# kepengxu/PGTFormer

Measured on NVIDIA B200. Metric: clips_per_s, higher is better.
Workload: dtype bf16

## Files before the change

pgtformer_b200/csrc/attention.cu:

```cuda
#include <cstdlib>

#include "common.cuh"

namespace pgt {

__device__ __forceinline__ void mma_bf16_16816(float (&c)[4], const uint32_t (&a)[4], uint32_t b0, uint32_t b1) {
  asm volatile(
      "mma.sync.aligned.m16n8k16.row.col.f32.bf16.bf16.f32 {%0,%1,%2,%3}, {%4,%5,%6,%7}, {%8,%9}, {%0,%1,%2,%3};"
      : "+f"(c[0]), "+f"(c[1]), "+f"(c[2]), "+f"(c[3])
      : "r"(a[0]), "r"(a[1]), "r"(a[2]), "r"(a[3]), "r"(b0), "r"(b1));
}
__device__ __forceinline__ void ldmatrix_x2_trans(uint32_t& r0, uint32_t& r1, const void* smem_row_ptr) {
  const uint32_t a = static_cast<uint32_t>(__cvta_generic_to_shared(smem_row_ptr));
  asm volatile("ldmatrix.sync.aligned.m8n8.x2.trans.shared.b16 {%0,%1}, [%2];" : "=r"(r0), "=r"(r1) : "r"(a));
}
__device__ __forceinline__ void cp_async16(void* smem_dst, const void* gsrc, bool pred) {
  const uint32_t d = static_cast<uint32_t>(__cvta_generic_to_shared(smem_dst));
  const int sz = pred ? 16 : 0;
  asm volatile("cp.async.cg.shared.global [%0], [%1], 16, %2;" ::"r"(d), "l"(gsrc), "r"(sz) : "memory");
}
__device__ __forceinline__ void cp_async_commit() { asm volatile("cp.async.commit_group;" ::: "memory"); }
template <int N>
__device__ __forceinline__ void cp_async_wait() { asm volatile("cp.async.wait_group %0;" ::"n"(N) : "memory"); }

constexpr int WIN_N = 48;

template <int D>
__global__ void __launch_bounds__(256)
window_attn_kernel(const __nv_bfloat16* __restrict__ qkv, int ldqkv, int H, int W, int C, int heads, int shift,
                   const float* __restrict__ bias_tab, __nv_bfloat16* __restrict__ out, int ldo) {
  extern __shared__ __align__(16) unsigned char smem_raw[];
  __shared__ int tok[WIN_N];
  __shared__ int lab[WIN_N];
  const int LDR = 3 * C + 8;
  __nv_bfloat16* rows = reinterpret_cast<__nv_bfloat16*>(smem_raw);
  const int nwx = W >> 2;
  const int wx = blockIdx.x % nwx, wy = blockIdx.x / nwx, clip = blockIdx.y;
  if (threadIdx.x < WIN_N) {
    const int i = threadIdx.x;
    const int fr = i >> 4, iy = (i >> 2) & 3, ix = i & 3;
    const int ys = wy * 4 + iy, xs = wx * 4 + ix;
    const int y = (ys + shift) % H, x = (xs + shift) % W;
    tok[i] = ((clip * 3 + fr) * H + y) * W + x;
    const int hr = ys < H - 4 ? 0 : (ys < H - shift ? 1 : 2);
    const int wr = xs < W - 4 ? 0 : (xs < W - shift ? 1 : 2);
    lab[i] = hr * 3 + wr;
  }
  __syncthreads();
  {
    const int chunks = (3 * C) >> 3;
    for (int i = threadIdx.x; i < WIN_N * chunks; i += 256) {
      const int r = i / chunks, c = i - r * chunks;
      cp_async16(rows + (size_t)r * LDR + c * 8, qkv + (size_t)tok[r] * ldqkv + c * 8, true);
    }
    cp_async_commit();
    cp_async_wait<0>();
  }
  __syncthreads();
  const int warp = threadIdx.x >> 5, lane = threadIdx.x & 31;
  const int g = lane >> 2, t = lane & 3;
  const float scale = rsqrtf((float)D);
  constexpr float LOG2E = 1.4426950408889634f;

// ... 69 lines not shown
        for (int nt = 0; nt < D / 8; ++nt) {
          uint32_t b0, b1;
          ldmatrix_x2_trans(b0, b1, vs + (size_t)(kk * 16 + (lane & 15)) * LDR + nt * 8);
          mma_bf16_16816(o[nt], a, b0, b1);
        }
      }
      __syncwarp();
      __nv_bfloat16* o0 = rows + (size_t)r0 * LDR + h * D;
      __nv_bfloat16* o1 = rows + (size_t)r1 * LDR + h * D;
#pragma unroll
      for (int nt = 0; nt < D / 8; ++nt) {
        *reinterpret_cast<uint32_t*>(o0 + nt * 8 + 2 * t) = pack_bf16x2(o[nt][0], o[nt][1]);
        *reinterpret_cast<uint32_t*>(o1 + nt * 8 + 2 * t) = pack_bf16x2(o[nt][2], o[nt][3]);
      }
    }
  }
  __syncthreads();
  {
    const int chunks = C >> 3;
    for (int i = threadIdx.x; i < WIN_N * chunks; i += 256) {
      const int r = i / chunks, c = i - r * chunks;
      *reinterpret_cast<uint4*>(out + (size_t)tok[r] * ldo + c * 8) = *reinterpret_cast<const uint4*>(rows + (size_t)r * LDR + c * 8);
    }
  }
}

constexpr int FA_BM = 64;
constexpr int FA_BN = 64;

template <int D>
__global__ void __launch_bounds__(128)
mha_fwd_kernel(const __nv_bfloat16* __restrict__ q, int ldq, const __nv_bfloat16* __restrict__ k, int ldk,
               const __nv_bfloat16* __restrict__ v, int ldv, int L, int heads, __nv_bfloat16* __restrict__ out, int ldo) {
  constexpr int LDS = D + 8;
  extern __shared__ __align__(16) unsigned char smem_raw[];
  __nv_bfloat16* ks = reinterpret_cast<__nv_bfloat16*>(smem_raw);
  __nv_bfloat16* vs = ks + 2 * FA_BN * LDS;
  const int qt = blockIdx.x, h = blockIdx.y, clip = blockIdx.z;
  const int warp = threadIdx.x >> 5, lane = threadIdx.x & 31, g = lane >> 2, t = lane & 3;
  const size_t row_base = (size_t)clip * L;
  const __nv_bfloat16* kbase = k + row_base * ldk + h * D;
  const __nv_bfloat16* vbase = v + row_base * ldv + h * D;
  const int ntiles = (L + FA_BN - 1) / FA_BN;
  constexpr int CH = D / 8;

  auto load_tile = [&](int tile, int buf) {
    for (int i = threadIdx.x; i < FA_BN * CH; i += 128) {
      const int r = i / CH, c = i % CH;
      const int key = tile * FA_BN + r;
      const bool ok = key < L;
      const size_t kr = ok ? key : 0;
      cp_async16(ks + ((size_t)buf * FA_BN + r) * LDS + c * 8, kbase + kr * ldk + c * 8, ok);
      cp_async16(vs + ((size_t)buf * FA_BN + r) * LDS + c * 8, vbase + kr * ldv + c * 8, ok);
    }
  };
  load_tile(0, 0);
  cp_async_commit();

  const int qr0 = qt * FA_BM + warp * 16 + g, qr1 = qr0 + 8;
  const bool v0 = qr0 < L, v1 = qr1 < L;
  const __nv_bfloat16* q0 = q + (row_base + (v0 ? qr0 : 0)) * ldq + h * D;
  const __nv_bfloat16* q1 = q + (row_base + (v1 ? qr1 : 0)) * ldq + h * D;
  uint32_t qa[D / 16][4];
#pragma unroll
  for (int kk = 0; kk < D / 16; ++kk) {
    qa[kk][0] = v0 ? __ldg(reinterpret_cast<const uint32_t*>(q0 + kk * 16 + 2 * t)) : 0u;
// ... 76 lines not shown
  __nv_bfloat16* o0 = out + (row_base + qr0) * ldo + h * D;
  __nv_bfloat16* o1 = out + (row_base + qr1) * ldo + h * D;
#pragma unroll
  for (int nt = 0; nt < D / 8; ++nt) {
    if (v0) *reinterpret_cast<uint32_t*>(o0 + nt * 8 + 2 * t) = pack_bf16x2(o[nt][0] * i0, o[nt][1] * i0);
    if (v1) *reinterpret_cast<uint32_t*>(o1 + nt * 8 + 2 * t) = pack_bf16x2(o[nt][2] * i1, o[nt][3] * i1);
  }
}

int mha_tc_launch(const void* q, int ldq, const void* k, int ldk, const void* v, int ldv, int clips, int L, int heads,
                  int d, void* out, int ldo, cudaStream_t stream);

}

using namespace pgt;

extern "C" int pgt_window_attention(const void* qkv, int ldqkv, int clips, int H, int W, int C, int heads, int shift,
                                    const float* bias_tab, void* out, int ldo, void* stream) {
  PGT_CHECK_ARG(qkv && bias_tab && out && clips > 0 && H > 0 && W > 0 && heads > 0);
  PGT_CHECK_ARG(H % 4 == 0 && W % 4 == 0 && C % heads == 0 && ldqkv % 8 == 0 && ldo % 8 == 0 && ldqkv >= 3 * C);
  PGT_CHECK_ARG(shift >= 0 && shift < 4);
  if (H <= 4 || W <= 4) shift = 0;
  const int d = C / heads;
  cudaStream_t st = static_cast<cudaStream_t>(stream);
  dim3 grid((H / 4) * (W / 4), clips);
  const size_t smem = (size_t)WIN_N * (3 * C + 8) * 2;
  ProfScope ps(PGT_PROF_WINDOW_ATTN, 4.0 * WIN_N * WIN_N * C * (double)grid.x * grid.y, st);
  if (d == 32) {
    static bool attr32 = false;
    if (!attr32) {
      PGT_CUDA_OK(cudaFuncSetAttribute(window_attn_kernel<32>, cudaFuncAttributeMaxDynamicSharedMemorySize, (int)smem));
      attr32 = true;
    }
    window_attn_kernel<32><<<grid, 256, smem, st>>>(reinterpret_cast<const __nv_bfloat16*>(qkv), ldqkv, H, W, C, heads,
                                                    shift, bias_tab, reinterpret_cast<__nv_bfloat16*>(out), ldo);
  } else if (d == 64) {
    static bool attr = false;
    if (!attr) {
      PGT_CUDA_OK(cudaFuncSetAttribute(window_attn_kernel<64>, cudaFuncAttributeMaxDynamicSharedMemorySize, (int)smem));
      attr = true;
    }
    window_attn_kernel<64><<<grid, 256, smem, st>>>(reinterpret_cast<const __nv_bfloat16*>(qkv), ldqkv, H, W, C, heads,
                                                    shift, bias_tab, reinterpret_cast<__nv_bfloat16*>(out), ldo);
  } else {
    return PGT_ERR_UNSUPPORTED;
  }
  PGT_LAUNCH_OK();
  return PGT_OK;
}

extern "C" int pgt_mha_fwd(const void* q, int ldq, const void* k, int ldk, const void* v, int ldv, int clips, int L,
                           int heads, int d, void* out, int ldo, void* stream) {
  PGT_CHECK_ARG(q && k && v && out && clips > 0 && L > 0 && heads > 0);
  PGT_CHECK_ARG(ldq % 8 == 0 && ldk % 8 == 0 && ldv % 8 == 0 && ldo % 8 == 0);
  if (d != 64) return PGT_ERR_UNSUPPORTED;
  static const bool no_tc = getenv("PGT_MHA_NO_TC") != nullptr;
  if (!no_tc) {
    ProfScope pst(PGT_PROF_MHA, 4.0 * (double)L * L * d * heads * clips, static_cast<cudaStream_t>(stream), "mha_tc");
    const int rc = mha_tc_launch(q, ldq, k, ldk, v, ldv, clips, L, heads, d, out, ldo, static_cast<cudaStream_t>(stream));
    if (rc != PGT_ERR_UNSUPPORTED) return rc;
  }
  dim3 grid(ceil_div(L, FA_BM), heads, clips);
  const size_t smem = (size_t)4 * FA_BN * (64 + 8) * 2;
  ProfScope ps(PGT_PROF_MHA, 4.0 * (double)L * L * d * heads * clips, static_cast<cudaStream_t>(stream));
  mha_fwd_kernel<64><<<grid, 128, smem, static_cast<cudaStream_t>(stream)>>>(
      reinterpret_cast<const __nv_bfloat16*>(q), ldq, reinterpret_cast<const __nv_bfloat16*>(k), ldk,
      reinterpret_cast<const __nv_bfloat16*>(v), ldv, L, heads, reinterpret_cast<__nv_bfloat16*>(out), ldo);
  PGT_LAUNCH_OK();
  return PGT_OK;
}
```

pgtformer_b200/csrc/codebook.cu:

```cuda
#include <float.h>

#include "common.cuh"

namespace pgt {

__global__ void __launch_bounds__(256)
argmax_gather_kernel(const float* __restrict__ logits, int T, int K, const float* __restrict__ codebook, int E,
                     const int64_t* __restrict__ idx_in, int64_t* __restrict__ idx_out, void* __restrict__ quant,
                     int ldq, int quant_dtype) {
  const int row = (blockIdx.x * blockDim.x + threadIdx.x) >> 5;
  const int lane = threadIdx.x & 31;
  if (row >= T) return;
  int best_i;
  if (idx_in != nullptr) {
    best_i = (int)idx_in[row];
  } else {
    const float4* p = reinterpret_cast<const float4*>(logits + (size_t)row * K);
    float best = -FLT_MAX;
    best_i = 0x7fffffff;
    const int nvec = K >> 2;
    for (int i = lane; i < nvec; i += 32) {
      float4 v;
      asm volatile("ld.global.nc.L1::no_allocate.v4.f32 {%0,%1,%2,%3}, [%4];"
                   : "=f"(v.x), "=f"(v.y), "=f"(v.z), "=f"(v.w) : "l"(p + i));
      const int b = i * 4;
      if (v.x > best) { best = v.x; best_i = b; }
      if (v.y > best) { best = v.y; best_i = b + 1; }
      if (v.z > best) { best = v.z; best_i = b + 2; }
      if (v.w > best) { best = v.w; best_i = b + 3; }
    }
#pragma unroll
    for (int o = 16; o > 0; o >>= 1) {
      const float ov = __shfl_xor_sync(0xffffffffu, best, o);
      const int oi = __shfl_xor_sync(0xffffffffu, best_i, o);
      if (ov > best || (ov == best && oi < best_i)) { best = ov; best_i = oi; }
    }
  }
  if (lane == 0 && idx_out != nullptr) idx_out[row] = best_i;
  if (quant != nullptr) {
    const float4* src = reinterpret_cast<const float4*>(codebook + (size_t)best_i * E);
    if (quant_dtype == PGT_BF16) {
      __nv_bfloat16* dst = reinterpret_cast<__nv_bfloat16*>(quant) + (size_t)row * ldq;
      for (int i = lane; i < (E >> 2); i += 32) {
        const float4 v = __ldg(src + i);
        uint2 u;
        u.x = pack_bf16x2(v.x, v.y);
        u.y = pack_bf16x2(v.z, v.w);
        *reinterpret_cast<uint2*>(dst + i * 4) = u;
      }
    } else {
      float4* dst = reinterpret_cast<float4*>(reinterpret_cast<float*>(quant) + (size_t)row * ldq);
      for (int i = lane; i < (E >> 2); i += 32) dst[i] = __ldg(src + i);
    }
  }
}

constexpr int AM_TT = 64;
constexpr int AM_TC = 64;
constexpr int AM_KC = 32;
constexpr int AM_LD = AM_TT + 4;

struct CandD {
  double v;
  int i;
};

__global__ void __launch_bounds__(256)
l2_argmin_kernel(const float* __restrict__ z, int T, int E, const float* __restrict__ cb, int K,
                 int64_t* __restrict__ idx, float* __restrict__ quant, const int* __restrict__ list,
                 const int* __restrict__ count, int min_count) {
  __shared__ __align__(16) float xs[AM_KC][AM_LD];
  __shared__ __align__(16) float es[AM_KC][AM_LD];
  __shared__ CandD merge[AM_TT][16];
  __shared__ int winner[AM_TT];
  const int tx = threadIdx.x & 15;
  const int ty = threadIdx.x >> 4;
  const int n_tok = list != nullptr ? *count : T;
  if (list != nullptr && n_tok <= min_count) return;
  auto token = [&](int i) { return list != nullptr ? list[i] : i; };
  const int lrow = threadIdx.x >> 2;
  const int lcol = (threadIdx.x & 3) * 8;
  for (int t0 = blockIdx.x * AM_TT; t0 < n_tok; t0 += gridDim.x * AM_TT) {
    CandD best[4];
#pragma unroll
    for (int a = 0; a < 4; ++a) { best[a].v = DBL_MAX; best[a].i = 0x7fffffff; }
    for (int c0 = 0; c0 < K; c0 += AM_TC) {
      double acc[4][4];
#pragma unroll
      for (int a = 0; a < 4; ++a)
#pragma unroll
        for (int b = 0; b < 4; ++b) acc[a][b] = 0.0;
      for (int k0 = 0; k0 < E; k0 += AM_KC) {
        {
          const int ti = t0 + lrow;
          float4 a = make_float4(0, 0, 0, 0), b = a;
          if (ti < n_tok) {
            const float4* p = reinterpret_cast<const float4*>(z + (size_t)token(ti) * E + k0 + lcol);
            a = __ldg(p); b = __ldg(p + 1);
          }
          xs[lcol + 0][lrow] = a.x; xs[lcol + 1][lrow] = a.y; xs[lcol + 2][lrow] = a.z; xs[lcol + 3][lrow] = a.w;
          xs[lcol + 4][lrow] = b.x; xs[lcol + 5][lrow] = b.y; xs[lcol + 6][lrow] = b.z; xs[lcol + 7][lrow] = b.w;
          const int c = c0 + lrow;
          a = make_float4(0, 0, 0, 0); b = a;
// ... 28 lines not shown
          const int c = c0 + tx * 4 + b;
          if (c < K && acc[a][b] < best[a].v) { best[a].v = acc[a][b]; best[a].i = c; }
        }
    }
#pragma unroll
    for (int a = 0; a < 4; ++a) merge[ty * 4 + a][tx] = best[a];
    __syncthreads();
    if (threadIdx.x < AM_TT) {
      CandD w = merge[threadIdx.x][0];
      for (int j = 1; j < 16; ++j) {
        const CandD c = merge[threadIdx.x][j];
        if (c.v < w.v || (c.v == w.v && c.i < w.i)) w = c;
      }
      winner[threadIdx.x] = w.i;
      if (t0 + threadIdx.x < n_tok) idx[token(t0 + threadIdx.x)] = w.i;
    }
    __syncthreads();
    if (quant != nullptr) {
      const int warp = threadIdx.x >> 5, lane = threadIdx.x & 31;
      for (int tt = warp; tt < AM_TT; tt += 8) {
        if (t0 + tt >= n_tok) continue;
        const int t = token(t0 + tt), bi = winner[tt];
        for (int e = lane; e < E; e += 32) quant[(size_t)t * E + e] = cb[(size_t)bi * E + e];
      }
    }
    __syncthreads();
  }
}

__global__ void __launch_bounds__(256)
l2_argmin_short_list_kernel(const float* __restrict__ z, int E, const float* __restrict__ cb, int K,
                            int64_t* __restrict__ idx, float* __restrict__ quant, const int* __restrict__ list,
                            const int* __restrict__ count, int max_count) {
  const int n_tok = *count;
  if (n_tok > max_count) return;
  const int lane = threadIdx.x & 31;
  const int gw = (blockIdx.x * blockDim.x + threadIdx.x) >> 5, nw = (gridDim.x * blockDim.x) >> 5;
  for (int i = gw; i < n_tok; i += nw) {
    const int t = list[i];
    double bd = DBL_MAX;
    int bi = 0x7fffffff;
    for (int k = 0; k < K; ++k) {
      double s = 0.0;
      for (int e = lane * 4; e < E; e += 128) {
        const float4 a = __ldg(reinterpret_cast<const float4*>(z + (size_t)t * E + e));
        const float4 b = __ldg(reinterpret_cast<const float4*>(cb + (size_t)k * E + e));
        double d;
        d = (double)a.x - (double)b.x; s = fma(d, d, s);
        d = (double)a.y - (double)b.y; s = fma(d, d, s);
        d = (double)a.z - (double)b.z; s = fma(d, d, s);
        d = (double)a.w - (double)b.w; s = fma(d, d, s);
      }
#pragma unroll
      for (int o = 16; o > 0; o >>= 1) s += __shfl_xor_sync(0xffffffffu, s, o);
      if (s < bd) { bd = s; bi = k; }
    }
    if (lane == 0) idx[t] = bi;
    if (quant != nullptr)
      for (int e = lane; e < E; e += 32) quant[(size_t)t * E + e] = cb[(size_t)bi * E + e];
  }
}

constexpr int AM_SHORT_LIST = 2048;

int l2_argmin_list_launch(const float* z, int T, int E, const float* codebook, int K, int64_t* idx, float* quant,
                          const int* list, const int* count, int grid, cudaStream_t st) {
  if (E % AM_KC != 0 || E % 4 != 0) return PGT_ERR_UNSUPPORTED;
  l2_argmin_short_list_kernel<<<num_sms(), 256, 0, st>>>(z, E, codebook, K, idx, quant, list, count, AM_SHORT_LIST);
  PGT_LAUNCH_OK();
  l2_argmin_kernel<<<grid, 256, 0, st>>>(z, T, E, codebook, K, idx, quant, list, count, AM_SHORT_LIST);
  PGT_LAUNCH_OK();
  return PGT_OK;
}

}

using namespace pgt;

extern "C" int pgt_argmax_gather(const float* logits, int T, int K, const float* codebook, int E,
                                 const int64_t* idx_in, int64_t* idx, void* quant, int ldq, int quant_dtype,
                                 void* stream) {
  PGT_CHECK_ARG((logits || idx_in) && T > 0 && K > 0 && K % 4 == 0);
  PGT_CHECK_ARG(quant == nullptr || (codebook != nullptr && E % 4 == 0 && ldq % 4 == 0));
  PGT_CHECK_ARG((reinterpret_cast<uintptr_t>(logits) & 15) == 0);
  const int warps = 8;
  ProfScope ps(PGT_PROF_ARGMAX, (double)T * K * 4 + (double)T * 8 + (quant ? (double)T * E * (quant_dtype == PGT_BF16 ? 2 : 4) : 0.0),
               static_cast<cudaStream_t>(stream));
  argmax_gather_kernel<<<ceil_div(T, warps), warps * 32, 0, static_cast<cudaStream_t>(stream)>>>(
      logits, T, K, codebook, E, idx_in, idx, quant, ldq, quant_dtype);
  PGT_LAUNCH_OK();
  return PGT_OK;
}

extern "C" int pgt_l2_argmin(const float* z, int T, int E, const float* codebook, int K, int64_t* idx, float* quant,
                             void* stream) {
  PGT_CHECK_ARG(z && codebook && idx && T > 0 && K > 0 && E > 0 && E % AM_KC == 0);
  PGT_CHECK_ARG((reinterpret_cast<uintptr_t>(z) & 15) == 0 && (reinterpret_cast<uintptr_t>(codebook) & 15) == 0);
  ProfScope ps(PGT_PROF_ARGMIN, 2.0 * T * (double)K * E, static_cast<cudaStream_t>(stream));
  l2_argmin_kernel<<<ceil_div(T, AM_TT), 256, 0, static_cast<cudaStream_t>(stream)>>>(z, T, E, codebook, K, idx, quant, nullptr, nullptr, 0);
  PGT_LAUNCH_OK();
  return PGT_OK;
}
```

pgtformer_b200/csrc/common.cuh:

```cuda
#pragma once
#include <cuda_bf16.h>
#include <cuda_runtime.h>
#include <stdint.h>

#include "../../include/pgt_b200.h"

namespace pgt {

void set_cuda_error(cudaError_t e, const char* where);
void count_launch(int n = 1);
int num_sms();
bool prof_enabled();
void prof_before(int cls, double work, cudaStream_t st, const char* desc);
void prof_after(cudaStream_t st);
struct ProfScope {
  cudaStream_t st; bool on;
  ProfScope(int cls, double work, cudaStream_t s, const char* desc = nullptr) : st(s), on(prof_enabled()) { if (on) prof_before(cls, work, s, desc); }
  ~ProfScope() { if (on) prof_after(st); }
};

#define PGT_CHECK_ARG(cond) \
  do {                      \
    if (!(cond)) return PGT_ERR_INVALID; \
  } while (0)

#define PGT_CUDA_OK(expr)                         \
  do {                                            \
    cudaError_t _e = (expr);                      \
    if (_e != cudaSuccess) {                      \
      ::pgt::set_cuda_error(_e, #expr);           \
      return PGT_ERR_CUDA;                        \
    }                                             \
  } while (0)

#define PGT_LAUNCH_OK()                           \
  do {                                            \
    cudaError_t _e = cudaGetLastError();          \
    if (_e != cudaSuccess) {                      \
      ::pgt::set_cuda_error(_e, "kernel launch"); \
      return PGT_ERR_CUDA;                        \
    }                                             \
    ::pgt::count_launch();                        \
  } while (0)

static inline int ceil_div(int a, int b) { return (a + b - 1) / b; }

__device__ __forceinline__ float rcp_approx(float x) {
  float r;
  asm("rcp.approx.ftz.f32 %0, %1;" : "=f"(r) : "f"(x));
  return r;
}
__device__ __forceinline__ float ex2_approx(float x) {
  float r;
  asm("ex2.approx.ftz.f32 %0, %1;" : "=f"(r) : "f"(x));
  return r;
}

__device__ __forceinline__ float gelu_erf(float v) {
  const float az = fabsf(v);
  const float t = rcp_approx(fmaf(0.3275911f * 0.70710678118654752440f, az, 1.0f));
  float poly = fmaf(1.061405429f, t, -1.453152027f);
  poly = fmaf(poly, t, 1.421413741f);
  poly = fmaf(poly, t, -0.284496736f);
  poly = fmaf(poly, t, 0.254829592f);
  const float e = ex2_approx(v * v * (-0.5f * 1.4426950408889634f));
  const float w = poly * t * e;
  return fmaf(az * -0.5f, w, fmaxf(v, 0.f));
}

__device__ __forceinline__ float apply_act(float v, int act) {
  switch (act) {
    case PGT_ACT_GELU: return gelu_erf(v);
    case PGT_ACT_SILU: return v * rcp_approx(1.0f + ex2_approx(v * -1.4426950408889634f));
    case PGT_ACT_LRELU02: return v > 0.f ? v : 0.2f * v;
    case PGT_ACT_RELU: return fmaxf(v, 0.f);
    case PGT_ACT_SIGMOID: return rcp_approx(1.0f + ex2_approx(v * -1.4426950408889634f));
    default: return v;
  }
// ... 25 lines not shown
```

pgtformer_b200/csrc/conv_out.cu:

```cuda
#include <cstdio>

#include "common.cuh"
#include "ptx.cuh"
#include "tmap.cuh"

namespace pgt {

constexpr int CO_TW = 8, CO_TH = 16;
constexpr int CO_SW = CO_TW + 2, CO_SH = CO_TH + 2;
constexpr int CO_PITCH = CO_SW * 128;
constexpr int CO_SLAB = ((CO_SH * CO_PITCH + 1023) / 1024) * 1024;
constexpr int CO_NB = 16;
constexpr int CO_WBYTES = 9 * CO_NB * 128;
constexpr int CO_BUILDERS = 256;
constexpr int CO_THREADS = 32 + CO_BUILDERS + 128;
constexpr int CO_SMEM = 2 * CO_SLAB + CO_WBYTES + 2 * 128 * 4  + 256 + 1024;

__device__ __forceinline__ uint64_t co_desc_sbo(uint32_t saddr, uint32_t sbo_bytes) {
  uint64_t d = 0;
  d |= static_cast<uint64_t>((saddr >> 4) & 0x3FFF);
  d |= static_cast<uint64_t>((sbo_bytes >> 4) & 0x3FFF) << 32;
  d |= static_cast<uint64_t>(1) << 46;
  d |= static_cast<uint64_t>(2) << 61;
  return d;
// ... 35 lines not shown
  uint8_t* sW = smem + 2 * CO_SLAB;
  float* sAB = reinterpret_cast<float*>(sW + CO_WBYTES);
  uint64_t* bars = reinterpret_cast<uint64_t*>(sAB + 2 * 128);
  uint64_t* slab_full = bars;
  uint64_t* slab_empty = bars + 2;
  uint64_t* acc_full = bars + 4;
  uint64_t* acc_empty = bars + 6;
  uint32_t* tmem_ptr = reinterpret_cast<uint32_t*>(bars + 8);

  const int warp = threadIdx.x >> 5, lane = threadIdx.x & 31;
  if (warp == 0) {
    if (lane == 0) {
      for (int i = 0; i < 2; ++i) {
        mbar_init(&slab_full[i], CO_BUILDERS);
        mbar_init(&slab_empty[i], 1);
        mbar_init(&acc_full[i], 1);
        mbar_init(&acc_empty[i], 128);
      }
      fence_barrier_init();
    }
    tmem_alloc<32>(tmem_ptr);
    tc_fence_before();
  }
  for (int i = threadIdx.x; i < 9 * CO_NB * 8; i += CO_THREADS) {
    const int tap = i / (CO_NB * 8), r = (i / 8) % CO_NB, ch = i % 8;
    uint4 v = make_uint4(0, 0, 0, 0);
    if (r < p.cout) v = __ldg(reinterpret_cast<const uint4*>(p.w + (size_t)r * p.ldw + tap * 64 + ch * 8));
    *reinterpret_cast<uint4*>(sW + tap * (CO_NB * 128) + r * 128 + ((ch ^ (r & 7)) << 4)) = v;
  }
  fence_proxy_async();
  __syncthreads();
  tc_fence_after();
  const uint32_t tmem_base = *tmem_ptr;
  const int per_frame = p.tiles_x * p.tiles_y;

  if (warp == 0) {
    constexpr uint32_t idesc = umma_idesc_bf16(128, CO_NB);
    int it = 0;
    for (int tile = blockIdx.x; tile < p.num_tiles; tile += gridDim.x, ++it) {
      const int buf = it & 1;
      const uint32_t ph = (it >> 1) & 1;
      mbar_wait(&slab_full[buf], ph);
      mbar_wait(&acc_empty[buf], ph ^ 1);
      tc_fence_after();
      if (elect_one()) {
        const uint32_t sa = smem_u32(slab + buf * CO_SLAB);
#pragma unroll
        for (int tap = 0; tap < 9; ++tap) {
          const uint64_t da = co_desc_sbo(sa + ((tap / 3) * CO_SW + (tap % 3)) * 128, CO_PITCH);
          const uint64_t db = umma_desc_k_sw128(smem_u32(sW + tap * (CO_NB * 128)));
#pragma unroll
          for (int k = 0; k < 4; ++k) umma_bf16_ss(tmem_base + buf * CO_NB, da + 2 * k, db + 2 * k, idesc, (tap | k) != 0 ? 1u : 0u);
        }
        umma_commit(&slab_empty[buf]);
        umma_commit(&acc_full[buf]);
      }
      __syncwarp();
    }
  } else if (warp <= 8) {
    const int bt = threadIdx.x - 32;
    const int chunk = bt & 7;
    int it = 0;
    for (int tile = blockIdx.x; tile < p.num_tiles; tile += gridDim.x, ++it) {
      const int buf = it & 1;
      const uint32_t ph = (it >> 1) & 1;
      const int f = tile / per_frame, r = tile - f * per_frame;
// ... 69 lines not shown
    }
  }

  tc_fence_before();
  __syncthreads();
  if (warp == 0) {
    tc_fence_after();
    tmem_dealloc<32>(tmem_base);
  }
}

}

using namespace pgt;

extern "C" int pgt_conv_out_gn(const void* x, int F, int H, int W, int Cin, int ldx, const float* gn_ab, const void* Wp,
                               int ldw, int Cout, const float* bias, float* out, void* stream) {
  PGT_CHECK_ARG(x && gn_ab && Wp && out && F > 0);
  if (Cin != 64 || Cout < 1 || Cout > 3 || H % CO_TH != 0 || W % CO_TW != 0 || ldx % 8 != 0 || ldw % 8 != 0)
    return PGT_ERR_UNSUPPORTED;
  PGT_CHECK_ARG((reinterpret_cast<uintptr_t>(x) & 15) == 0 && (reinterpret_cast<uintptr_t>(Wp) & 15) == 0 &&
                (reinterpret_cast<uintptr_t>(gn_ab) & 15) == 0);
  cudaStream_t st = static_cast<cudaStream_t>(stream);
  ConvOutParams p{};
  p.x = reinterpret_cast<const __nv_bfloat16*>(x); p.ldx = ldx; p.F = F; p.H = H; p.W = W; p.cout = Cout;
  p.ab = gn_ab; p.w = reinterpret_cast<const __nv_bfloat16*>(Wp); p.ldw = ldw; p.bias = bias; p.out = out;
  p.tiles_x = W / CO_TW; p.tiles_y = H / CO_TH; p.num_tiles = F * p.tiles_x * p.tiles_y;
  static PerDeviceOnce once;
  PGT_CUDA_OK(once.run([] { return cudaFuncSetAttribute(conv_out_gn_kernel, cudaFuncAttributeMaxDynamicSharedMemorySize, CO_SMEM); }));
  const int grid = p.num_tiles < 2 * num_sms() ? p.num_tiles : 2 * num_sms();
  char desc[64];
  snprintf(desc, sizeof(desc), "conv_out_gn F%d H%d W%d N%d", F, H, W, Cout);
  ProfScope ps(PGT_PROF_GEMM, 2.0 * F * (double)H * W * Cout * 9 * Cin, st, desc);
  conv_out_gn_kernel<<<grid, CO_THREADS, CO_SMEM, st>>>(p);
  PGT_LAUNCH_OK();
  return PGT_OK;
}
```

pgtformer_b200/csrc/elementwise.cu:

```cuda
#include <algorithm>

#include "common.cuh"
#include "tmap.cuh"

namespace pgt {

__global__ void copy2d_kernel(const __nv_bfloat16* __restrict__ x, int ldx, size_t T, int C,
                              __nv_bfloat16* __restrict__ y, int ldy) {
  const int vc = C >> 3;
  const size_t total = T * vc;
  const size_t stride = (size_t)gridDim.x * blockDim.x;
  size_t i = (size_t)blockIdx.x * blockDim.x + threadIdx.x;
  for (; i + 3 * stride < total; i += 4 * stride) {
    uint4 u[4];
#pragma unroll
    for (int k = 0; k < 4; ++k) {
      const size_t j = i + k * stride;
      u[k] = __ldg(reinterpret_cast<const uint4*>(x + (j / vc) * ldx) + (j % vc));
    }
#pragma unroll
    for (int k = 0; k < 4; ++k) {
      const size_t j = i + k * stride;
      reinterpret_cast<uint4*>(y + (j / vc) * ldy)[j % vc] = u[k];
    }
  }
  for (; i < total; i += stride)
    reinterpret_cast<uint4*>(y + (i / vc) * ldy)[i % vc] = __ldg(reinterpret_cast<const uint4*>(x + (i / vc) * ldx) + (i % vc));
}

__global__ void nchw_to_nhwc_kernel(const float* __restrict__ x, int C, int HW, const float* __restrict__ mean,
                                    const float* __restrict__ stdv, __nv_bfloat16* __restrict__ y, int ldy) {
  __shared__ float tile[32][33];
  const int f = blockIdx.z;
  const int p0 = blockIdx.x * 32, c0 = blockIdx.y * 32;
  for (int j = threadIdx.y; j < 32; j += blockDim.y) {
    const int c = c0 + j, p = p0 + threadIdx.x;
    float v = 0.f;
    if (c < C && p < HW) {
      v = x[((size_t)f * C + c) * HW + p];
      if (mean != nullptr) v = (v - mean[c]) / stdv[c];
    }
    tile[j][threadIdx.x] = v;
  }
  __syncthreads();
  for (int j = threadIdx.y; j < 32; j += blockDim.y) {
    const int p = p0 + j, c = c0 + threadIdx.x;
    if (p < HW && c < ldy && c0 + 32 <= ((C + 31) / 32) * 32) {
      if (c < C) y[((size_t)f * HW + p) * ldy + c] = __float2bfloat16_rn(tile[threadIdx.x][j]);
    }
  }
}

__global__ void nhwc_to_f32_kernel(const __nv_bfloat16* __restrict__ x, int ldx, int HW, int C, float* __restrict__ y,
                                   int to_nchw) {
  __shared__ float tile[32][33];
  const int f = blockIdx.z;
  const int p0 = blockIdx.x * 32, c0 = blockIdx.y * 32;
  for (int j = threadIdx.y; j < 32; j += blockDim.y) {
    const int p = p0 + j, c = c0 + threadIdx.x;
    tile[j][threadIdx.x] = (p < HW && c < C) ? __bfloat162float(x[((size_t)f * HW + p) * ldx + c]) : 0.f;
  }
  __syncthreads();
  if (to_nchw) {
    for (int j = threadIdx.y; j < 32; j += blockDim.y) {
      const int c = c0 + j, p = p0 + threadIdx.x;
      if (c < C && p < HW) y[((size_t)f * C + c) * HW + p] = tile[threadIdx.x][j];
    }
  } else {
    for (int j = threadIdx.y; j < 32; j += blockDim.y) {
      const int p = p0 + j, c = c0 + threadIdx.x;
      if (c < C && p < HW) y[((size_t)f * HW + p) * C + c] = tile[j][threadIdx.x];
    }
  }
}

}

using namespace pgt;

static int ew_grid(size_t total, int threads) {
  size_t b = (total + threads - 1) / threads;
  const size_t cap = (size_t)num_sms() * 32;
  return (int)(b < cap ? (b ? b : 1) : cap);
}

extern "C" int pgt_copy2d(const void* x, int ldx, int T, int C, void* y, int ldy, void* stream) {
  PGT_CHECK_ARG(x && y && T > 0 && C % 8 == 0 && ldx % 8 == 0 && ldy % 8 == 0);
  ProfScope ps(PGT_PROF_MOVE, 2.0 * (double)T * C * 2, static_cast<cudaStream_t>(stream), "pgt_copy2d");
  const size_t total = (size_t)T * (C / 8);
  copy2d_kernel<<<ew_grid(total, 256), 256, 0, static_cast<cudaStream_t>(stream)>>>(
      reinterpret_cast<const __nv_bfloat16*>(x), ldx, (size_t)T, C, reinterpret_cast<__nv_bfloat16*>(y), ldy);
  PGT_LAUNCH_OK();
  return PGT_OK;
}

extern "C" int pgt_nchw_f32_to_nhwc_bf16(const float* x, int F, int C, int HW, const float* mean, const float* stdv,
                                         void* y, int ldy, void* stream) {
  PGT_CHECK_ARG(x && y && F > 0 && C > 0 && HW > 0 && ldy >= C && (mean == nullptr) == (stdv == nullptr));
  ProfScope ps(PGT_PROF_MOVE, 6.0 * F * (double)C * HW, static_cast<cudaStream_t>(stream), "pgt_nchw_f32_to_nhwc_bf16");
  dim3 grid(ceil_div(HW, 32), ceil_div(C, 32), F);
  nchw_to_nhwc_kernel<<<grid, dim3(32, 8), 0, static_cast<cudaStream_t>(stream)>>>(
      x, C, HW, mean, stdv, reinterpret_cast<__nv_bfloat16*>(y), ldy);
  PGT_LAUNCH_OK();
  return PGT_OK;
}

extern "C" int pgt_nhwc_bf16_to_f32(const void* x, int ldx, int F, int HW, int C, float* y, int to_nchw, void* stream) {
  PGT_CHECK_ARG(x && y && F > 0 && C > 0 && HW > 0 && ldx >= C);
  ProfScope ps(PGT_PROF_MOVE, 6.0 * F * (double)C * HW, static_cast<cudaStream_t>(stream), "pgt_nhwc_bf16_to_f32");
  dim3 grid(ceil_div(HW, 32), ceil_div(C, 32), F);
  nhwc_to_f32_kernel<<<grid, dim3(32, 8), 0, static_cast<cudaStream_t>(stream)>>>(
      reinterpret_cast<const __nv_bfloat16*>(x), ldx, HW, C, y, to_nchw);
  PGT_LAUNCH_OK();
  return PGT_OK;
}

namespace pgt {
__global__ void regroup_frames_kernel(const __nv_bfloat16* __restrict__ x, int ldx, int b, int P, int C,
                                      __nv_bfloat16* __restrict__ y, int ldy, int dir) {
  const int vc = C >> 3;
  const size_t total = (size_t)b * 3 * P * vc;
  for (size_t i = (size_t)blockIdx.x * blockDim.x + threadIdx.x; i < total; i += (size_t)gridDim.x * blockDim.x) {
    const int v = (int)(i % vc);
    size_t r = i / vc;
    const int p = (int)(r % P); r /= P;
    const int fr = (int)(r % 3);
    const int clip = (int)(r / 3);
    const size_t frame_row = ((size_t)clip * 3 + fr) * P + p;
    const size_t clip_row = (size_t)clip * P + p;
    if (dir == 0)
      reinterpret_cast<uint4*>(y + clip_row * ldy + fr * C)[v] = __ldg(reinterpret_cast<const uint4*>(x + frame_row * ldx) + v);
    else
      reinterpret_cast<uint4*>(y + frame_row * ldy)[v] = __ldg(reinterpret_cast<const uint4*>(x + clip_row * ldx + fr * C) + v);
  }
}
}

extern "C" int pgt_regroup_frames(const void* x, int ldx, int clips, int P, int C, void* y, int ldy, int dir,
                                  void* stream) {
  PGT_CHECK_ARG(x && y && clips > 0 && P > 0 && C % 8 == 0 && ldx % 8 == 0 && ldy % 8 == 0 && (dir == 0 || dir == 1));
  ProfScope ps(PGT_PROF_MOVE, 4.0 * clips * 3.0 * P * C, static_cast<cudaStream_t>(stream), "pgt_regroup_frames");
  const size_t total = (size_t)clips * 3 * P * (C / 8);
  regroup_frames_kernel<<<ew_grid(total, 256), 256, 0, static_cast<cudaStream_t>(stream)>>>(
      reinterpret_cast<const __nv_bfloat16*>(x), ldx, clips, P, C, reinterpret_cast<__nv_bfloat16*>(y), ldy, dir);
  PGT_LAUNCH_OK();
  return PGT_OK;
}


namespace pgt {
__constant__ float c_u8_to_unit[256];

__global__ void u8hwc_to_f32nchw_kernel(const uint8_t* __restrict__ x, size_t HW, size_t total, float* __restrict__ y) {
  for (size_t i = (size_t)blockIdx.x * blockDim.x + threadIdx.x; i < total; i += (size_t)gridDim.x * blockDim.x) {
    const size_t f = i / HW, p = i - f * HW;
    const uint8_t* s = x + (f * HW + p) * 3;
    float* d = y + f * 3 * HW + p;
    d[0] = c_u8_to_unit[s[0]];
    d[HW] = c_u8_to_unit[s[1]];
    d[2 * HW] = c_u8_to_unit[s[2]];
  }
}

__global__ void f32nchw_to_u8hwc_kernel(const float* __restrict__ x, size_t HW, int first, int step, size_t total,
                                        uint8_t* __restrict__ y) {
  for (size_t i = (size_t)blockIdx.x * blockDim.x + threadIdx.x; i < total; i += (size_t)gridDim.x * blockDim.x) {
    const size_t j = i / HW, p = i - j * HW;
    const float* s = x + ((size_t)first + j * step) * 3 * HW + p;
    uint8_t* d = y + (j * HW + p) * 3;
#pragma unroll
    for (int c = 0; c < 3; ++c) {
      const float v = fminf(fmaxf(s[c * HW], 0.f), 1.f) * 255.0f;
      d[c] = (uint8_t)v;
    }
  }
}

__global__ void gather_frames_kernel(const uint4* __restrict__ x, size_t vec_per_frame, const int* __restrict__ idx,
                                     uint4* __restrict__ y) {
  const uint4* s = x + (size_t)idx[blockIdx.y] * vec_per_frame;
  uint4* d = y + (size_t)blockIdx.y * vec_per_frame;
  for (size_t i = (size_t)blockIdx.x * blockDim.x + threadIdx.x; i < vec_per_frame; i += (size_t)gridDim.x * blockDim.x)
    d[i] = __ldg(s + i);
}
}

extern "C" int pgt_u8hwc_to_f32nchw(const void* x_u8, int F, int H, int W, float* y, void* stream) {
  PGT_CHECK_ARG(x_u8 && y && F > 0 && H > 0 && W > 0);
  static pgt::PerDeviceOnce once;
  PGT_CUDA_OK(once.run([] {
    float t[256];
    for (int v = 0; v < 256; ++v) t[v] = (float)((double)v / 255.0);
    return cudaMemcpyToSymbol(pgt::c_u8_to_unit, t, sizeof(t));
  }));
  const size_t HW = (size_t)H * W, total = (size_t)F * HW;
  ProfScope ps(PGT_PROF_MOVE, 15.0 * (double)total, static_cast<cudaStream_t>(stream), "pgt_u8hwc_to_f32nchw");
  pgt::u8hwc_to_f32nchw_kernel<<<ew_grid(total, 256), 256, 0, static_cast<cudaStream_t>(stream)>>>(
      static_cast<const uint8_t*>(x_u8), HW, total, y);
  PGT_LAUNCH_OK();
  return PGT_OK;
}

extern "C" int pgt_f32nchw_to_u8hwc(const float* x, int first, int step, int n, int H, int W, void* y_u8, void* stream) {
  PGT_CHECK_ARG(x && y_u8 && n > 0 && H > 0 && W > 0 && first >= 0 && step >= 1);
  const size_t HW = (size_t)H * W, total = (size_t)n * HW;
  ProfScope ps(PGT_PROF_MOVE, 15.0 * (double)total, static_cast<cudaStream_t>(stream), "pgt_f32nchw_to_u8hwc");
  pgt::f32nchw_to_u8hwc_kernel<<<ew_grid(total, 256), 256, 0, static_cast<cudaStream_t>(stream)>>>(
      x, HW, first, step, total, static_cast<uint8_t*>(y_u8));
  PGT_LAUNCH_OK();
  return PGT_OK;
}

extern "C" int pgt_gather_frames(const void* x, long long frame_bytes, const int* idx_dev, int n, void* y, void* stream) {
  PGT_CHECK_ARG(x && y && idx_dev && n > 0 && frame_bytes > 0 && frame_bytes % 16 == 0);
  PGT_CHECK_ARG((reinterpret_cast<uintptr_t>(x) & 15) == 0 && (reinterpret_cast<uintptr_t>(y) & 15) == 0);
  const size_t vec = (size_t)frame_bytes / 16;
  ProfScope ps(PGT_PROF_MOVE, 2.0 * (double)n * frame_bytes, static_cast<cudaStream_t>(stream), "pgt_gather_frames");
  unsigned bx = (unsigned)std::min<size_t>((vec + 255) / 256, 1024);
  pgt::gather_frames_kernel<<<dim3(bx, n), 256, 0, static_cast<cudaStream_t>(stream)>>>(
      static_cast<const uint4*>(x), vec, idx_dev, static_cast<uint4*>(y));
  PGT_LAUNCH_OK();
  return PGT_OK;
}
```

pgtformer_b200/csrc/gemm_tc.cu:

```cuda
#include <cudaTypedefs.h>
#include <cstdio>
#include <cstdlib>

#include "common.cuh"
#include "tmap.cuh"
#include "ptx.cuh"
#include "epi_common.cuh"

namespace pgt {

constexpr int BM = 128;
constexpr int BK = 64;
constexpr int EPI_WARPS = 8;
constexpr int GEMM_THREADS = 64 + EPI_WARPS * 32 + 32;
constexpr int A_STAGE_BYTES = BM * BK * 2;
constexpr int PANEL_BYTES = BM * 128;
constexpr int NUM_SLOTS = 4;
constexpr int PREFETCH_TILES = 2;

enum { MODE_LINEAR = 0, MODE_CONV_S1 = 1, MODE_CONV_S2 = 2 };

struct GemmParams {
  int mode;
  int M, N, K;
// ... 497 lines not shown
  const int num_tiles = p.m_tiles * p.n_tiles;

  if (warp == 0 && lane == 0) {
    tma_prefetch_desc(&tmA);
    tma_prefetch_desc(&tmB);
    if (p.fast_epi) tma_prefetch_desc(&tmO);
    if (p.has_res_map) tma_prefetch_desc(&tmR);
    if (p.fast_epi && p.epi_mode == PGT_EPI_SFT) tma_prefetch_desc(&tmX);
    for (int i = 0; i < STAGES; ++i) {
      mbar_init(&full_bar[i], 1);
      mbar_init(&empty_bar[i], 1);
    }
    for (int i = 0; i < 2; ++i) {
      mbar_init(&tmem_full[i], 1);
      mbar_init(&tmem_empty[i], PAIR ? 2 * EPI_WARPS : EPI_WARPS * 32);
      mbar_init(&res_bar[2 * i], 1);
      mbar_init(&res_bar[2 * i + 1], 1);
      mbar_init(&slot_ready[2 * i], EPI_WARPS * 32);
      mbar_init(&slot_ready[2 * i + 1], EPI_WARPS * 32);
    }
    fence_barrier_init();
  }
  if (warp == 1) {
    if constexpr (PAIR) tmem_alloc_2cta<Cfg::TMEM_COLS>(tmem_ptr);
    else tmem_alloc<Cfg::TMEM_COLS>(tmem_ptr);
    tc_fence_before();
  }
  __syncthreads();
  if constexpr (PAIR) cluster_sync_all();
  tc_fence_after();
  const uint32_t tmem_base = *tmem_ptr;
  const uint32_t rank = PAIR ? cluster_ctarank() : 0u;

  if (warp == 0) {
    {
      int stage = 0;
      uint32_t phase = 0;
      for (int tile = blockIdx.x; tile < num_tiles; tile += gridDim.x) {
        int n_blk, m_blk;
        tile_mn(p, tile, m_blk, n_blk);
        int n0 = 0, y0 = 0, x0 = 0;
        if (p.mode != MODE_LINEAR) decode_conv_tile(p, m_blk, n0, y0, x0);
        for (int kb = 0; kb < p.num_kb; ++kb) {
          mbar_wait(&empty_bar[stage], phase ^ 1);
          if (elect_one()) {
            void* dst_a = smem_a + stage * A_STAGE_BYTES;
            void* dst_b = smem_b + stage * Cfg::B_STAGE_BYTES;
            int cb = 0, ax = 0, ay = 0, a5 = 0;
            if (p.mode != MODE_LINEAR) {
              const int tap = kb / p.cin_blocks;
              cb = kb - tap * p.cin_blocks;
              const int dy = tap / p.ksize;
              const int dx = tap - dy * p.ksize;
              if (p.mode == MODE_CONV_S1) {
                ax = x0 + dx - p.pad_x; ay = y0 + dy - p.pad_y;
              } else {
                const int oy = dy - p.pad_lo, ox = dx - p.pad_lo;
                const int qy = (oy < 0) ? -((1 - oy) >> 1) : (oy >> 1);
                const int qx = (ox < 0) ? -((1 - ox) >> 1) : (ox >> 1);
                const int py = oy - 2 * qy, px = ox - 2 * qx;
                cb = px * p.cin_ld + cb * BK;
                ax = x0 + qx; ay = y0 + qy; a5 = py;
              }
            }
            if constexpr (PAIR) {
              const uint32_t fb = mapa_u32(smem_u32(&full_bar[stage]), 0);
              if (rank == 0) mbar_arrive_expect_tx(&full_bar[stage], 2 * Cfg::STAGE_BYTES);
              if (p.mode == MODE_LINEAR) tma_load_2d_2sm(dst_a, &tmA, fb, kb * BK, m_blk * BM);
              else if (p.mode == MODE_CONV_S1) tma_load_4d_2sm(dst_a, &tmA, fb, cb * BK, ax, ay, n0);
              else tma_load_5d_2sm(dst_a, &tmA, fb, cb, ax, a5, ay, n0);
              tma_load_2d_2sm(dst_b, &tmB, fb, kb * BK, n_blk * BN + (int)rank * (BN / 2));
            } else {
              mbar_arrive_expect_tx(&full_bar[stage], Cfg::STAGE_BYTES);
              if (p.mode == MODE_LINEAR) tma_load_2d(dst_a, &tmA, &full_bar[stage], kb * BK, m_blk * BM);
              else if (p.mode == MODE_CONV_S1) tma_load_4d(dst_a, &tmA, &full_bar[stage], cb * BK, ax, ay, n0);
              else tma_load_5d(dst_a, &tmA, &full_bar[stage], cb, ax, a5, ay, n0);
              tma_load_2d(dst_b, &tmB, &full_bar[stage], kb * BK, n_blk * BN);
            }
          }
          __syncwarp();
          if (++stage == STAGES) { stage = 0; phase ^= 1; }
        }
      }
    }
  } else if (warp == 1) {
    if (!PAIR || rank == 0) {
      constexpr uint32_t idesc = umma_idesc_bf16(PAIR ? 2 * BM : BM, BN);
      int stage = 0;
      uint32_t phase = 0;
      int it = 0;
      for (int tile = blockIdx.x; tile < num_tiles; tile += gridDim.x, ++it) {
        const int acc = it & 1;
        const uint32_t acc_phase = (it >> 1) & 1;
        mbar_wait(&tmem_empty[acc], acc_phase ^ 1);
        tc_fence_after();
        const uint32_t d_tmem = tmem_base + acc * BN;
        if (elect_one()) {
          int s = stage;
          uint32_t ph = phase;
          const uint64_t da0 = umma_desc_k_sw128(smem_u32(smem_a));
          const uint64_t db0 = umma_desc_k_sw128(smem_u32(smem_b));
          for (int kb = 0; kb < p.num_kb; ++kb) {
            mbar_wait(&full_bar[s], ph);
            tc_fence_after();
            const uint64_t da = da0 + (uint64_t)(s * (A_STAGE_BYTES >> 4));
            const uint64_t db = db0 + (uint64_t)(s * (Cfg::B_STAGE_BYTES >> 4));
#pragma unroll
            for (int k = 0; k < BK / 16; ++k) {
              if constexpr (PAIR) umma_bf16_ss_2cta(d_tmem, da + 2 * k, db + 2 * k, idesc, (kb | k) != 0 ? 1u : 0u);
              else umma_bf16_ss(d_tmem, da + 2 * k, db + 2 * k, idesc, (kb | k) != 0 ? 1u : 0u);
// ... 82 lines not shown
  uint64_t* a_ready = tmem_full + 14;

  const int warp = threadIdx.x >> 5;
  const int lane = threadIdx.x & 31;
  const int num_tiles = p.m_tiles * p.n_tiles;
  const int cin_pad = p.cin_blocks * BK;

  if (warp == 0 && lane == 0) {
    tma_prefetch_desc(&tmA);
    tma_prefetch_desc(&tmB);
    if (p.fast_epi) tma_prefetch_desc(&tmO);
    if (p.has_res_map) tma_prefetch_desc(&tmR);
    if (p.fast_epi && p.epi_mode == PGT_EPI_SFT) tma_prefetch_desc(&tmX);
    for (int i = 0; i < AS; ++i) { mbar_init(&a_full[i], 1); mbar_init(&a_empty[i], 1); mbar_init(&a_ready[i], HALO_GN_THREADS); }
    for (int i = 0; i < BS; ++i) { mbar_init(&b_full[i], 1); mbar_init(&b_empty[i], 1); }
    for (int i = 0; i < 2; ++i) {
      mbar_init(&tmem_full[i], 1);
      mbar_init(&tmem_empty[i], EPI_WARPS * 32);
      mbar_init(&res_bar[2 * i], 1);
      mbar_init(&res_bar[2 * i + 1], 1);
      mbar_init(&slot_ready[2 * i], EPI_WARPS * 32);
      mbar_init(&slot_ready[2 * i + 1], EPI_WARPS * 32);
    }
    fence_barrier_init();
  }
  if (warp == 1) {
    tmem_alloc<Cfg::TMEM_COLS>(tmem_ptr);
    tc_fence_before();
  }
  __syncthreads();
  tc_fence_after();
  const uint32_t tmem_base = *tmem_ptr;

  if (warp == 0) {
    int as = 0, bs = 0;
    uint32_t aph = 0, bph = 0;
    for (int tile = blockIdx.x; tile < num_tiles; tile += gridDim.x) {
      const int n_blk = tile % p.n_tiles;
      const int m_blk = tile / p.n_tiles;
      int n0, y0, x0;
      decode_conv_tile(p, m_blk, n0, y0, x0);
      {
        const int pt = tile + PREFETCH_TILES * (int)gridDim.x;
        if (BN == 64 && pt < num_tiles && elect_one()) {
          int pn0, py0, px0;
          decode_conv_tile(p, pt / p.n_tiles, pn0, py0, px0);
          for (int cb = 0; cb < p.cin_blocks; ++cb) tma_prefetch_4d(&tmA, cb * BK, px0 - 1, py0 - 1, pn0);
          if (p.has_res_map) {
            const int c0 = (pt % p.n_tiles) * BN;
            const int rw = p.out_dtype == PGT_BF16 ? 64 : 32;
            for (int c = 0; c < BN && c0 + c < p.N; c += rw) {
              tma_prefetch_4d(&tmR, c0 + c, px0, py0, pn0);
              if (p.epi_mode == PGT_EPI_SFT) tma_prefetch_4d(&tmX, c0 + c, px0, py0, pn0);
            }
          }
        }
        __syncwarp();
      }
      for (int cb = 0; cb < p.cin_blocks; ++cb) {
        mbar_wait(&a_empty[as], aph ^ 1);
        if (elect_one()) {
          mbar_arrive_expect_tx(&a_full[as], HALO_A_BYTES);
          tma_load_4d(smem_a + as * HALO_A_STRIDE, &tmA, &a_full[as], cb * BK, x0 - 1, y0 - 1, n0);
        }
        __syncwarp();
        if (++as == AS) { as = 0; aph ^= 1; }
        if (p.b_resident && tile != (int)blockIdx.x) continue;
        for (int t = 0; t < p.ntaps; ++t) {
          mbar_wait(&b_empty[bs], bph ^ 1);
          if (elect_one()) {
            mbar_arrive_expect_tx(&b_full[bs], Cfg::B_BYTES);
            tma_load_2d(smem_b + bs * Cfg::B_BYTES, &tmB, &b_full[bs], t * cin_pad + cb * BK, n_blk * BN);
          }
          __syncwarp();
          if (++bs == BS) { bs = 0; bph ^= 1; }
        }
      }
    }
  } else if (warp == 1) {
    constexpr uint32_t idesc = umma_idesc_bf16(BM, BN);
    int as = 0, bs = 0;
    uint32_t aph = 0, bph = 0;
    int it = 0;
    for (int tile = blockIdx.x; tile < num_tiles; tile += gridDim.x, ++it) {
      const int acc = it & 1;
      const uint32_t acc_phase = (it >> 1) & 1;
      mbar_wait(&tmem_empty[acc], acc_phase ^ 1);
      tc_fence_after();
      const uint32_t d_tmem = tmem_base + acc * BN;
      if (elect_one()) {
        int a = as, b = bs;
        uint32_t ap = aph, bp = bph;
        const uint64_t da_base = umma_desc_k_sw128_sbo(smem_u32(smem_a), HALO_PITCH);
        const uint64_t db_base = umma_desc_k_sw128(smem_u32(smem_b));
        for (int cb = 0; cb < p.cin_blocks; ++cb) {
          mbar_wait(GN ? &a_ready[a] : &a_full[a], ap);
          const uint64_t da0 = da_base + (uint64_t)(a * (HALO_A_STRIDE >> 4));
          if (p.b_resident) {
            if (it == 0) {
              for (int t = 0; t < p.ntaps; ++t) mbar_wait(&b_full[cb * p.ntaps + t], 0);
            }
            tc_fence_after();
            if (p.ntaps == 9) {
#pragma unroll
              for (int t = 0; t < 9; ++t) {
                const uint64_t da = da0 + (uint64_t)(((t / 3) * (HALO_TW + 2) + (t % 3)) * 8);
                const uint64_t db = db_base + (uint64_t)((cb * 9 + t) * (Cfg::B_BYTES >> 4));
// ... 155 lines not shown

  const int warp = threadIdx.x >> 5;
  const int lane = threadIdx.x & 31;
  const uint32_t rank = cluster_ctarank();
  const int num_tiles = p.m_tiles;
  const int cin_pad = p.cin_blocks * BK;

  if (warp == 0 && lane == 0) {
    tma_prefetch_desc(&tmA);
    tma_prefetch_desc(&tmB);
    if (p.fast_epi) tma_prefetch_desc(&tmO);
    if (p.has_res_map) tma_prefetch_desc(&tmR);
    if (p.fast_epi && p.epi_mode == PGT_EPI_SFT) tma_prefetch_desc(&tmX);
    for (int i = 0; i < AS; ++i) { mbar_init(&a_full[i], 1); mbar_init(&a_empty[i], 1); }
    for (int i = 0; i < BS; ++i) { mbar_init(&b_full[i], 1); mbar_init(&b_empty[i], 1); }
    for (int i = 0; i < 2; ++i) {
      mbar_init(&tmem_full[i], 1);
      mbar_init(&tmem_empty[i], 2 * EPI_WARPS);
      mbar_init(&res_bar[2 * i], 1);
      mbar_init(&res_bar[2 * i + 1], 1);
      mbar_init(&slot_ready[2 * i], EPI_WARPS * 32);
      mbar_init(&slot_ready[2 * i + 1], EPI_WARPS * 32);
    }
    fence_barrier_init();
  }
  if (warp == 1) {
    tmem_alloc_2cta<Cfg::TMEM_COLS>(tmem_ptr);
    tc_fence_before();
  }
  __syncthreads();
  cluster_sync_all();
  tc_fence_after();
  const uint32_t tmem_base = *tmem_ptr;

  if (warp == 0) {
    int as = 0, bs = 0;
    uint32_t aph = 0, bph = 0;
    const uint32_t a_full0 = mapa_u32(smem_u32(a_full), 0), b_full0 = mapa_u32(smem_u32(b_full), 0);
    for (int tile = blockIdx.x; tile < num_tiles; tile += gridDim.x) {
      int n0, y0, x0;
      decode_conv_tile(p, tile, n0, y0, x0);
      {
        const int pt = tile + PREFETCH_TILES * (int)gridDim.x;
        if (BN == 64 && pt < num_tiles && elect_one()) {
          int pn0, py0, px0;
          decode_conv_tile(p, pt, pn0, py0, px0);
          for (int cb = 0; cb < p.cin_blocks; ++cb) tma_prefetch_4d(&tmA, cb * BK, px0 - 1, py0 - 1, pn0);
          if (p.has_res_map) {
            const int rw = p.out_dtype == PGT_BF16 ? 64 : 32;
            for (int c = 0; c < BN && c < p.N; c += rw) {
              tma_prefetch_4d(&tmR, c, px0, py0, pn0);
              if (p.epi_mode == PGT_EPI_SFT) tma_prefetch_4d(&tmX, c, px0, py0, pn0);
            }
          }
        }
        __syncwarp();
      }
      for (int cb = 0; cb < p.cin_blocks; ++cb) {
        mbar_wait(&a_empty[as], aph ^ 1);
        if (elect_one()) {
          if (rank == 0) mbar_arrive_expect_tx(&a_full[as], 2 * HALO_A_BYTES);
          tma_load_4d_2sm(smem_a + as * HALO_A_STRIDE, &tmA, a_full0 + as * 8, cb * BK, x0 - 1, y0 - 1, n0);
        }
        __syncwarp();
        if (++as == AS) { as = 0; aph ^= 1; }
        if (p.b_resident && tile != (int)blockIdx.x) continue;
        for (int t = 0; t < p.ntaps; ++t) {
          mbar_wait(&b_empty[bs], bph ^ 1);
          if (elect_one()) {
            if (rank == 0) mbar_arrive_expect_tx(&b_full[bs], 2 * Cfg::B_BYTES);
            tma_load_2d_2sm(smem_b + bs * Cfg::B_BYTES, &tmB, b_full0 + bs * 8, t * cin_pad + cb * BK, (int)rank * (BN / 2));
          }
          __syncwarp();
          if (++bs == BS) { bs = 0; bph ^= 1; }
        }
      }
    }
  } else if (warp == 1) {
    if (rank == 0) {
      constexpr uint32_t idesc = umma_idesc_bf16(2 * BM, BN);
      int as = 0, bs = 0;
      uint32_t aph = 0, bph = 0;
      int it = 0;
      for (int tile = blockIdx.x; tile < num_tiles; tile += gridDim.x, ++it) {
        const int acc = it & 1;
        const uint32_t acc_phase = (it >> 1) & 1;
        mbar_wait(&tmem_empty[acc], acc_phase ^ 1);
        tc_fence_after();
        const uint32_t d_tmem = tmem_base + acc * BN;
        if (elect_one()) {
          int a = as, b = bs;
          uint32_t ap = aph, bp = bph;
          const uint64_t da_base = umma_desc_k_sw128_sbo(smem_u32(smem_a), HALO_PITCH);
          const uint64_t db_base = umma_desc_k_sw128(smem_u32(smem_b));
          for (int cb = 0; cb < p.cin_blocks; ++cb) {
            mbar_wait(&a_full[a], ap);
            const uint64_t da0 = da_base + (uint64_t)(a * (HALO_A_STRIDE >> 4));
            if (p.ntaps == 9) {
#pragma unroll
              for (int t = 0; t < 9; ++t) {
                int slot = b;
                if (p.b_resident) {
                  slot = cb * 9 + t;
                  if (it == 0) mbar_wait(&b_full[slot], 0);
                } else {
                  mbar_wait(&b_full[b], bp);
// ... 126 lines not shown
  return PGT_OK;
}

static int encode_weight_map(CUtensorMap* tmB, const void* W, int ldw, int K, int N, int BN) {
  uint64_t dims[2] = {(uint64_t)K, (uint64_t)N};
  uint64_t str[1] = {(uint64_t)ldw * 2};
  uint32_t box[2] = {BK, (uint32_t)BN};
  return encode_map(tmB, W, 2, dims, str, box);
}

template <int BN, bool PAIR>
static int launch_gemm(const CUtensorMap& tmA, const void* W, int ldw, GemmParams& p, cudaStream_t stream) {
  using Cfg = GemmCfg<BN, PAIR>;
  static_assert(Cfg::STAGES >= 3, "pipeline too shallow");
  CUtensorMap tmB, tmO, tmR, tmX;
  int rc = encode_weight_map(&tmB, W, ldw, p.K, p.N, PAIR ? BN / 2 : BN);
  if (rc != PGT_OK) return rc;
  rc = setup_epilogue_maps(p, tmA, tmO, tmR, tmX);
  if (rc != PGT_OK) return rc;
  p.n_tiles = ceil_div(p.N, BN);
  p.pair_map = PAIR ? 1 : 0;
  static PerDeviceOnce once;
  PGT_CUDA_OK(once.run([] { return cudaFuncSetAttribute(gemm_tc_kernel<BN, PAIR>, cudaFuncAttributeMaxDynamicSharedMemorySize, Cfg::SMEM_BYTES); }));
  const int tiles = p.m_tiles * p.n_tiles;
  int grid = tiles < num_sms() ? tiles : num_sms();
  if (PAIR) grid &= ~1;
  {
    char desc[96];
    if (prof_enabled()) {
      if (p.mode == MODE_LINEAR) snprintf(desc, sizeof(desc), "linear%s M%d N%d K%d BN%d e%d", PAIR ? " x2cta" : "", p.M, p.N, p.K, BN, p.fast_epi);
      else snprintf(desc, sizeof(desc), "conv%d%s s%d F%d H%d W%d K%d N%d BN%d t%dx%dx%d e%d", p.ksize, PAIR ? " x2cta" : "", p.mode, p.F, p.H, p.W, p.K, p.N, BN, p.tn, p.th, p.tw, p.fast_epi);
    }
    ProfScope ps(PGT_PROF_GEMM, p.flops, stream, desc);
    if (PAIR) {
      cudaLaunchConfig_t cfg = {};
      cfg.gridDim = dim3(grid); cfg.blockDim = dim3(GEMM_THREADS); cfg.dynamicSmemBytes = Cfg::SMEM_BYTES; cfg.stream = stream;
      cudaLaunchAttribute attr[1];
      attr[0].id = cudaLaunchAttributeClusterDimension;
      attr[0].val.clusterDim.x = 2; attr[0].val.clusterDim.y = 1; attr[0].val.clusterDim.z = 1;
      cfg.attrs = attr; cfg.numAttrs = 1;
      PGT_CUDA_OK(cudaLaunchKernelEx(&cfg, gemm_tc_kernel<BN, PAIR>, tmA, tmB, tmO, tmR, tmX, p));
    } else {
      gemm_tc_kernel<BN, PAIR><<<grid, GEMM_THREADS, Cfg::SMEM_BYTES, stream>>>(tmA, tmB, tmO, tmR, tmX, p);
    }
  }
  PGT_LAUNCH_OK();
  return PGT_OK;
}

template <int BN, bool GN>
static int launch_halo(const CUtensorMap& tmA, const void* W, int ldw, GemmParams& p, cudaStream_t stream) {
  using Cfg = HaloCfg<BN>;
  CUtensorMap tmB, tmO, tmR, tmX;
  int rc = encode_weight_map(&tmB, W, ldw, p.K, p.N, BN);
  if (rc != PGT_OK) return rc;
  rc = setup_epilogue_maps(p, tmA, tmO, tmR, tmX);
  if (rc != PGT_OK) return rc;
  p.n_tiles = ceil_div(p.N, BN);
  p.b_resident = (p.ntaps * p.cin_blocks <= Cfg::B_STAGES && p.n_tiles == 1) ? 1 : 0;
  static PerDeviceOnce once;
  PGT_CUDA_OK(once.run([] { return cudaFuncSetAttribute(conv_halo_kernel<BN, GN>, cudaFuncAttributeMaxDynamicSharedMemorySize, Cfg::SMEM_BYTES); }));
  const int tiles = p.m_tiles * p.n_tiles;
  const int grid = tiles < num_sms() ? tiles : num_sms();
  {
    char desc[96];
    if (prof_enabled())
      snprintf(desc, sizeof(desc), "halo3%s F%d H%d W%d K%d N%d BN%d e%d r%d", GN ? "+gn" : "", p.F, p.H, p.W, p.K, p.N, BN,
               p.fast_epi, p.b_resident);
    ProfScope ps(PGT_PROF_GEMM, p.flops, stream, desc);
    conv_halo_kernel<BN, GN><<<grid, GN ? GEMM_THREADS + HALO_GN_THREADS : GEMM_THREADS, Cfg::SMEM_BYTES, stream>>>(
        tmA, tmB, tmO, tmR, tmX, p);
  }
  PGT_LAUNCH_OK();
  return PGT_OK;
}

template <int BN>
static int launch_halo2(const CUtensorMap& tmA, const void* W, int ldw, GemmParams& p, cudaStream_t stream) {
  using Cfg = Halo2Cfg<BN>;
  CUtensorMap tmB, tmO, tmR, tmX;
  int rc = encode_weight_map(&tmB, W, ldw, p.K, p.N, BN / 2);
  if (rc != PGT_OK) return rc;
  rc = setup_epilogue_maps(p, tmA, tmO, tmR, tmX);
  if (rc != PGT_OK) return rc;
  p.n_tiles = 1;
  p.b_resident = (p.ntaps * p.cin_blocks <= Cfg::B_STAGES) ? 1 : 0;
  static PerDeviceOnce once;
  PGT_CUDA_OK(once.run([] { return cudaFuncSetAttribute(conv_halo2_kernel<BN>, cudaFuncAttributeMaxDynamicSharedMemorySize, Cfg::SMEM_BYTES); }));
  int grid = p.m_tiles < num_sms() ? p.m_tiles : num_sms();
  grid &= ~1;
  {
    char desc[96];
    if (prof_enabled())
      snprintf(desc, sizeof(desc), "halo%d x2cta F%d H%d W%d K%d N%d BN%d e%d r%d", p.tap_kw, p.F, p.H, p.W, p.K, p.N, BN,
               p.fast_epi, p.b_resident);
    ProfScope ps(PGT_PROF_GEMM, p.flops, stream, desc);
    conv_halo2_kernel<BN><<<grid, GEMM_THREADS, Cfg::SMEM_BYTES, stream>>>(tmA, tmB, tmO, tmR, tmX, p);
  }
  PGT_LAUNCH_OK();
  return PGT_OK;
}

static int pick_bn(int N, int m_tiles) {
  if (N <= 64) return 64;
  if (N <= 128) return 128;
  const int t256 = m_tiles * ceil_div(N, 256);
  return (t256 >= num_sms()) ? 256 : 128;
}

static int dispatch_gemm(const CUtensorMap& tmA, const void* W, int ldw, GemmParams& p, cudaStream_t stream) {
  static const bool no_pair = getenv("PGT_NO_2CTA") != nullptr;
  switch (pick_bn(p.N, p.m_tiles)) {
    case 64: return launch_gemm<64, false>(tmA, W, ldw, p, stream);
    case 128: return launch_gemm<128, false>(tmA, W, ldw, p, stream);
    default:
      if (!no_pair && p.mode != MODE_LINEAR && p.num_kb >= 16 && (p.m_tiles % 2) == 0 && p.m_tiles >= 2)
        return launch_gemm<256, true>(tmA, W, ldw, p, stream);
      return launch_gemm<256, false>(tmA, W, ldw, p, stream);
  }
}

static int fill_epilogue(GemmParams& p, const pgt_epilogue* ep) {
  if (ep == nullptr || ep->out == nullptr) return PGT_ERR_INVALID;
  p.bias = ep->bias;
  p.act = ep->act;
  p.epi_mode = ep->mode;
  p.residual = ep->residual;
  p.ldr = ep->ldr;
  p.res_dtype = ep->res_dtype;
  p.aux = ep->aux;
  p.ldaux = ep->ldaux;
  p.sft_w = ep->sft_w;
// ... 188 lines not shown
```

pgtformer_b200/csrc/l2_argmin_tc.cu:

```cuda
#include <float.h>

#include "common.cuh"
#include "ptx.cuh"
#include "tmap.cuh"

namespace pgt {

constexpr int LT_BM = 128;
constexpr int LT_BN = 256;
constexpr int LT_BK = 64;
constexpr int LT_EMAX = 512;
constexpr int LT_A_KB_BYTES = LT_BM * 128;
constexpr int LT_KBMAX = LT_EMAX / LT_BK;
constexpr int LT_BST = (LT_BN / 2) * 128;
constexpr int LT_NST = 3;
constexpr int LT_THREADS = 11 * 32;
constexpr int LT_TOP = 16;
constexpr int LT_LIST = 16;
constexpr int LT_XCH = 2 * LT_BM * LT_LIST * 8  + 2 * LT_BM * 4  + LT_BM * LT_TOP * 4  + 2 * LT_BM * 4 ;
constexpr int LT_SMEM = LT_BM * LT_EMAX * 2 + LT_NST * LT_BST + LT_XCH + 512  + 1024 ;

__device__ __forceinline__ float4 ld_nc_f4(const float4* p) {
  float4 v;
  asm("ld.global.nc.L1::no_allocate.v4.f32 {%0,%1,%2,%3}, [%4];" : "=f"(v.x), "=f"(v.y), "=f"(v.z), "=f"(v.w) : "l"(p));
  return v;
}

__global__ void __launch_bounds__(256)
codebook_pack_kernel(const float* __restrict__ cb, int K, int E, __nv_bfloat16* __restrict__ cb16, float* __restrict__ norm) {
  const int row = (blockIdx.x * blockDim.x + threadIdx.x) >> 5, lane = threadIdx.x & 31;
  if (row >= K) return;
  double s = 0.0;
  float sr = 0.f, sd = 0.f;
  for (int e = lane; e < E; e += 32) {
    const float v = cb[(size_t)row * E + e];
    const __nv_bfloat16 b = __float2bfloat16_rn(v);
    const float vb = __bfloat162float(b);
    cb16[(size_t)row * E + e] = b;
    s += (double)v * (double)v;
    sr = fmaf(vb, vb, sr);
    const float dd = v - vb;
    sd = fmaf(dd, dd, sd);
  }
#pragma unroll
  for (int o = 16; o > 0; o >>= 1) {
    s += __shfl_xor_sync(0xffffffffu, s, o);
    sr += __shfl_xor_sync(0xffffffffu, sr, o);
    sd += __shfl_xor_sync(0xffffffffu, sd, o);
  }
  if (lane == 0) {
    norm[row] = (float)s;
    atomicMax(reinterpret_cast<int*>(norm + K), __float_as_int(sr * 1.0001f));
    atomicMax(reinterpret_cast<int*>(norm + K + 1), __float_as_int(sd * 1.0001f));
  }
}

__global__ void __launch_bounds__(256)
z_pack_kernel(const float* __restrict__ z, int T, int E, __nv_bfloat16* __restrict__ zb, float2* __restrict__ zn2) {
  constexpr int RB = 4;
  const int lane = threadIdx.x & 31;
  const int gw = (blockIdx.x * blockDim.x + threadIdx.x) >> 5, nw = (gridDim.x * blockDim.x) >> 5;
  const int nstep = (E + 255) / 256;
  for (int t0 = gw * RB; t0 < T; t0 += nw * RB) {
    float4 va[RB][2][2];
#pragma unroll
    for (int i = 0; i < RB; ++i) {
#pragma unroll
      for (int sp = 0; sp < 2; ++sp) {
        const int c = sp * 256 + lane * 8;
        if (sp < nstep && t0 + i < T && c < E) {
          const float4* p = reinterpret_cast<const float4*>(z + (size_t)(t0 + i) * E + c);
          va[i][sp][0] = ld_nc_f4(p);
          va[i][sp][1] = ld_nc_f4(p + 1);
        } else {
          va[i][sp][0] = va[i][sp][1] = make_float4(0.f, 0.f, 0.f, 0.f);
        }
      }
    }
#pragma unroll
    for (int i = 0; i < RB; ++i) {
      const int t = t0 + i;
      if (t >= T) break;
      float s2 = 0.f, d2 = 0.f;
#pragma unroll
      for (int sp = 0; sp < 2; ++sp) {
        const int c = sp * 256 + lane * 8;
        if (sp < nstep && c < E) {
          const float4 a = va[i][sp][0], b = va[i][sp][1];
          const float f[8] = {a.x, a.y, a.z, a.w, b.x, b.y, b.z, b.w};
          uint32_t u[4];
#pragma unroll
// ... 138 lines not shown
  int* ncand = mi + LT_BM * LT_TOP;
  int* ovf = ncand + LT_BM;
  uint64_t* b_full = reinterpret_cast<uint64_t*>(tail + LT_XCH);
  uint64_t* b_empty = b_full + LT_NST;
  uint64_t* a_full = b_empty + LT_NST;
  uint64_t* a_empty = a_full + LT_KBMAX;
  uint64_t* t_full = a_empty + LT_KBMAX;
  uint64_t* t_empty = t_full + 2;
  uint32_t* tmem_ptr = reinterpret_cast<uint32_t*>(t_empty + 2);

  const int warp = threadIdx.x >> 5, lane = threadIdx.x & 31;
  const int KB = E / LT_BK;
  const int NT = K / LT_BN;
  const int n_pt = (T + 2 * LT_BM - 1) / (2 * LT_BM);
  const int pair = blockIdx.x >> 1, npairs = gridDim.x >> 1;

  if (warp == 0 && lane == 0) {
    tma_prefetch_desc(&tmA);
    tma_prefetch_desc(&tmB);
    for (int i = 0; i < LT_NST; ++i) { mbar_init(&b_full[i], 1); mbar_init(&b_empty[i], 1); }
    for (int i = 0; i < LT_KBMAX; ++i) { mbar_init(&a_full[i], 1); mbar_init(&a_empty[i], 1); }
    for (int i = 0; i < 2; ++i) { mbar_init(&t_full[i], 1); mbar_init(&t_empty[i], 8); }
    fence_barrier_init();
  }
  if (warp == 1) {
    tmem_alloc_2cta<512>(tmem_ptr);
    tc_fence_before();
  }
  if (threadIdx.x < LT_BM) { ncand[threadIdx.x] = 0; ovf[threadIdx.x] = 0; }
  __syncthreads();
  cluster_sync_all();
  tc_fence_after();
  const uint32_t tmem_base = *tmem_ptr;
  const uint32_t rank = cluster_ctarank();

  if (warp == 0) {
    int st = 0;
    uint32_t ph = 0;
    for (int pt = pair; pt < n_pt; pt += npairs) {
      for (int nt = 0; nt < NT; ++nt) {
        for (int kb = 0; kb < KB; ++kb) {
          mbar_wait(&b_empty[st], ph ^ 1);
          if (elect_one()) {
            const uint32_t fb = mapa_u32(smem_u32(&b_full[st]), 0);
            if (rank == 0) mbar_arrive_expect_tx(&b_full[st], 2 * LT_BST);
            tma_load_2d_2sm(sB + st * LT_BST, &tmB, fb, kb * LT_BK, nt * LT_BN + (int)rank * (LT_BN / 2));
          }
          __syncwarp();
          if (++st == LT_NST) { st = 0; ph ^= 1; }
        }
      }
    }
  } else if (warp == 10) {
    int it = 0;
    for (int pt = pair; pt < n_pt; pt += npairs, ++it) {
      const int t0 = pt * 2 * LT_BM + (int)rank * LT_BM;
      for (int kb = 0; kb < KB; ++kb) {
        if (it > 0) mbar_wait(&a_empty[kb], (it - 1) & 1);
        if (elect_one()) {
          const uint32_t fa = mapa_u32(smem_u32(&a_full[kb]), 0);
          if (rank == 0) mbar_arrive_expect_tx(&a_full[kb], 2 * LT_A_KB_BYTES);
          tma_load_2d_2sm(sA + kb * LT_A_KB_BYTES, &tmA, fa, kb * LT_BK, t0);
        }
        __syncwarp();
      }
    }
// ... 101 lines not shown
          while (have != 0) {
            const int l = __ffs(have) - 1;
            have &= have - 1;
            const int b = __shfl_sync(0xffffffffu, best, l);
            const float4* src = reinterpret_cast<const float4*>(cb + (size_t)b * E);
            float4* dst = reinterpret_cast<float4*>(quant + (size_t)(t0 + w8 + 8 * l) * E);
            for (int e = lane; e < (E >> 2); e += 32) dst[e] = __ldg(src + e);
          }
        }
      }
    }
  }

  tc_fence_before();
  __syncthreads();
  cluster_sync_all();
  if (warp == 1) {
    tc_fence_after();
    tmem_dealloc_2cta<512>(tmem_base);
  }
}

int l2_argmin_list_launch(const float* z, int T, int E, const float* codebook, int K, int64_t* idx, float* quant,
                          const int* list, const int* count, int grid, cudaStream_t st);

}

using namespace pgt;

extern "C" int pgt_codebook_pack(const float* codebook, int K, int E, void* cb_bf16, float* cb_norm, void* stream) {
  PGT_CHECK_ARG(codebook && cb_bf16 && cb_norm && K > 0 && E > 0);
  cudaStream_t st = static_cast<cudaStream_t>(stream);
  PGT_CUDA_OK(cudaMemsetAsync(cb_norm + K, 0, 2 * sizeof(float), st));
  codebook_pack_kernel<<<ceil_div(K, 8), 256, 0, st>>>(codebook, K, E, reinterpret_cast<__nv_bfloat16*>(cb_bf16), cb_norm);
  PGT_LAUNCH_OK();
  return PGT_OK;
}

static inline int64_t ws_align4(int64_t v) { return (v + 3) & ~int64_t(3); }
static inline int64_t ws_off_list(int T) { (void)T; return 4; }
static inline int64_t ws_off_zn2(int T) { return ws_align4(ws_off_list(T) + T); }
static inline int64_t ws_off_zb(int T) { return ws_align4(ws_off_zn2(T) + (int64_t)T * 2); }

extern "C" int64_t pgt_l2_argmin_ws_ints(int T) {
  return ws_off_zb(T) + (int64_t)T * (LT_EMAX / 2);
}

extern "C" int pgt_l2_argmin_tc(const float* z, int T, int E, const float* codebook, const void* cb_bf16,
                                const float* cb_norm, int K, int64_t* idx, float* quant, int32_t* workspace,
                                void* stream) {
  PGT_CHECK_ARG(z && codebook && cb_bf16 && cb_norm && idx && workspace && T > 0);
  if (K % LT_BN != 0 || E % LT_BK != 0 || E > LT_EMAX || E % 128 != 0) return PGT_ERR_UNSUPPORTED;
  PGT_CHECK_ARG((reinterpret_cast<uintptr_t>(z) & 15) == 0 && (reinterpret_cast<uintptr_t>(codebook) & 15) == 0 &&
                (reinterpret_cast<uintptr_t>(cb_bf16) & 15) == 0 && (reinterpret_cast<uintptr_t>(workspace) & 15) == 0 &&
                (quant == nullptr || (reinterpret_cast<uintptr_t>(quant) & 15) == 0));
  cudaStream_t st = static_cast<cudaStream_t>(stream);
  int* fb_count = workspace;
  int* fb_list = workspace + ws_off_list(T);
  float2* zn2 = reinterpret_cast<float2*>(workspace + ws_off_zn2(T));
  __nv_bfloat16* zb = reinterpret_cast<__nv_bfloat16*>(workspace + ws_off_zb(T));
  CUtensorMap tmA, tmB;
  int rc = tmap_rows_bf16(&tmA, zb, E, T, E, LT_BM);
  if (rc == PGT_OK) rc = tmap_rows_bf16(&tmB, cb_bf16, E, K, E, LT_BN / 2);
  if (rc != PGT_OK) return rc;
  static PerDeviceOnce once;
  PGT_CUDA_OK(once.run([] { return cudaFuncSetAttribute(l2_argmin_pair_kernel, cudaFuncAttributeMaxDynamicSharedMemorySize, LT_SMEM); }));
  PGT_CUDA_OK(cudaMemsetAsync(workspace, 0, sizeof(int32_t), st));
  const int n_pt = ceil_div(T, 2 * LT_BM);
  const int npairs = n_pt < num_sms() / 2 ? n_pt : num_sms() / 2;
  {
    ProfScope ps(PGT_PROF_ARGMIN, 2.0 * T * (double)K * E, st, "l2_argmin_tc");
    int pack_ctas = num_sms() * 2;
    {
      const long long items = ceil_div(T, 4);
      long long best_waste = -1;
      for (int c = num_sms() * 2; c >= num_sms(); --c) {
        const long long w = (long long)c * 8;
        const long long waste = ((items + w - 1) / w) * w - items;
        if (best_waste < 0 || waste < best_waste) { best_waste = waste; pack_ctas = c; }
      }
    }
    z_pack_kernel<<<pack_ctas, 256, 0, st>>>(z, T, E, zb, zn2);
    l2_argmin_pair_kernel<<<2 * npairs, LT_THREADS, LT_SMEM, st>>>(tmA, tmB, z, zn2, T, E, codebook, cb_norm, K, idx, quant,
                                                                   fb_count, fb_list);
    PGT_LAUNCH_OK();
  }
  return l2_argmin_list_launch(z, T, E, codebook, K, idx, quant, fb_list, fb_count, num_sms(), st);
}
```

pgtformer_b200/csrc/ln_linear.cu:

```cuda
#include <cudaTypedefs.h>

#include <cstdio>

#include "common.cuh"
#include "tmap.cuh"
#include "ptx.cuh"

namespace pgt {

constexpr int LL_C = 256;
constexpr int LL_BM = 128;
constexpr int LL_SUB = LL_BM * 128;
constexpr int LL_WST = 2;
constexpr int LL_WBYTES = LL_C * 128;
constexpr int LL_THREADS = 480;
constexpr int LL_SMEM = 8 * LL_SUB  + 2 * LL_SUB  + LL_WST * LL_WBYTES + 256;
static_assert(LL_SMEM <= 232448, "ln_linear smem budget");

struct LnLinearParams {
  int T, m_tiles, nb;
  const float* ln_g;
  const float* ln_b;
  float eps;
  const float* bias;
// ... 7 lines not shown
  uint8_t* sX = smem;
  uint8_t* sO = sX + 8 * LL_SUB;
  uint8_t* sW = sO + 2 * LL_SUB;
  uint64_t* bars = reinterpret_cast<uint64_t*>(sW + LL_WST * LL_WBYTES);
  uint64_t* x_full = bars;
  uint64_t* sx_free = bars + 2;
  uint64_t* y_ready = bars + 4;
  uint64_t* acc_full = bars + 6;
  uint64_t* acc_free = bars + 8;
  uint64_t* so_free = bars + 10;
  uint64_t* out_ready = bars + 12;
  uint64_t* w_full = bars + 14;
  uint64_t* w_empty = w_full + LL_WST;
  uint32_t* tmem_ptr = reinterpret_cast<uint32_t*>(w_empty + LL_WST);

  const int warp = threadIdx.x >> 5, lane = threadIdx.x & 31;
  if (warp == 0 && lane == 0) {
    tma_prefetch_desc(&tmX); tma_prefetch_desc(&tmO); tma_prefetch_desc(&tmW);
    for (int i = 0; i < 2; ++i) {
      mbar_init(&x_full[i], 1); mbar_init(&sx_free[i], 1); mbar_init(&y_ready[i], 128);
      mbar_init(&acc_full[i], 1); mbar_init(&acc_free[i], 256);
      mbar_init(&so_free[i], 1); mbar_init(&out_ready[i], 256);
    }
    for (int i = 0; i < LL_WST; ++i) { mbar_init(&w_full[i], 1); mbar_init(&w_empty[i], 1); }
    fence_barrier_init();
  }
  if (warp == 1) {
    tmem_alloc<512>(tmem_ptr);
    tc_fence_before();
  }
  __syncthreads();
  tc_fence_after();
  const uint32_t tmem_base = *tmem_ptr;
  const int NB = p.nb;

  if (warp == 0) {
    int st = 0;
    uint32_t ph = 0;
    for (int tile = blockIdx.x; tile < p.m_tiles; tile += gridDim.x) {
      for (int j = 0; j < NB; ++j) {
        for (int kb = 0; kb < 4; ++kb) {
          mbar_wait(&w_empty[st], ph ^ 1);
          if (elect_one()) {
            mbar_arrive_expect_tx(&w_full[st], LL_WBYTES);
            tma_load_2d(sW + st * LL_WBYTES, &tmW, &w_full[st], kb * 64, j * LL_C);
          }
          __syncwarp();
          if (++st == LL_WST) { st = 0; ph ^= 1; }
        }
      }
    }
  } else if (warp == 1) {
    constexpr uint32_t idesc = umma_idesc_bf16(LL_BM, LL_C);
    int st = 0;
    uint32_t ph = 0;
    int it = 0;
    for (int tile = blockIdx.x; tile < p.m_tiles; tile += gridDim.x, ++it) {
      const int xb = it & 1;
      mbar_wait(&y_ready[xb], (it >> 1) & 1);
      tc_fence_after();
      if (elect_one()) {
        int s = st;
        uint32_t sp = ph;
        const uint64_t da0 = umma_desc_k_sw128(smem_u32(sX + xb * 4 * LL_SUB));
        const uint64_t db0 = umma_desc_k_sw128(smem_u32(sW));
        for (int j = 0; j < NB; ++j) {
// ... 173 lines not shown
  }
}

static int ll_enc2d(CUtensorMap* map, const void* base, int ld, long long rows, int cols, int box_rows) {
  return tmap_rows_bf16(map, base, ld, rows, cols, box_rows);
}

}

using namespace pgt;

extern "C" int pgt_ln_linear_bf16(const void* x, int ldx, int T, int C, const float* ln_g, const float* ln_b, float eps,
                                  const void* W, int ldw, int N, const float* bias, void* out, int ldo, void* stream) {
  PGT_CHECK_ARG(x && out && W && bias && T > 0 && N > 0 && ((ln_g == nullptr) == (ln_b == nullptr)));
  if (C != LL_C || (N % LL_C) != 0) return PGT_ERR_UNSUPPORTED;
  auto al = [](const void* q) { return (reinterpret_cast<uintptr_t>(q) & 15) == 0; };
  PGT_CHECK_ARG(al(x) && al(out) && al(W) && ldx % 8 == 0 && ldo % 8 == 0 && ldw % 8 == 0 && ldw >= C && ldo >= N);
  CUtensorMap tx, to, tw;
  int rc = ll_enc2d(&tx, x, ldx, T, C, LL_BM);
  if (rc == PGT_OK) rc = ll_enc2d(&to, out, ldo, T, N, LL_BM);
  if (rc == PGT_OK) rc = ll_enc2d(&tw, W, ldw, N, C, LL_C);
  if (rc != PGT_OK) return rc;
  static PerDeviceOnce once;
  PGT_CUDA_OK(once.run([] { return cudaFuncSetAttribute(ln_linear_kernel, cudaFuncAttributeMaxDynamicSharedMemorySize, LL_SMEM); }));
  LnLinearParams p{};
  p.T = T; p.m_tiles = ceil_div(T, LL_BM); p.nb = N / LL_C;
  p.ln_g = ln_g; p.ln_b = ln_b; p.eps = eps; p.bias = bias;
  cudaStream_t st = static_cast<cudaStream_t>(stream);
  const int grid = p.m_tiles < num_sms() ? p.m_tiles : num_sms();
  {
    char desc[64];
    if (prof_enabled()) snprintf(desc, sizeof(desc), "ln_linear M%d N%d K256", T, N);
    ProfScope ps(PGT_PROF_GEMM, 2.0 * (double)T * N * C, st, desc);
    ln_linear_kernel<<<grid, LL_THREADS, LL_SMEM, st>>>(tx, to, tw, p);
  }
  PGT_LAUNCH_OK();
  return PGT_OK;
}
```

pgtformer_b200/csrc/mha_tc.cu:

```cuda
#include <cudaTypedefs.h>

#include "common.cuh"
#include "tmap.cuh"
#include "ptx.cuh"

namespace pgt {

constexpr int FT_D = 64;
constexpr int FT_BM = 128;
constexpr int FT_BN = 128;
constexpr int FT_NST = 3;
constexpr int FT_TILE = FT_BN * FT_D * 2;
constexpr int FT_THREADS = 64 + 256;
constexpr int FT_SMEM = 2 * FT_TILE  + FT_NST * 2 * FT_TILE  + 2 * 2 * FT_TILE  + FT_TILE  + 256 + 1024;
constexpr float FT_TAU = 256.f;

__device__ __forceinline__ void tmem_st_32x32(uint32_t taddr, const uint32_t (&v)[32]) {
  asm volatile(
      "tcgen05.st.sync.aligned.32x32b.x32.b32 [%0], "
      "{%1, %2, %3, %4, %5, %6, %7, %8, %9, %10, %11, %12, %13, %14, %15, %16, "
      "%17, %18, %19, %20, %21, %22, %23, %24, %25, %26, %27, %28, %29, %30, %31, %32};"
      ::"r"(taddr), "r"(v[0]), "r"(v[1]), "r"(v[2]), "r"(v[3]), "r"(v[4]), "r"(v[5]), "r"(v[6]), "r"(v[7]), "r"(v[8]),
        "r"(v[9]), "r"(v[10]), "r"(v[11]), "r"(v[12]), "r"(v[13]), "r"(v[14]), "r"(v[15]), "r"(v[16]), "r"(v[17]),
        "r"(v[18]), "r"(v[19]), "r"(v[20]), "r"(v[21]), "r"(v[22]), "r"(v[23]), "r"(v[24]), "r"(v[25]), "r"(v[26]),
// ... 54 lines not shown
  uint64_t* kv_empty = kv_full + FT_NST;
  uint64_t* s_full = kv_empty + FT_NST;
  uint64_t* p_full = s_full + 2;
  uint64_t* o_full = p_full + 2;
  uint32_t* tmem_ptr = reinterpret_cast<uint32_t*>(o_full + 2);

  const int warp = threadIdx.x >> 5, lane = threadIdx.x & 31;
  const int h = blockIdx.y, clip = blockIdx.z;
  const int q0 = clip * L + blockIdx.x * 2 * FT_BM;
  const int kv0 = clip * L;
  const int NT = L / FT_BN;

  if (warp == 0 && lane == 0) {
    tma_prefetch_desc(&tmQ); tma_prefetch_desc(&tmK); tma_prefetch_desc(&tmV);
    mbar_init(q_full, 1);
    for (int i = 0; i < FT_NST; ++i) { mbar_init(&kv_full[i], 1); mbar_init(&kv_empty[i], 1); }
    for (int g = 0; g < 2; ++g) {
      mbar_init(&s_full[g], 1);
      mbar_init(&p_full[g], 128);
      mbar_init(&o_full[g], 1);
    }
    fence_barrier_init();
  }
  for (int i = threadIdx.x; i < FT_TILE / 16; i += FT_THREADS)
    reinterpret_cast<uint4*>(sOnes)[i] = make_uint4(0x3F803F80u, 0x3F803F80u, 0x3F803F80u, 0x3F803F80u);
  fence_proxy_async();
  if (warp == 1) {
    tmem_alloc<512>(tmem_ptr);
    tc_fence_before();
  }
  __syncthreads();
  tc_fence_after();
  const uint32_t tmem_base = *tmem_ptr;

  if (warp == 0) {
    if (elect_one()) {
      mbar_arrive_expect_tx(q_full, 2 * FT_TILE);
      tma_load_2d(sQ, &tmQ, q_full, h * FT_D, q0);
      tma_load_2d(sQ + FT_TILE, &tmQ, q_full, h * FT_D, q0 + FT_BM);
    }
    __syncwarp();
    int st = 0;
    uint32_t ph = 0;
    for (int j = 0; j < NT; ++j) {
      mbar_wait(&kv_empty[st], ph ^ 1);
      if (elect_one()) {
        mbar_arrive_expect_tx(&kv_full[st], 2 * FT_TILE);
        tma_load_2d(sK + st * FT_TILE, &tmK, &kv_full[st], h * FT_D, kv0 + j * FT_BN);
        tma_load_2d(sV + st * FT_TILE, &tmV, &kv_full[st], h * FT_D, kv0 + j * FT_BN);
      }
      __syncwarp();
      if (++st == FT_NST) { st = 0; ph ^= 1; }
    }
  } else if (warp == 1) {
    constexpr uint32_t idesc_s = umma_idesc_bf16(FT_BM, FT_BN);
    constexpr uint32_t idesc_o = umma_idesc_bf16(FT_BM, FT_D) | (1u << 16);
    auto issue_s = [&](int g, int st) {
      const uint64_t da = umma_desc_k_sw128(smem_u32(sQ + g * FT_TILE));
      const uint64_t db = umma_desc_k_sw128(smem_u32(sK + st * FT_TILE));
#pragma unroll
      for (int k = 0; k < FT_D / 16; ++k) umma_bf16_ss(tmem_base + g * FT_BN, da + 2 * k, db + 2 * k, idesc_s, k != 0 ? 1u : 0u);
      umma_commit(&s_full[g]);
    };
    constexpr uint32_t idesc_o80 = umma_idesc_bf16(FT_BM, FT_D + 16) | (1u << 16);
    auto issue_o = [&](int g, int st, uint32_t acc) {
#pragma unroll
// ... 132 lines not shown
        u.z = pack_bf16x2(__uint_as_float(v[8 * q + 4]) * inv, __uint_as_float(v[8 * q + 5]) * inv);
        u.w = pack_bf16x2(__uint_as_float(v[8 * q + 6]) * inv, __uint_as_float(v[8 * q + 7]) * inv);
        reinterpret_cast<uint4*>(orow)[(c >> 3) + q] = u;
      }
    }
  }

  tc_fence_before();
  __syncthreads();
  if (warp == 1) {
    tc_fence_after();
    tmem_dealloc<512>(tmem_base);
  }
}

static int encode_rows_map(CUtensorMap* map, const void* base, int ld, long long rows, int cols) {
  return tmap_rows_bf16(map, base, ld, rows, cols, FT_BN);
}

int mha_tc_launch(const void* q, int ldq, const void* k, int ldk, const void* v, int ldv, int clips, int L, int heads,
                  int d, void* out, int ldo, cudaStream_t stream) {
  if (d != FT_D || L % (2 * FT_BM) != 0) return PGT_ERR_UNSUPPORTED;
  auto al = [](const void* p) { return (reinterpret_cast<uintptr_t>(p) & 15) == 0; };
  if (!al(q) || !al(k) || !al(v) || !al(out) || ldq % 8 || ldk % 8 || ldv % 8 || ldo % 8) return PGT_ERR_UNSUPPORTED;
  CUtensorMap tq, tk, tv;
  const long long rows = (long long)clips * L;
  int rc = encode_rows_map(&tq, q, ldq, rows, heads * d);
  if (rc == PGT_OK) rc = encode_rows_map(&tk, k, ldk, rows, heads * d);
  if (rc == PGT_OK) rc = encode_rows_map(&tv, v, ldv, rows, heads * d);
  if (rc != PGT_OK) return rc;
  static PerDeviceOnce once;
  PGT_CUDA_OK(once.run([] { return cudaFuncSetAttribute(mha_tc_kernel, cudaFuncAttributeMaxDynamicSharedMemorySize, FT_SMEM); }));
  dim3 grid(L / (2 * FT_BM), heads, clips);
  mha_tc_kernel<<<grid, FT_THREADS, FT_SMEM, stream>>>(tq, tk, tv, L, reinterpret_cast<__nv_bfloat16*>(out), ldo);
  PGT_LAUNCH_OK();
  return PGT_OK;
}

}
```

pgtformer_b200/csrc/norm.cu:

```cuda
#include "common.cuh"

namespace pgt {

constexpr int GN_GROUPS = 32;
constexpr int GN_MAX_CHUNKS = 64;
constexpr int GN_THREADS = 512;

__device__ __forceinline__ void load8_bf16(const __nv_bfloat16* p, float (&v)[8]) {
  const uint4 u = __ldg(reinterpret_cast<const uint4*>(p));
  float2 a = unpack_bf16x2(u.x), b = unpack_bf16x2(u.y), c = unpack_bf16x2(u.z), d = unpack_bf16x2(u.w);
  v[0] = a.x; v[1] = a.y; v[2] = b.x; v[3] = b.y; v[4] = c.x; v[5] = c.y; v[6] = d.x; v[7] = d.y;
}
__device__ __forceinline__ void store8_bf16(__nv_bfloat16* p, const float (&v)[8]) {
  uint4 u;
  u.x = pack_bf16x2(v[0], v[1]); u.y = pack_bf16x2(v[2], v[3]);
  u.z = pack_bf16x2(v[4], v[5]); u.w = pack_bf16x2(v[6], v[7]);
  *reinterpret_cast<uint4*>(p) = u;
}

__global__ void __launch_bounds__(GN_THREADS)
gn_stats_kernel(const __nv_bfloat16* __restrict__ x, int ldx, int HW, int C, int pix_per_chunk,
                float* __restrict__ partial ) {
  extern __shared__ float sm[];
  const int vc = C >> 3;
  const int rows_par = GN_THREADS / vc;
  const int vcol = threadIdx.x % vc;
  const int prow = threadIdx.x / vc;
  const int chunk = blockIdx.x, f = blockIdx.y, nchunks = gridDim.x;
  const int p0 = chunk * pix_per_chunk;
  const int p1 = min(HW, p0 + pix_per_chunk);
  float s[8], q[8];
#pragma unroll
  for (int i = 0; i < 8; ++i) { s[i] = 0.f; q[i] = 0.f; }
  if (prow < rows_par) {
    const __nv_bfloat16* base = x + ((size_t)f * HW) * ldx + vcol * 8;
    int p = p0 + prow;
    for (; p + 3 * rows_par < p1; p += 4 * rows_par) {
      float v0[8], v1[8], v2[8], v3[8];
      load8_bf16(base + (size_t)p * ldx, v0);
      load8_bf16(base + (size_t)(p + rows_par) * ldx, v1);
      load8_bf16(base + (size_t)(p + 2 * rows_par) * ldx, v2);
      load8_bf16(base + (size_t)(p + 3 * rows_par) * ldx, v3);
#pragma unroll
      for (int i = 0; i < 8; ++i) {
        s[i] += (v0[i] + v1[i]) + (v2[i] + v3[i]);
        q[i] += (v0[i] * v0[i] + v1[i] * v1[i]) + (v2[i] * v2[i] + v3[i] * v3[i]);
      }
    }
    for (; p < p1; p += rows_par) {
      float v[8];
      load8_bf16(base + (size_t)p * ldx, v);
#pragma unroll
      for (int i = 0; i < 8; ++i) { s[i] += v[i]; q[i] += v[i] * v[i]; }
    }
#pragma unroll
    for (int i = 0; i < 8; ++i) {
      sm[(prow * 2 + 0) * C + vcol * 8 + i] = s[i];
      sm[(prow * 2 + 1) * C + vcol * 8 + i] = q[i];
    }
  }
  __syncthreads();
  for (int c = threadIdx.x; c < 2 * C; c += GN_THREADS) {
    const int which = c / C, ch = c % C;
    float t = 0.f;
    for (int rr = 0; rr < rows_par; ++rr) t += sm[(rr * 2 + which) * C + ch];
    sm[(size_t)rows_par * 2 * C + c] = t;
  }
  __syncthreads();
  if (threadIdx.x < GN_GROUPS) {
    const float* tot = sm + (size_t)rows_par * 2 * C;
    const int cpg = C / GN_GROUPS;
    float gs = 0.f, gq = 0.f;
    for (int c = threadIdx.x * cpg; c < (threadIdx.x + 1) * cpg; ++c) { gs += tot[c]; gq += tot[C + c]; }
    float* o = partial + (((size_t)f * nchunks + chunk) * GN_GROUPS + threadIdx.x) * 2;
    o[0] = gs; o[1] = gq;
  }
}

constexpr int GN_FIN_PARTS = 32;
__global__ void __launch_bounds__(GN_FIN_PARTS * 32)
gn_finalize_kernel(const float* __restrict__ partial, int nchunks, int HW, int C, const float* __restrict__ gamma,
                   const float* __restrict__ beta, float eps, float* __restrict__ ab ) {
  __shared__ float smean[GN_GROUPS], srstd[GN_GROUPS];
  __shared__ double ps[GN_FIN_PARTS][GN_GROUPS], pq[GN_FIN_PARTS][GN_GROUPS];
  const int f = blockIdx.x;
  const int cpg = C / GN_GROUPS;
  {
    const int g = threadIdx.x & 31, part = threadIdx.x >> 5;
    const float2* base = reinterpret_cast<const float2*>(partial) + (size_t)f * nchunks * GN_GROUPS + g;
    double s = 0.0, q = 0.0;
    int ch = part;
    for (; ch + 3 * GN_FIN_PARTS < nchunks; ch += 4 * GN_FIN_PARTS) {
      const float2 o0 = __ldg(base + (size_t)ch * GN_GROUPS);
      const float2 o1 = __ldg(base + (size_t)(ch + GN_FIN_PARTS) * GN_GROUPS);
      const float2 o2 = __ldg(base + (size_t)(ch + 2 * GN_FIN_PARTS) * GN_GROUPS);
      const float2 o3 = __ldg(base + (size_t)(ch + 3 * GN_FIN_PARTS) * GN_GROUPS);
      s += ((double)o0.x + (double)o1.x) + ((double)o2.x + (double)o3.x);
      q += ((double)o0.y + (double)o1.y) + ((double)o2.y + (double)o3.y);
    }
    for (; ch < nchunks; ch += GN_FIN_PARTS) {
      const float2 o = __ldg(base + (size_t)ch * GN_GROUPS);
      s += (double)o.x; q += (double)o.y;
    }
    ps[part][g] = s; pq[part][g] = q;
  }
  __syncthreads();
  if (threadIdx.x < GN_GROUPS) {
    double s = 0.0, q = 0.0;
    for (int part = 0; part < GN_FIN_PARTS; ++part) { s += ps[part][threadIdx.x]; q += pq[part][threadIdx.x]; }
    const double n = (double)HW * cpg;
    const double mean = s / n;
    double var = q / n - mean * mean;
    if (var < 0.0) var = 0.0;
    smean[threadIdx.x] = (float)mean;
    srstd[threadIdx.x] = (float)(1.0 / sqrt(var + (double)eps));
  }
  __syncthreads();
  for (int c = threadIdx.x; c < C; c += blockDim.x) {
    const int g = c / cpg;
    const float a = srstd[g] * gamma[c];
    ab[((size_t)f * 2 + 0) * C + c] = a;
    ab[((size_t)f * 2 + 1) * C + c] = beta[c] - smean[g] * a;
  }
}

constexpr int GN_APPLY_THREADS = 256;
__global__ void __launch_bounds__(GN_APPLY_THREADS, 3)
gn_apply_kernel(const __nv_bfloat16* __restrict__ x, int ldx, int HW, int C, int pix_per_block,
                const float* __restrict__ ab, int apply_silu, __nv_bfloat16* __restrict__ y, int ldy) {
  const int f = blockIdx.y;
  const int vc = C >> 3;
  const int rows_par = GN_APPLY_THREADS / vc;
  const int vcol = threadIdx.x % vc;
  const int prow = threadIdx.x / vc;
  if (prow >= rows_par) return;
  float a[8], b[8];
  {
    const float4* pa = reinterpret_cast<const float4*>(ab + ((size_t)f * 2 + 0) * C + vcol * 8);
    const float4* pb = reinterpret_cast<const float4*>(ab + ((size_t)f * 2 + 1) * C + vcol * 8);
    const float4 a0 = __ldg(pa), a1 = __ldg(pa + 1), b0 = __ldg(pb), b1 = __ldg(pb + 1);
    a[0] = a0.x; a[1] = a0.y; a[2] = a0.z; a[3] = a0.w; a[4] = a1.x; a[5] = a1.y; a[6] = a1.z; a[7] = a1.w;
    b[0] = b0.x; b[1] = b0.y; b[2] = b0.z; b[3] = b0.w; b[4] = b1.x; b[5] = b1.y; b[6] = b1.z; b[7] = b1.w;
  }
  const int p0 = blockIdx.x * pix_per_block;
  const int p1 = min(HW, p0 + pix_per_block);
  const __nv_bfloat16* xb = x + ((size_t)f * HW) * ldx + vcol * 8;
  __nv_bfloat16* yb = y + ((size_t)f * HW) * ldy + vcol * 8;
  if (apply_silu) {
#pragma unroll
    for (int j = 0; j < 8; ++j) { a[j] *= 0.5f; b[j] *= 0.5f; }
  }
  auto act = [&](float (&v)[8]) {
#pragma unroll
    for (int j = 0; j < 8; ++j) {
      const float h = fmaf(v[j], a[j], b[j]);
      float th;
      asm("tanh.approx.f32 %0, %1;" : "=f"(th) : "f"(h));
      v[j] = apply_silu ? fmaf(h, th, h) : h;
    }
  };
  int p = p0 + prow;
  for (; p + 3 * rows_par < p1; p += 4 * rows_par) {
    float v0[8], v1[8], v2[8], v3[8];
    load8_bf16(xb + (size_t)p * ldx, v0);
    load8_bf16(xb + (size_t)(p + rows_par) * ldx, v1);
    load8_bf16(xb + (size_t)(p + 2 * rows_par) * ldx, v2);
    load8_bf16(xb + (size_t)(p + 3 * rows_par) * ldx, v3);
    act(v0); act(v1); act(v2); act(v3);
    store8_bf16(yb + (size_t)p * ldy, v0);
    store8_bf16(yb + (size_t)(p + rows_par) * ldy, v1);
    store8_bf16(yb + (size_t)(p + 2 * rows_par) * ldy, v2);
    store8_bf16(yb + (size_t)(p + 3 * rows_par) * ldy, v3);
  }
  for (; p < p1; p += rows_par) {
    float v[8];
    load8_bf16(xb + (size_t)p * ldx, v);
    act(v);
    store8_bf16(yb + (size_t)p * ldy, v);
  }
}

constexpr int LN_ROWS = 4;
template <int NV, bool POS>
__global__ void __launch_bounds__(256)
layernorm_kernel(const void* __restrict__ xin, int ldx, int x_dtype, int T, const float* __restrict__ gamma,
                 const float* __restrict__ beta, float eps, __nv_bfloat16* __restrict__ y, int ldy,
                 const __nv_bfloat16* __restrict__ pos, int ldpos, __nv_bfloat16* __restrict__ y2, int ldy2) {
  constexpr int C = 256 * NV;
  const int warp = (blockIdx.x * blockDim.x + threadIdx.x) >> 5;
  const int lane = threadIdx.x & 31;
  const int row0 = warp * LN_ROWS;
  if (row0 >= T) return;
  float v[LN_ROWS][NV][8];
#pragma unroll
  for (int r = 0; r < LN_ROWS; ++r) {
    const int row = min(row0 + r, T - 1);
#pragma unroll
    for (int i = 0; i < NV; ++i) {
      const int c0 = (i * 32 + lane) * 8;
      if (x_dtype == PGT_BF16) {
        load8_bf16(reinterpret_cast<const __nv_bfloat16*>(xin) + (size_t)row * ldx + c0, v[r][i]);
      } else {
        const float4* p = reinterpret_cast<const float4*>(reinterpret_cast<const float*>(xin) + (size_t)row * ldx + c0);
        const float4 a = __ldg(p), b = __ldg(p + 1);
        v[r][i][0] = a.x; v[r][i][1] = a.y; v[r][i][2] = a.z; v[r][i][3] = a.w;
        v[r][i][4] = b.x; v[r][i][5] = b.y; v[r][i][6] = b.z; v[r][i][7] = b.w;
      }
    }
  }
  uint4 pr[POS ? LN_ROWS : 1][NV];
  if constexpr (POS) {
#pragma unroll
    for (int r = 0; r < LN_ROWS; ++r) {
      const int row = min(row0 + r, T - 1);
#pragma unroll
      for (int i = 0; i < NV; ++i)
        pr[r][i] = __ldg(reinterpret_cast<const uint4*>(pos + (size_t)row * ldpos + (i * 32 + lane) * 8));
    }
  }
  float g[NV][8], bt[NV][8];
// ... 17 lines not shown
    for (int o = 16; o > 0; o >>= 1) {
      s += __shfl_xor_sync(0xffffffffu, s, o);
      q += __shfl_xor_sync(0xffffffffu, q, o);
    }
    const float mean = s * (1.0f / C);
    const float rstd = rsqrtf(fmaxf(q * (1.0f / C) - mean * mean, 0.f) + eps);
    const float nm = -mean * rstd;
    if (row < T) {
#pragma unroll
      for (int i = 0; i < NV; ++i) {
        const int c0 = (i * 32 + lane) * 8;
        float o[8];
#pragma unroll
        for (int j = 0; j < 8; ++j) o[j] = fmaf(fmaf(v[r][i][j], rstd, nm), g[i][j], bt[i][j]);
        store8_bf16(y + (size_t)row * ldy + c0, o);
        if constexpr (POS) {
          const uint32_t pw[4] = {pr[r][i].x, pr[r][i].y, pr[r][i].z, pr[r][i].w};
#pragma unroll
          for (int j = 0; j < 4; ++j) {
            const float2 pv = unpack_bf16x2(pw[j]);
            o[2 * j] += pv.x; o[2 * j + 1] += pv.y;
          }
          store8_bf16(y2 + (size_t)row * ldy2 + c0, o);
        }
      }
    }
  }
}

constexpr int ADAIN_THREADS = 256;
__global__ void __launch_bounds__(ADAIN_THREADS)
adain_kernel(const void* __restrict__ qin, int ldq, int q_dtype, const __nv_bfloat16* __restrict__ l, int ldl, int HW,
             int C, float eps, __nv_bfloat16* __restrict__ y, int ldy) {
  __shared__ float red[4][ADAIN_THREADS / 8][64];
  __shared__ float sa[64], sb[64];
  const int f = blockIdx.y;
  const int cbase = blockIdx.x * 64;
  const int vcol = threadIdx.x & 7;
  const int prow = threadIdx.x >> 3;
  const int rows_par = ADAIN_THREADS / 8;
  const int c0 = cbase + vcol * 8;
  float acc[4][8];
#pragma unroll
  for (int k = 0; k < 4; ++k)
#pragma unroll
    for (int j = 0; j < 8; ++j) acc[k][j] = 0.f;
  auto load_q = [&](int p, float (&v)[8]) {
    if (q_dtype == PGT_BF16) {
      load8_bf16(reinterpret_cast<const __nv_bfloat16*>(qin) + ((size_t)f * HW + p) * ldq + c0, v);
    } else {
      const float4* pp = reinterpret_cast<const float4*>(reinterpret_cast<const float*>(qin) + ((size_t)f * HW + p) * ldq + c0);
      const float4 a = __ldg(pp), b = __ldg(pp + 1);
      v[0] = a.x; v[1] = a.y; v[2] = a.z; v[3] = a.w; v[4] = b.x; v[5] = b.y; v[6] = b.z; v[7] = b.w;
    }
  };
  for (int p = prow; p < HW; p += rows_par) {
    float vq[8], vl[8];
    load_q(p, vq);
    load8_bf16(l + ((size_t)f * HW + p) * ldl + c0, vl);
#pragma unroll
    for (int j = 0; j < 8; ++j) {
      acc[0][j] += vq[j]; acc[1][j] += vq[j] * vq[j];
      acc[2][j] += vl[j]; acc[3][j] += vl[j] * vl[j];
    }
  }
#pragma unroll
// ... 19 lines not shown
  __syncthreads();
  for (int p = prow; p < HW; p += rows_par) {
    float vq[8];
    load_q(p, vq);
#pragma unroll
    for (int j = 0; j < 8; ++j) vq[j] = vq[j] * sa[vcol * 8 + j] + sb[vcol * 8 + j];
    store8_bf16(y + ((size_t)f * HW + p) * ldy + c0, vq);
  }
}

}

using namespace pgt;

static int gn_chunks(int HW) {
  int c = ceil_div(HW, 1024);
  return c < 1 ? 1 : (c > GN_MAX_CHUNKS ? GN_MAX_CHUNKS : c);
}

extern "C" int64_t pgt_groupnorm_ws_floats(int F, int HW, int C) {
  return (int64_t)F * gn_chunks(HW) * GN_GROUPS * 2 + (int64_t)F * 2 * C;
}

extern "C" int pgt_groupnorm_silu(const void* x, int ldx, int F, int HW, int C, const float* gamma, const float* beta,
                                  float eps, int apply_silu, void* y, int ldy, float* ws, void* stream) {
  PGT_CHECK_ARG(x && y && ws && gamma && beta && F > 0 && HW > 0);
  PGT_CHECK_ARG(C % 32 == 0 && C % 8 == 0 && C / 8 <= GN_APPLY_THREADS && ldx % 8 == 0 && ldy % 8 == 0);
  cudaStream_t st = static_cast<cudaStream_t>(stream);
  ProfScope ps(PGT_PROF_NORM, 3.0 * F * (double)HW * C * 2, st);
  const int nchunks = gn_chunks(HW);
  const int ppc = ceil_div(HW, nchunks);
  float* ab = ws + (size_t)F * nchunks * GN_GROUPS * 2;
  const size_t stats_smem = ((size_t)(GN_THREADS / (C / 8)) + 1) * 2 * C * sizeof(float);
  gn_stats_kernel<<<dim3(nchunks, F), GN_THREADS, stats_smem, st>>>(
      reinterpret_cast<const __nv_bfloat16*>(x), ldx, HW, C, ppc, ws);
  PGT_LAUNCH_OK();
  gn_finalize_kernel<<<F, GN_FIN_PARTS * 32, 0, st>>>(ws, nchunks, HW, C, gamma, beta, eps, ab);
  PGT_LAUNCH_OK();
  int ppb = (131072 / (C * 2));
  if (ppb < 16) ppb = 16;
  const int nblk = ceil_div(HW, ppb);
  gn_apply_kernel<<<dim3(nblk, F), GN_APPLY_THREADS, 0, st>>>(
      reinterpret_cast<const __nv_bfloat16*>(x), ldx, HW, C, ppb, ab, apply_silu,
      reinterpret_cast<__nv_bfloat16*>(y), ldy);
  PGT_LAUNCH_OK();
  return PGT_OK;
}

extern "C" int pgt_groupnorm_apply_stats(const void* x, int ldx, int F, int HW, int C, const float* gamma,
                                         const float* beta, float eps, int apply_silu, void* y, int ldy,
                                         const float* stats, int chunks_per_frame, float* ws, void* stream) {
  PGT_CHECK_ARG(x && y && ws && gamma && beta && stats && F > 0 && HW > 0 && chunks_per_frame > 0);
  PGT_CHECK_ARG(C % 32 == 0 && C % 8 == 0 && C / 8 <= GN_APPLY_THREADS && ldx % 8 == 0 && ldy % 8 == 0);
  cudaStream_t st = static_cast<cudaStream_t>(stream);
  ProfScope ps(PGT_PROF_NORM, 2.0 * F * (double)HW * C * 2, st, "gn_apply_stats");
  gn_finalize_kernel<<<F, GN_FIN_PARTS * 32, 0, st>>>(stats, chunks_per_frame, HW, C, gamma, beta, eps, ws);
  PGT_LAUNCH_OK();
  int ppb = (131072 / (C * 2));
  if (ppb < 16) ppb = 16;
  gn_apply_kernel<<<dim3(ceil_div(HW, ppb), F), GN_APPLY_THREADS, 0, st>>>(
      reinterpret_cast<const __nv_bfloat16*>(x), ldx, HW, C, ppb, ws, apply_silu, reinterpret_cast<__nv_bfloat16*>(y), ldy);
  PGT_LAUNCH_OK();
  return PGT_OK;
}

extern "C" int pgt_groupnorm_ab(const void* x, int ldx, int F, int HW, int C, const float* gamma, const float* beta,
                                float eps, const float* stats, int chunks_per_frame, float* ws, float* ab, void* stream) {
  PGT_CHECK_ARG(gamma && beta && ab && F > 0 && HW > 0 && C % 32 == 0 && C / 8 <= GN_APPLY_THREADS);
  cudaStream_t st = static_cast<cudaStream_t>(stream);
  if (stats != nullptr) {
    PGT_CHECK_ARG(chunks_per_frame > 0);
    gn_finalize_kernel<<<F, GN_FIN_PARTS * 32, 0, st>>>(stats, chunks_per_frame, HW, C, gamma, beta, eps, ab);
    PGT_LAUNCH_OK();
    return PGT_OK;
  }
  PGT_CHECK_ARG(x && ws && ldx % 8 == 0);
  ProfScope ps(PGT_PROF_NORM, 1.0 * F * (double)HW * C * 2, st, "gn_stats");
  const int nchunks = gn_chunks(HW);
  const int ppc = ceil_div(HW, nchunks);
  const size_t stats_smem = ((size_t)(GN_THREADS / (C / 8)) + 1) * 2 * C * sizeof(float);
  gn_stats_kernel<<<dim3(nchunks, F), GN_THREADS, stats_smem, st>>>(reinterpret_cast<const __nv_bfloat16*>(x), ldx, HW, C, ppc, ws);
  PGT_LAUNCH_OK();
  gn_finalize_kernel<<<F, GN_FIN_PARTS * 32, 0, st>>>(ws, nchunks, HW, C, gamma, beta, eps, ab);
  PGT_LAUNCH_OK();
  return PGT_OK;
}

extern "C" int pgt_layernorm(const void* x, int ldx, int x_dtype, int T, int C, const float* gamma, const float* beta,
                             float eps, void* y, int ldy, const void* pos, int ldpos, void* y2, int ldy2,
                             void* stream) {
  PGT_CHECK_ARG(x && y && gamma && beta && T > 0);
  PGT_CHECK_ARG(C % 256 == 0 && C <= 1024 && ldx % 8 == 0 && ldy % 8 == 0);
  PGT_CHECK_ARG(y2 == nullptr || (pos != nullptr && ldpos % 8 == 0 && ldy2 % 8 == 0));
  cudaStream_t st = static_cast<cudaStream_t>(stream);
  ProfScope ps(7, (double)T * C * ((x_dtype == PGT_BF16 ? 2.0 : 4.0) + 2.0 + (y2 ? 4.0 : 0.0)), st, "layernorm");
  const int warps_per_block = 8;
  const int grid = ceil_div(T, warps_per_block * LN_ROWS);
  auto yb = reinterpret_cast<__nv_bfloat16*>(y);
  auto pb = reinterpret_cast<const __nv_bfloat16*>(pos);
  auto y2b = reinterpret_cast<__nv_bfloat16*>(y2);
#define PGT_LN_LAUNCH(NV_)                                                                                              \
  do {                                                                                                                \
    if (y2b != nullptr) layernorm_kernel<NV_, true><<<grid, 256, 0, st>>>(x, ldx, x_dtype, T, gamma, beta, eps, yb, ldy, pb, ldpos, y2b, ldy2); \
    else layernorm_kernel<NV_, false><<<grid, 256, 0, st>>>(x, ldx, x_dtype, T, gamma, beta, eps, yb, ldy, pb, ldpos, y2b, ldy2);           \
  } while (0)
  if (C == 256) PGT_LN_LAUNCH(1);
  else if (C == 512) PGT_LN_LAUNCH(2);
  else if (C == 768) PGT_LN_LAUNCH(3);
  else PGT_LN_LAUNCH(4);
#undef PGT_LN_LAUNCH
  PGT_LAUNCH_OK();
  return PGT_OK;
}

extern "C" int pgt_adain(const void* q, int ldq, int q_dtype, const void* l, int ldl, int F, int HW, int C, float eps,
                         void* y, int ldy, void* stream) {
  PGT_CHECK_ARG(q && l && y && F > 0 && HW > 1 && C % 64 == 0 && ldq % 8 == 0 && ldl % 8 == 0 && ldy % 8 == 0);
  ProfScope ps(PGT_PROF_MOVE, 8.0 * F * (double)HW * C, static_cast<cudaStream_t>(stream), "adain");
  adain_kernel<<<dim3(C / 64, F), ADAIN_THREADS, 0, static_cast<cudaStream_t>(stream)>>>(
      q, ldq, q_dtype, reinterpret_cast<const __nv_bfloat16*>(l), ldl, HW, C, eps,
      reinterpret_cast<__nv_bfloat16*>(y), ldy);
  PGT_LAUNCH_OK();
  return PGT_OK;
}
```

pgtformer_b200/csrc/parsing.cu:

```cuda
#include <float.h>

#include "common.cuh"

namespace pgt {

__device__ __forceinline__ void ld8(const __nv_bfloat16* p, float (&v)[8]) {
  const uint4 u = __ldg(reinterpret_cast<const uint4*>(p));
  float2 a = unpack_bf16x2(u.x), b = unpack_bf16x2(u.y), c = unpack_bf16x2(u.z), d = unpack_bf16x2(u.w);
  v[0] = a.x; v[1] = a.y; v[2] = b.x; v[3] = b.y; v[4] = c.x; v[5] = c.y; v[6] = d.x; v[7] = d.y;
}
__device__ __forceinline__ void st8(__nv_bfloat16* p, const float (&v)[8]) {
  uint4 u;
  u.x = pack_bf16x2(v[0], v[1]); u.y = pack_bf16x2(v[2], v[3]);
  u.z = pack_bf16x2(v[4], v[5]); u.w = pack_bf16x2(v[6], v[7]);
  *reinterpret_cast<uint4*>(p) = u;
}

__global__ void maxpool3x3s2_kernel(const __nv_bfloat16* __restrict__ x, int ldx, int F, int H, int W, int C,
                                    __nv_bfloat16* __restrict__ y, int ldy) {
  const int Ho = H >> 1, Wo = W >> 1, vc = C >> 3;
  const size_t total = (size_t)F * Ho * Wo * vc;
  for (size_t i = (size_t)blockIdx.x * blockDim.x + threadIdx.x; i < total; i += (size_t)gridDim.x * blockDim.x) {
    const int v = (int)(i % vc);
    size_t pix = i / vc;
    const int ox = (int)(pix % Wo); pix /= Wo;
    const int oy = (int)(pix % Ho);
    const int f = (int)(pix / Ho);
    float m[8];
#pragma unroll
    for (int j = 0; j < 8; ++j) m[j] = -FLT_MAX;
#pragma unroll
    for (int dy = 0; dy < 3; ++dy) {
      const int iy = 2 * oy - 1 + dy;
      if (iy < 0 || iy >= H) continue;
#pragma unroll
      for (int dx = 0; dx < 3; ++dx) {
        const int ix = 2 * ox - 1 + dx;
        if (ix < 0 || ix >= W) continue;
        float t[8];
        ld8(x + (((size_t)f * H + iy) * W + ix) * ldx + v * 8, t);
#pragma unroll
        for (int j = 0; j < 8; ++j) m[j] = fmaxf(m[j], t[j]);
      }
    }
    st8(y + (((size_t)f * Ho + oy) * Wo + ox) * ldy + v * 8, m);
  }
}

__global__ void __launch_bounds__(256)
global_avgpool_kernel(const __nv_bfloat16* __restrict__ x, int ldx, int HW, int C, __nv_bfloat16* __restrict__ y, int ldy) {
  __shared__ float red[32][64];
  const int f = blockIdx.y, cbase = blockIdx.x * 64;
  const int vcol = threadIdx.x & 7, prow = threadIdx.x >> 3;
  const int c0 = cbase + vcol * 8;
  float acc[8];
#pragma unroll
  for (int j = 0; j < 8; ++j) acc[j] = 0.f;
  if (c0 < C) {
    for (int p = prow; p < HW; p += 32) {
      float v[8];
      ld8(x + ((size_t)f * HW + p) * ldx + c0, v);
#pragma unroll
      for (int j = 0; j < 8; ++j) acc[j] += v[j];
    }
  }
#pragma unroll
  for (int j = 0; j < 8; ++j) red[prow][vcol * 8 + j] = acc[j];
  __syncthreads();
  if (threadIdx.x < 64 && cbase + threadIdx.x < C) {
    float s = 0.f;
    for (int r = 0; r < 32; ++r) s += red[r][threadIdx.x];
    y[(size_t)f * ldy + cbase + threadIdx.x] = __float2bfloat16_rn(s / (float)HW);
  }
}

__global__ void channel_affine_kernel(const __nv_bfloat16* __restrict__ x, int ldx, int F, int HW, int C,
                                      const __nv_bfloat16* __restrict__ scale, int lds, int plus_one,
                                      const __nv_bfloat16* __restrict__ addv, int ldv,
                                      const __nv_bfloat16* __restrict__ addm, int ldm, __nv_bfloat16* __restrict__ y, int ldy) {
  const int vc = C >> 3;
  const size_t total = (size_t)F * HW * vc;
  for (size_t i = (size_t)blockIdx.x * blockDim.x + threadIdx.x; i < total; i += (size_t)gridDim.x * blockDim.x) {
    const int v = (int)(i % vc);
    const size_t pix = i / vc;
    const int f = (int)(pix / HW);
    float a[8], s[8];
    ld8(x + pix * ldx + v * 8, a);
    ld8(scale + (size_t)f * lds + v * 8, s);
#pragma unroll
    for (int j = 0; j < 8; ++j) a[j] *= (plus_one ? s[j] + 1.f : s[j]);
    if (addv != nullptr) {
      float t[8];
      ld8(addv + (size_t)f * ldv + v * 8, t);
#pragma unroll
      for (int j = 0; j < 8; ++j) a[j] += t[j];
    }
    if (addm != nullptr) {
      float t[8];
      ld8(addm + pix * ldm + v * 8, t);
#pragma unroll
      for (int j = 0; j < 8; ++j) a[j] += t[j];
    }
    st8(y + pix * ldy + v * 8, a);
  }
}

__global__ void assemble_cond_kernel(const __nv_bfloat16* __restrict__ o0, int ld0, const __nv_bfloat16* __restrict__ o1,
                                     int ld1, const __nv_bfloat16* __restrict__ o2, int ld2, int F, int h8, int w8, int h16,
                                     int w16, int ncls, __nv_bfloat16* __restrict__ cond, int ldc) {
  const size_t total = (size_t)F * h16 * w16 * 64;
  const float sy = h16 > 1 ? (float)(h8 - 1) / (float)(h16 - 1) : 0.f;
  const float sx = w16 > 1 ? (float)(w8 - 1) / (float)(w16 - 1) : 0.f;
  for (size_t i = (size_t)blockIdx.x * blockDim.x + threadIdx.x; i < total; i += (size_t)gridDim.x * blockDim.x) {
    const int c = (int)(i & 63);
    size_t pix = i >> 6;
    const int x = (int)(pix % w16); pix /= w16;
    const int y = (int)(pix % h16);
    const int f = (int)(pix / h16);
    float v = 0.f;
    if (c < 2 * ncls) {
      const __nv_bfloat16* src = c < ncls ? o0 : o1;
      const int ld = c < ncls ? ld0 : ld1;
      const int ch = c < ncls ? c : c - ncls;
      const float fy = y * sy, fx = x * sx;
      const int y0 = (int)fy, x0 = (int)fx;
      const int y1 = min(y0 + 1, h8 - 1), x1 = min(x0 + 1, w8 - 1);
      const float ly = fy - y0, lx = fx - x0;
      auto at = [&](int yy, int xx) { return __bfloat162float(src[(((size_t)f * h8 + yy) * w8 + xx) * ld + ch]); };
      v = (1.f - ly) * ((1.f - lx) * at(y0, x0) + lx * at(y0, x1)) + ly * ((1.f - lx) * at(y1, x0) + lx * at(y1, x1));
    } else if (c < 3 * ncls) {
      v = __bfloat162float(o2[(((size_t)f * h16 + y) * w16 + x) * ld2 + (c - 2 * ncls)]);
    }
    cond[(((size_t)f * h16 + y) * w16 + x) * ldc + c] = __float2bfloat16_rn(v);
  }
}

}

using namespace pgt;

static int grid_for(size_t total, int threads) {
  size_t b = (total + threads - 1) / threads;
  const size_t cap = (size_t)num_sms() * 32;
  return (int)(b < cap ? (b ? b : 1) : cap);
}

extern "C" int pgt_maxpool3x3s2(const void* x, int ldx, int F, int H, int W, int C, void* y, int ldy, void* stream) {
  PGT_CHECK_ARG(x && y && F > 0 && (H % 2) == 0 && (W % 2) == 0 && C % 8 == 0 && ldx % 8 == 0 && ldy % 8 == 0);
  const size_t total = (size_t)F * (H / 2) * (W / 2) * (C / 8);
  cudaStream_t st = static_cast<cudaStream_t>(stream);
  ProfScope ps(PGT_PROF_MOVE, 2.5 * F * (double)H * W * C, st, "maxpool");
  maxpool3x3s2_kernel<<<grid_for(total, 256), 256, 0, st>>>(reinterpret_cast<const __nv_bfloat16*>(x), ldx, F, H, W, C,
                                                           reinterpret_cast<__nv_bfloat16*>(y), ldy);
  PGT_LAUNCH_OK();
  return PGT_OK;
}

extern "C" int pgt_global_avgpool(const void* x, int ldx, int F, int HW, int C, void* y, int ldy, void* stream) {
  PGT_CHECK_ARG(x && y && F > 0 && HW > 0 && C % 8 == 0 && ldx % 8 == 0 && ldy >= C);
  cudaStream_t st = static_cast<cudaStream_t>(stream);
  ProfScope ps(PGT_PROF_MOVE, 2.0 * F * (double)HW * C, st, "avgpool");
  global_avgpool_kernel<<<dim3(ceil_div(C, 64), F), 256, 0, st>>>(reinterpret_cast<const __nv_bfloat16*>(x), ldx, HW, C,
                                                                 reinterpret_cast<__nv_bfloat16*>(y), ldy);
  PGT_LAUNCH_OK();
  return PGT_OK;
}

extern "C" int pgt_channel_affine(const void* x, int ldx, int F, int HW, int C, const void* scale, int lds, int plus_one,
                                  const void* addv, int ldv, const void* addm, int ldm, void* y, int ldy, void* stream) {
  PGT_CHECK_ARG(x && y && scale && F > 0 && HW > 0 && C % 8 == 0 && ldx % 8 == 0 && ldy % 8 == 0 && lds % 8 == 0);
  PGT_CHECK_ARG((addv == nullptr || ldv % 8 == 0) && (addm == nullptr || ldm % 8 == 0));
  const size_t total = (size_t)F * HW * (C / 8);
  cudaStream_t st = static_cast<cudaStream_t>(stream);
  ProfScope ps(PGT_PROF_MOVE, (addm ? 6.0 : 4.0) * F * (double)HW * C, st, "channel_affine");
  channel_affine_kernel<<<grid_for(total, 256), 256, 0, st>>>(
      reinterpret_cast<const __nv_bfloat16*>(x), ldx, F, HW, C, reinterpret_cast<const __nv_bfloat16*>(scale), lds, plus_one,
      reinterpret_cast<const __nv_bfloat16*>(addv), ldv, reinterpret_cast<const __nv_bfloat16*>(addm), ldm,
      reinterpret_cast<__nv_bfloat16*>(y), ldy);
  PGT_LAUNCH_OK();
  return PGT_OK;
}

extern "C" int pgt_assemble_cond(const void* o0, int ld0, const void* o1, int ld1, const void* o2, int ld2, int F, int h8,
                                 int w8, int h16, int w16, int ncls, void* cond, int ldc, void* stream) {
  PGT_CHECK_ARG(o0 && o1 && o2 && cond && F > 0 && h8 > 0 && w8 > 0 && h16 > 0 && w16 > 0 && ncls > 0 && 3 * ncls <= 64 &&
                ldc >= 64);
  const size_t total = (size_t)F * h16 * w16 * 64;
  cudaStream_t st = static_cast<cudaStream_t>(stream);
  ProfScope ps(PGT_PROF_MOVE, 4.0 * (double)total, st, "assemble_cond");
  assemble_cond_kernel<<<grid_for(total, 256), 256, 0, st>>>(
      reinterpret_cast<const __nv_bfloat16*>(o0), ld0, reinterpret_cast<const __nv_bfloat16*>(o1), ld1,
      reinterpret_cast<const __nv_bfloat16*>(o2), ld2, F, h8, w8, h16, w16, ncls, reinterpret_cast<__nv_bfloat16*>(cond), ldc);
  PGT_LAUNCH_OK();
  return PGT_OK;
}
```

pgtformer_b200/csrc/rgb_conv.cu:

```cuda
#include <cudaTypedefs.h>

#include "common.cuh"
#include "tmap.cuh"
#include "ptx.cuh"
#include "epi_common.cuh"

namespace pgt {

constexpr int RC_N = 64;
constexpr int RC_SUB = 128 * 128;
constexpr int RC_BSUB = RC_N * 128;

struct RgbConvParams {
  const float* x;
  int H, W, Ho, Wo;
  long long M;
  int m_tiles;
  float mean[3], istd[3];
  const float* bias;
  int relu;
  float* gn_stats;
};

template <int KS>
// ... 44 lines not shown
  extern __shared__ __align__(1024) uint8_t smem[];
  if ((smem_u32(smem) & 1023u) != 0) __trap();
  uint8_t* sA = smem;
  uint8_t* sB = sA + 2 * Cfg::A_BYTES;
  uint8_t* sO = sB + Cfg::B_BYTES;
  uint64_t* bars = reinterpret_cast<uint64_t*>(sO + 2 * RC_SUB);
  uint64_t* a_full = bars;
  uint64_t* a_free = bars + 2;
  uint64_t* acc_full = bars + 4;
  uint64_t* acc_free = bars + 6;
  uint64_t* b_full = bars + 8;
  uint32_t* tmem_ptr = reinterpret_cast<uint32_t*>(bars + 9);

  const int warp = threadIdx.x >> 5, lane = threadIdx.x & 31;
  constexpr int BW = Cfg::BW;
  if (warp == BW + 4) {
    if (lane == 0) {
      tma_prefetch_desc(&tmW); tma_prefetch_desc(&tmO);
      for (int i = 0; i < 2; ++i) {
        mbar_init(&a_full[i], BW * 32); mbar_init(&a_free[i], 1); mbar_init(&acc_full[i], 1); mbar_init(&acc_free[i], 128);
      }
      mbar_init(b_full, 1);
      fence_barrier_init();
      mbar_arrive_expect_tx(b_full, Cfg::B_BYTES);
      for (int s = 0; s < Cfg::NSUB; ++s) tma_load_2d(sB + s * RC_BSUB, &tmW, b_full, s * 64, 0);
    }
    __syncwarp();
    tmem_alloc<128>(tmem_ptr);
    tc_fence_before();
  }
  __syncthreads();
  tc_fence_after();
  const uint32_t tmem_base = *tmem_ptr;

  if (warp < BW) {
    const int r = threadIdx.x & 127;
    const int part = threadIdx.x >> 7;
    constexpr int CH_PER = (Cfg::NCH + Cfg::PARTS - 1) / Cfg::PARTS;
    const size_t plane = (size_t)p.H * p.W;
    const int HoWo = p.Ho * p.Wo;
    int it = 0;
    for (int tile = blockIdx.x; tile < p.m_tiles; tile += gridDim.x, ++it) {
      const int buf = it & 1;
      const long long row = (long long)tile * 128 + r;
      const bool valid = row < p.M;
      const int f = valid ? (int)(row / HoWo) : 0;
      const int rem = valid ? (int)(row - (long long)f * HoWo) : 0;
      const int oy = rem / p.Wo, ox = rem - oy * p.Wo;
      const int iy0 = oy * STRIDE - PAD, ix0 = ox * STRIDE - PAD;
      const float* x0 = p.x + (size_t)f * 3 * plane + (long long)iy0 * p.W + ix0;
      mbar_wait(&a_free[buf], ((it >> 1) & 1) ^ 1);
      uint8_t* arow = sA + buf * Cfg::A_BYTES + r * 128;
      if (part == 0) rgb_build_chunks<KS, 0, CH_PER < Cfg::NCH ? CH_PER : Cfg::NCH>(p, x0, plane, iy0, ix0, valid, arow, r);
      else rgb_build_chunks<KS, CH_PER < Cfg::NCH ? CH_PER : Cfg::NCH, Cfg::NCH>(p, x0, plane, iy0, ix0, valid, arow, r);
      fence_proxy_async();
      mbar_arrive(&a_full[buf]);
    }
  } else if (warp < BW + 4) {
    const int quad = warp & 3;
    const int r = quad * 32 + lane;
    const int et = threadIdx.x - BW * 32;
    int it = 0;
    for (int tile = blockIdx.x; tile < p.m_tiles; tile += gridDim.x, ++it) {
      const int buf = it & 1;
      mbar_wait(&acc_full[buf], (it >> 1) & 1);
      tc_fence_after();
// ... 61 lines not shown
        }
        umma_commit(&a_free[buf]);
        umma_commit(&acc_full[buf]);
      }
      __syncwarp();
    }
  }

  tc_fence_before();
  __syncthreads();
  if (warp == BW + 4) {
    tc_fence_after();
    tmem_dealloc<128>(tmem_base);
  }
}

static int rc_enc2d(CUtensorMap* map, const void* base, long long ld, long long rows, int cols, int box_rows) {
  return tmap_rows_bf16(map, base, ld, rows, cols, box_rows);
}

template <int KS, int STRIDE, int PAD>
static int launch_rgb(const CUtensorMap& tw, const CUtensorMap& to, const RgbConvParams& p, cudaStream_t st, const char* desc) {
  using Cfg = RgbCfg<KS>;
  static PerDeviceOnce once;
  PGT_CUDA_OK(once.run([] {
    cudaError_t e = cudaFuncSetAttribute(rgb_conv_kernel<KS, STRIDE, PAD>, cudaFuncAttributeMaxDynamicSharedMemorySize, Cfg::SMEM);
    if (e != cudaSuccess) return e;
    return cudaFuncSetAttribute(rgb_conv_kernel<KS, STRIDE, PAD>, cudaFuncAttributePreferredSharedMemoryCarveout,
                                cudaSharedmemCarveoutMaxShared);
  }));
  const int grid = p.m_tiles < num_sms() * Cfg::PER_SM ? p.m_tiles : num_sms() * Cfg::PER_SM;
  {
    ProfScope ps(PGT_PROF_GEMM, 2.0 * (double)p.M * RC_N * Cfg::K, st, desc);
    rgb_conv_kernel<KS, STRIDE, PAD><<<grid, Cfg::THREADS, Cfg::SMEM, st>>>(tw, to, p);
  }
  PGT_LAUNCH_OK();
  return PGT_OK;
}

}

using namespace pgt;

extern "C" int pgt_conv_rgb_bf16(const float* x_nchw, int F, int H, int W, int ksize, int stride, int pad,
                                 const float* mean3, const float* std3, const void* Wp, int ldw, int Cout,
                                 const float* bias, int act, void* out, int ldo, float* gn_stats, void* stream) {
  PGT_CHECK_ARG(x_nchw && Wp && bias && out && F > 0 && H > 0 && W > 0);
  if (Cout != RC_N || !((ksize == 3 && stride == 1 && pad == 1) || (ksize == 7 && stride == 2 && pad == 3)))
    return PGT_ERR_UNSUPPORTED;
  PGT_CHECK_ARG(act == PGT_ACT_NONE || act == PGT_ACT_RELU);
  auto al = [](const void* q) { return (reinterpret_cast<uintptr_t>(q) & 15) == 0; };
  PGT_CHECK_ARG(al(Wp) && al(out) && ldw % 8 == 0 && ldo % 8 == 0 && ldw >= 3 * ksize * ksize && ldo >= Cout);
  RgbConvParams p{};
  p.x = x_nchw; p.H = H; p.W = W;
  p.Ho = (H + 2 * pad - ksize) / stride + 1;
  p.Wo = (W + 2 * pad - ksize) / stride + 1;
  PGT_CHECK_ARG(p.Ho > 0 && p.Wo > 0);
  p.M = (long long)F * p.Ho * p.Wo;
  p.m_tiles = (int)((p.M + 127) / 128);
  for (int c = 0; c < 3; ++c) {
    p.mean[c] = mean3 ? mean3[c] : 0.f;
    p.istd[c] = std3 ? 1.f / std3[c] : 1.f;
  }
  p.bias = bias; p.relu = act == PGT_ACT_RELU; p.gn_stats = gn_stats;
  if (gn_stats != nullptr && (p.Ho * p.Wo) % 128 != 0) return PGT_ERR_UNSUPPORTED;
  CUtensorMap tw, to;
  int rc = rc_enc2d(&tw, Wp, ldw, Cout, 3 * ksize * ksize, RC_N);
  if (rc == PGT_OK) rc = rc_enc2d(&to, out, ldo, p.M, Cout, 128);
  if (rc != PGT_OK) return rc;
// ... 4 lines not shown
```

pgtformer_b200/csrc/swin_mlp.cu:

```cuda
#include <cudaTypedefs.h>

#include "common.cuh"
#include "tmap.cuh"
#include "ptx.cuh"
#include "epi_common.cuh"

namespace pgt {

constexpr int SM_C = 256;
constexpr int SM_BM = 128;
constexpr int SM_SUB = SM_BM * 128;
constexpr int SM_WST = 3;
constexpr int SM_WBYTES = SM_C * 128;
constexpr int SM_THREADS = 640;
constexpr int SM_SMEM = 2 * 4 * SM_SUB  + SM_WST * SM_WBYTES + 2 * 128 * 8  + 256;

struct SwinMlpParams {
  int T, m_tiles;
  const float* ln_g;
  const float* ln_b;
  float eps;
  const float* b1;
  const float* b2;
  float* gn_stats;
// ... 133 lines not shown

__global__ void __launch_bounds__(SM_THREADS, 1)
swin_mlp_kernel(const __grid_constant__ CUtensorMap tmX, const __grid_constant__ CUtensorMap tmO,
                const __grid_constant__ CUtensorMap tmW1, const __grid_constant__ CUtensorMap tmW2,
                const SwinMlpParams p) {
  extern __shared__ __align__(1024) uint8_t smem[];
  if ((smem_u32(smem) & 1023u) != 0) __trap();
  uint8_t* sW = smem + 2 * 4 * SM_SUB;
  float2* xch = reinterpret_cast<float2*>(sW + SM_WST * SM_WBYTES);
  SmGroupBars* gbar = reinterpret_cast<SmGroupBars*>(xch + 256);
  uint64_t* w_full = reinterpret_cast<uint64_t*>(gbar + 2);
  uint64_t* w_empty = w_full + SM_WST;
  uint32_t* tmem_ptr = reinterpret_cast<uint32_t*>(w_empty + SM_WST);

  const int warp = threadIdx.x >> 5, lane = threadIdx.x & 31;
  if (warp == 0 && lane == 0) {
    tma_prefetch_desc(&tmX); tma_prefetch_desc(&tmO); tma_prefetch_desc(&tmW1); tma_prefetch_desc(&tmW2);
    for (int g = 0; g < 2; ++g) {
      mbar_init(&gbar[g].x_full, 1); mbar_init(&gbar[g].res_full, 1);
      mbar_init(&gbar[g].y_ready, 256); mbar_init(&gbar[g].acc1_full, 1);
      mbar_init(&gbar[g].h_ready, 256); mbar_init(&gbar[g].acc2_full, 1);
      mbar_init(&gbar[g].out_ready, 256);
    }
    for (int i = 0; i < SM_WST; ++i) { mbar_init(&w_full[i], 1); mbar_init(&w_empty[i], 1); }
    fence_barrier_init();
  }
  if (warp == 1) {
    tmem_alloc<512>(tmem_ptr);
    tc_fence_before();
  }
  __syncthreads();
  tc_fence_after();
  const uint32_t tmem_base = *tmem_ptr;

  const int n_loc = (int)blockIdx.x < p.m_tiles ? (p.m_tiles - 1 - (int)blockIdx.x) / (int)gridDim.x + 1 : 0;
  const int n_grp[2] = {(n_loc + 1) >> 1, n_loc >> 1};

  auto for_each_gemm = [&](auto&& fn) {
    for (int it = 0; it < n_grp[0]; ++it) {
      if (it >= 1 && it - 1 < n_grp[1]) fn(1, 1, it - 1);
      fn(0, 0, it);
      fn(1, 0, it);
      if (it < n_grp[1]) fn(0, 1, it);
    }
    if (n_grp[1] >= 1 && n_grp[1] == n_grp[0]) fn(1, 1, n_grp[1] - 1);
  };

  if (warp == 0) {
    int st = 0;
    uint32_t ph = 0;
    for_each_gemm([&](int gemm, int , int ) {
      for (int kb = 0; kb < 4; ++kb) {
        mbar_wait(&w_empty[st], ph ^ 1);
        if (elect_one()) {
          mbar_arrive_expect_tx(&w_full[st], SM_WBYTES);
          tma_load_2d(sW + st * SM_WBYTES, gemm == 0 ? &tmW1 : &tmW2, &w_full[st], kb * 64, 0);
        }
        __syncwarp();
        if (++st == SM_WST) { st = 0; ph ^= 1; }
      }
    });
  } else if (warp == 1) {
    constexpr uint32_t idesc = umma_idesc_bf16(SM_BM, SM_C);
    int st = 0;
    uint32_t ph = 0;
    for_each_gemm([&](int gemm, int g, int it) {
// ... 56 lines not shown
  }
}

static int enc2d(CUtensorMap* map, const void* base, int ld, long long rows, int cols, int box_rows) {
  return tmap_rows_bf16(map, base, ld, rows, cols, box_rows);
}

}

using namespace pgt;

extern "C" int pgt_swin_mlp_bf16(const void* x, int ldx, int T, int C, const float* ln_g, const float* ln_b, float eps,
                                 const void* W1, const float* b1, const void* W2, const float* b2, void* out, int ldo,
                                 float* gn_stats, void* stream) {
  PGT_CHECK_ARG(x && out && W1 && W2 && b1 && b2 && T > 0 && ((ln_g == nullptr) == (ln_b == nullptr)));
  if (C != SM_C) return PGT_ERR_UNSUPPORTED;
  auto al = [](const void* q) { return (reinterpret_cast<uintptr_t>(q) & 15) == 0; };
  PGT_CHECK_ARG(al(x) && al(out) && al(W1) && al(W2) && ldx % 8 == 0 && ldo % 8 == 0);
  CUtensorMap tx, to, t1, t2;
  int rc = enc2d(&tx, x, ldx, T, C, SM_BM);
  if (rc == PGT_OK) rc = enc2d(&to, out, ldo, T, C, SM_BM);
  if (rc == PGT_OK) rc = enc2d(&t1, W1, C, C, C, SM_C);
  if (rc == PGT_OK) rc = enc2d(&t2, W2, C, C, C, SM_C);
  if (rc != PGT_OK) return rc;
  static PerDeviceOnce once;
  PGT_CUDA_OK(once.run([] { return cudaFuncSetAttribute(swin_mlp_kernel, cudaFuncAttributeMaxDynamicSharedMemorySize, SM_SMEM); }));
  SwinMlpParams p{};
  p.T = T; p.m_tiles = ceil_div(T, SM_BM);
  p.ln_g = ln_g; p.ln_b = ln_b; p.eps = eps; p.b1 = b1; p.b2 = b2; p.gn_stats = gn_stats;
  cudaStream_t st = static_cast<cudaStream_t>(stream);
  const int grid = p.m_tiles < num_sms() ? p.m_tiles : num_sms();
  {
    ProfScope ps(PGT_PROF_GEMM, 4.0 * (double)T * C * C, st, "swin_mlp_fused C256");
    swin_mlp_kernel<<<grid, SM_THREADS, SM_SMEM, st>>>(tx, to, t1, t2, p);
  }
  PGT_LAUNCH_OK();
  return PGT_OK;
}
```

pgtformer_b200/csrc/window3d.cu:

```cuda
#include "common.cuh"
#include "tmap.cuh"

namespace pgt {

__device__ __forceinline__ void w3_mma_16816(float (&c)[4], const uint32_t (&a)[4], uint32_t b0, uint32_t b1) {
  asm volatile(
      "mma.sync.aligned.m16n8k16.row.col.f32.bf16.bf16.f32 {%0,%1,%2,%3}, {%4,%5,%6,%7}, {%8,%9}, {%0,%1,%2,%3};"
      : "+f"(c[0]), "+f"(c[1]), "+f"(c[2]), "+f"(c[3])
      : "r"(a[0]), "r"(a[1]), "r"(a[2]), "r"(a[3]), "r"(b0), "r"(b1));
}
__device__ __forceinline__ void w3_ldmatrix_x2_trans(uint32_t& r0, uint32_t& r1, const void* smem_row_ptr) {
  const uint32_t a = static_cast<uint32_t>(__cvta_generic_to_shared(smem_row_ptr));
  asm volatile("ldmatrix.sync.aligned.m8n8.x2.trans.shared.b16 {%0,%1}, [%2];" : "=r"(r0), "=r"(r1) : "r"(a));
}

struct Win3dParams {
  const __nv_bfloat16* qkv;
  int ldqkv;
  const __nv_bfloat16* pad_qkv;
  const float* bias;
  __nv_bfloat16* out;
  int ldo;
  int B, D, H, W, C, heads;
  int wd, wh, ww, sd, sh, sw;
  int Dp, Hp, Wp, nd, nh, nw;
  int N, NP;
};

constexpr int W3_MAXNP = 128;

template <int HD>
__global__ void __launch_bounds__(256)
window3d_attn_kernel(const Win3dParams p) {
  constexpr int LDS = HD + 8;
  extern __shared__ __align__(16) unsigned char smem_raw[];
  __nv_bfloat16* qs = reinterpret_cast<__nv_bfloat16*>(smem_raw);
  __nv_bfloat16* ks = qs + W3_MAXNP * LDS;
  __nv_bfloat16* vs = ks + W3_MAXNP * LDS;
  __shared__ int tok[W3_MAXNP];
  __shared__ int lab[W3_MAXNP];
  const int win = blockIdx.x, h = blockIdx.y;
  const int per_b = p.nd * p.nh * p.nw;
  const int b = win / per_b;
  int r = win - b * per_b;
  const int wz = r / (p.nh * p.nw);
  r -= wz * p.nh * p.nw;
  const int wy = r / p.nw, wx = r - wy * p.nw;
  const bool shifted = (p.sd | p.sh | p.sw) != 0;
  if (threadIdx.x < p.NP) {
    const int i = threadIdx.x;
    int t = -1, l = 0;
    if (i < p.N) {
      const int id = i / (p.wh * p.ww), ih = (i / p.ww) % p.wh, iw = i % p.ww;
      const int pd = wz * p.wd + id, ph = wy * p.wh + ih, pw = wx * p.ww + iw;
      const int d = (pd + p.sd) % p.Dp, y = (ph + p.sh) % p.Hp, x = (pw + p.sw) % p.Wp;
      if (d < p.D && y < p.H && x < p.W) t = ((b * p.D + d) * p.H + y) * p.W + x;
      const int rd = p.sd == 0 ? 2 : (pd < p.Dp - p.wd ? 0 : (pd < p.Dp - p.sd ? 1 : 2));
      const int rh = p.sh == 0 ? 2 : (ph < p.Hp - p.wh ? 0 : (ph < p.Hp - p.sh ? 1 : 2));
      const int rw = p.sw == 0 ? 2 : (pw < p.Wp - p.ww ? 0 : (pw < p.Wp - p.sw ? 1 : 2));
      l = rd * 9 + rh * 3 + rw;
    }
    tok[i] = t;
    lab[i] = l;
  }
  __syncthreads();
  {
// ... 109 lines not shown
      for (int nt = 0; nt < HD / 8; ++nt) *reinterpret_cast<uint32_t*>(dst + nt * 8 + 2 * t4) = pack_bf16x2(o[nt][2], o[nt][3]);
    }
  }
}

}

using namespace pgt;

extern "C" int pgt_window3d_attention(const void* qkv, int ldqkv, const void* pad_qkv, int B, int D, int H, int W, int C,
                                      int heads, int wd, int wh, int ww, int sd, int sh, int sw, const float* bias,
                                      void* out, int ldo, void* stream) {
  PGT_CHECK_ARG(qkv && bias && out && B > 0 && D > 0 && H > 0 && W > 0 && heads > 0 && C % heads == 0);
  PGT_CHECK_ARG(wd > 0 && wh > 0 && ww > 0 && sd >= 0 && sh >= 0 && sw >= 0 && ldqkv % 8 == 0 && ldo % 8 == 0 && ldqkv >= 3 * C);
  if (D <= wd) { wd = D; sd = 0; }
  if (H <= wh) { wh = H; sh = 0; }
  if (W <= ww) { ww = W; sw = 0; }
  const int N = wd * wh * ww, hd = C / heads;
  if (N > W3_MAXNP || (hd != 16 && hd != 32 && hd != 64)) return PGT_ERR_UNSUPPORTED;
  PGT_CHECK_ARG(sd < wd && sh < wh && sw < ww);
  Win3dParams p{};
  p.qkv = reinterpret_cast<const __nv_bfloat16*>(qkv); p.ldqkv = ldqkv;
  p.pad_qkv = reinterpret_cast<const __nv_bfloat16*>(pad_qkv);
  p.bias = bias; p.out = reinterpret_cast<__nv_bfloat16*>(out); p.ldo = ldo;
  p.B = B; p.D = D; p.H = H; p.W = W; p.C = C; p.heads = heads;
  p.wd = wd; p.wh = wh; p.ww = ww; p.sd = sd; p.sh = sh; p.sw = sw;
  p.nd = ceil_div(D, wd); p.nh = ceil_div(H, wh); p.nw = ceil_div(W, ww);
  p.Dp = p.nd * wd; p.Hp = p.nh * wh; p.Wp = p.nw * ww;
  p.N = N; p.NP = (N + 15) / 16 * 16;
  cudaStream_t st = static_cast<cudaStream_t>(stream);
  dim3 grid(B * p.nd * p.nh * p.nw, heads);
  const size_t smem = (size_t)3 * W3_MAXNP * (hd + 8) * 2;
  ProfScope ps(PGT_PROF_WINDOW_ATTN, 4.0 * N * N * C * (double)grid.x, st, "window3d");
  if (hd == 16) window3d_attn_kernel<16><<<grid, 256, smem, st>>>(p);
  else if (hd == 32) window3d_attn_kernel<32><<<grid, 256, smem, st>>>(p);
  else {
    static PerDeviceOnce once;
    PGT_CUDA_OK(once.run([] { return cudaFuncSetAttribute(window3d_attn_kernel<64>, cudaFuncAttributeMaxDynamicSharedMemorySize,
                                                          3 * W3_MAXNP * (64 + 8) * 2); }));
    window3d_attn_kernel<64><<<grid, 256, smem, st>>>(p);
  }
  PGT_LAUNCH_OK();
  return PGT_OK;
}
```

pgtformer_b200/csrc/window_attn_tc.cu:

```cuda
#include <cuda_fp16.h>

#include "common.cuh"
#include "ptx.cuh"
#include "tmap.cuh"

namespace pgt {

constexpr int WT_N = 48;
constexpr int WT_TILE = 2 * WT_N * 128;
constexpr int WT_STAGE = 3 * WT_TILE;
constexpr int WT_NST = 4;
constexpr int WT_PTILE = 128 * 128;
constexpr int WT_THREADS = 64 + 256;
constexpr int WT_HEADS = 8;
constexpr int WT_TAB_BYTES = WT_HEADS * 6 * WT_N * 16;
constexpr int WT_SMEM = 2048  + WT_NST * WT_STAGE + 2 * WT_PTILE + WT_TAB_BYTES + 512  + 1024 ;

struct WinParams {
  int clips, H, W, C, heads, d, shift;
  int nwx, nwy, n_windows, n_pairs, n_chunks, hpc;
  int ldo;
  __nv_bfloat16* out;
  float sl2;
  const uint4* tab;
// ... 63 lines not shown
  uint8_t* sP = ring + WT_NST * WT_STAGE;
  uint8_t* sTab = sP + 2 * WT_PTILE;
  uint64_t* bars = reinterpret_cast<uint64_t*>(sTab + WT_TAB_BYTES);
  uint64_t* st_full = bars;
  uint64_t* st_empty = st_full + WT_NST;
  uint64_t* s_full = st_empty + WT_NST;
  uint64_t* p_full = s_full + 4;
  uint64_t* o_full = p_full + 2;
  uint64_t* o_empty = o_full + 2;
  uint32_t* tmem_ptr = reinterpret_cast<uint32_t*>(o_empty + 2);

  const int warp = threadIdx.x >> 5, lane = threadIdx.x & 31;
  const CUtensorMap* tmI[4] = {&tmI0, &tmI1, &tmI2, &tmI3};

  if (warp == 0 && lane == 0) {
    for (int i = 0; i < 4; ++i) tma_prefetch_desc(tmI[i]);
    for (int i = 0; i < WT_NST; ++i) { mbar_init(&st_full[i], 1); mbar_init(&st_empty[i], 1); }
    for (int i = 0; i < 4; ++i) mbar_init(&s_full[i], 1);
    for (int g = 0; g < 2; ++g) {
      mbar_init(&p_full[g], 128);
      mbar_init(&o_full[g], 1);
      mbar_init(&o_empty[g], 128);
    }
    fence_barrier_init();
  }
  if (warp == 1) {
    tmem_alloc<512>(tmem_ptr);
    tc_fence_before();
  }
  for (int i = threadIdx.x; i < WT_TAB_BYTES / 16; i += WT_THREADS) reinterpret_cast<uint4*>(sTab)[i] = __ldg(p.tab + i);
  __syncthreads();
  tc_fence_after();
  const uint32_t tmem_base = *tmem_ptr;

  const int my_pairs = (p.n_pairs - (int)blockIdx.x + (int)gridDim.x - 1) / (int)gridDim.x;
  const int NCH = p.n_chunks;
  const int items = my_pairs * (NCH / 2) * HPC;

  if (warp == 0) {
    int st = 0;
    uint32_t ph = 0;
    for (int i = 0; i < my_pairs; ++i) {
      const int pair = blockIdx.x + i * gridDim.x;
      const int nwin = (2 * pair + 1 < p.n_windows) ? 2 : 1;
      WinCoord wc[2];
      wc[0] = win_coord(p, 2 * pair);
      wc[1] = win_coord(p, nwin == 2 ? 2 * pair + 1 : 2 * pair);
      for (int c = 0; c < NCH; ++c) {
        mbar_wait(&st_empty[st], ph ^ 1);
        if (elect_one()) {
          uint8_t* sK = ring + st * WT_STAGE;
          uint8_t* sV = sK + WT_TILE;
          uint8_t* sQ = sV + WT_TILE;
          mbar_arrive_expect_tx(&st_full[st], nwin * 3 * WT_N * 128);
          for (int wi = 0; wi < nwin; ++wi) {
            const int nx = wc[wi].xs ? 2 : 1, ny = wc[wi].ys ? 2 : 1;
            const CUtensorMap* m = tmI[wc[wi].ys * 2 + wc[wi].xs];
            const int part_bytes = (WT_N / (nx * ny)) * 128;
            int off = wi * WT_N * 128;
            for (int py = 0; py < ny; ++py) {
              const int y = wc[wi].ys ? (py == 0 ? p.H - 2 : 0) : wc[wi].y0;
              for (int px = 0; px < nx; ++px) {
                const int x = wc[wi].xs ? (px == 0 ? p.W - 2 : 0) : wc[wi].x0;
                tma_load_5d(sK + off, m, &st_full[st], p.C + c * 64, x, y, 0, wc[wi].clip);
                tma_load_5d(sQ + off, m, &st_full[st], c * 64, x, y, 0, wc[wi].clip);
                tma_load_5d(sV + off, m, &st_full[st], 2 * p.C + c * 64, x, y, 0, wc[wi].clip);
// ... 216 lines not shown
extern "C" int pgt_window_attention_tc(const void* qkv, int ldqkv, int clips, int H, int W, int C, int heads, int shift,
                                       const void* tab, void* out, int ldo, int mode_n64, void* stream) {
  (void)mode_n64;
  PGT_CHECK_ARG(qkv && tab && out && clips > 0 && H > 0 && W > 0 && heads > 0);
  PGT_CHECK_ARG(H % 4 == 0 && W % 4 == 0 && C % heads == 0 && ldqkv % 8 == 0 && ldo % 8 == 0 && ldqkv >= 3 * C);
  if (H <= 4 || W <= 4) shift = 0;
  const int d = C / heads;
  if ((d != 32 && d != 64) || heads != WT_HEADS || C % 128 != 0 || (shift != 0 && shift != 2)) return PGT_ERR_UNSUPPORTED;
  auto al = [](const void* q) { return (reinterpret_cast<uintptr_t>(q) & 15) == 0; };
  if (!al(qkv) || !al(out) || !al(tab)) return PGT_ERR_UNSUPPORTED;
  cudaStream_t st = static_cast<cudaStream_t>(stream);
  CUtensorMap mi[4];
  for (int t = 0; t < 4; ++t) {
    const int bx = (t & 1) ? 2 : 4, by = (t & 2) ? 2 : 4;
    const int rc = win_map(&mi[t], qkv, ldqkv, 3 * C, clips, H, W, bx, by);
    if (rc != PGT_OK) return rc;
  }
  WinParams p{};
  p.clips = clips; p.H = H; p.W = W; p.C = C; p.heads = heads; p.d = d; p.shift = shift;
  p.nwx = W / 4; p.nwy = H / 4;
  p.n_windows = clips * p.nwx * p.nwy;
  p.n_pairs = (p.n_windows + 1) / 2;
  p.n_chunks = C / 64;
  p.hpc = 64 / d;
  p.ldo = ldo;
  p.out = reinterpret_cast<__nv_bfloat16*>(out);
  p.sl2 = (1.0f / sqrtf((float)d)) * 1.4426950408889634f;
  p.tab = reinterpret_cast<const uint4*>(tab);
  const int grid = p.n_pairs < num_sms() ? p.n_pairs : num_sms();
  ProfScope ps(PGT_PROF_WINDOW_ATTN, 4.0 * WT_N * WT_N * C * (double)p.n_windows, st, "window_attn_tc");
  if (d == 32) {
    static PerDeviceOnce once;
    PGT_CUDA_OK(once.run([] { return cudaFuncSetAttribute(window_attn_tc_kernel<32>, cudaFuncAttributeMaxDynamicSharedMemorySize, WT_SMEM); }));
    window_attn_tc_kernel<32><<<grid, WT_THREADS, WT_SMEM, st>>>(mi[0], mi[1], mi[2], mi[3], p);
  } else {
    static PerDeviceOnce once;
    PGT_CUDA_OK(once.run([] { return cudaFuncSetAttribute(window_attn_tc_kernel<64>, cudaFuncAttributeMaxDynamicSharedMemorySize, WT_SMEM); }));
    window_attn_tc_kernel<64><<<grid, WT_THREADS, WT_SMEM, st>>>(mi[0], mi[1], mi[2], mi[3], p);
  }
  PGT_LAUNCH_OK();
  return PGT_OK;
}
```

Baseline: 184.0.

## Enable programmatic dependent launch across all kernels with griddepcontrol waits

Routes every kernel launch through cudaLaunchKernelEx with the programmatic stream serialization attribute, and adds griddepcontrol.wait in each kernel. Heavy tcgen05 kernels wait only after their barrier, TMEM and table setup. The GEMM kernel also issues weight-tile prefetches before waiting, so that setup overlaps the previous kernel's tail. This targets launch latency and prologue gaps between the many small back-to-back kernels. The risk is a race if any kernel touches producer outputs before its wait, or if weights are not truly independent of the prior kernel.

```diff
diff --git a/pgtformer_b200/csrc/attention.cu b/pgtformer_b200/csrc/attention.cu
--- a/pgtformer_b200/csrc/attention.cu
+++ b/pgtformer_b200/csrc/attention.cu
@@ -29,6 +29,7 @@
 __global__ void __launch_bounds__(256)
 window_attn_kernel(const __nv_bfloat16* __restrict__ qkv, int ldqkv, int H, int W, int C, int heads, int shift,
                    const float* __restrict__ bias_tab, __nv_bfloat16* __restrict__ out, int ldo) {
+  pdl_wait();
   extern __shared__ __align__(16) unsigned char smem_raw[];
   __shared__ int tok[WIN_N];
   __shared__ int lab[WIN_N];
@@ -164,6 +165,7 @@
 __global__ void __launch_bounds__(128)
 mha_fwd_kernel(const __nv_bfloat16* __restrict__ q, int ldq, const __nv_bfloat16* __restrict__ k, int ldk,
                const __nv_bfloat16* __restrict__ v, int ldv, int L, int heads, __nv_bfloat16* __restrict__ out, int ldo) {
+  pdl_wait();
   constexpr int LDS = D + 8;
   extern __shared__ __align__(16) unsigned char smem_raw[];
   __nv_bfloat16* ks = reinterpret_cast<__nv_bfloat16*>(smem_raw);
@@ -306,7 +308,7 @@
       PGT_CUDA_OK(cudaFuncSetAttribute(window_attn_kernel<32>, cudaFuncAttributeMaxDynamicSharedMemorySize, (int)smem));
       attr32 = true;
     }
-    window_attn_kernel<32><<<grid, 256, smem, st>>>(reinterpret_cast<const __nv_bfloat16*>(qkv), ldqkv, H, W, C, heads,
+    PGT_LAUNCH((window_attn_kernel<32>), dim3(grid), dim3(256), smem, st, reinterpret_cast<const __nv_bfloat16*>(qkv), ldqkv, H, W, C, heads,
                                                     shift, bias_tab, reinterpret_cast<__nv_bfloat16*>(out), ldo);
   } else if (d == 64) {
     static bool attr = false;
@@ -314,12 +316,11 @@
       PGT_CUDA_OK(cudaFuncSetAttribute(window_attn_kernel<64>, cudaFuncAttributeMaxDynamicSharedMemorySize, (int)smem));
       attr = true;
     }
-    window_attn_kernel<64><<<grid, 256, smem, st>>>(reinterpret_cast<const __nv_bfloat16*>(qkv), ldqkv, H, W, C, heads,
+    PGT_LAUNCH((window_attn_kernel<64>), dim3(grid), dim3(256), smem, st, reinterpret_cast<const __nv_bfloat16*>(qkv), ldqkv, H, W, C, heads,
                                                     shift, bias_tab, reinterpret_cast<__nv_bfloat16*>(out), ldo);
   } else {
     return PGT_ERR_UNSUPPORTED;
   }
-  PGT_LAUNCH_OK();
   return PGT_OK;
 }
 
@@ -337,9 +338,8 @@
   dim3 grid(ceil_div(L, FA_BM), heads, clips);
   const size_t smem = (size_t)4 * FA_BN * (64 + 8) * 2;
   ProfScope ps(PGT_PROF_MHA, 4.0 * (double)L * L * d * heads * clips, static_cast<cudaStream_t>(stream));
-  mha_fwd_kernel<64><<<grid, 128, smem, static_cast<cudaStream_t>(stream)>>>(
+  PGT_LAUNCH((mha_fwd_kernel<64>), dim3(grid), dim3(128), smem, static_cast<cudaStream_t>(stream),
       reinterpret_cast<const __nv_bfloat16*>(q), ldq, reinterpret_cast<const __nv_bfloat16*>(k), ldk,
       reinterpret_cast<const __nv_bfloat16*>(v), ldv, L, heads, reinterpret_cast<__nv_bfloat16*>(out), ldo);
-  PGT_LAUNCH_OK();
   return PGT_OK;
 }
diff --git a/pgtformer_b200/csrc/codebook.cu b/pgtformer_b200/csrc/codebook.cu
--- a/pgtformer_b200/csrc/codebook.cu
+++ b/pgtformer_b200/csrc/codebook.cu
@@ -8,6 +8,7 @@
 argmax_gather_kernel(const float* __restrict__ logits, int T, int K, const float* __restrict__ codebook, int E,
                      const int64_t* __restrict__ idx_in, int64_t* __restrict__ idx_out, void* __restrict__ quant,
                      int ldq, int quant_dtype) {
+  pdl_wait();
   const int row = (blockIdx.x * blockDim.x + threadIdx.x) >> 5;
   const int lane = threadIdx.x & 31;
   if (row >= T) return;
@@ -69,6 +70,7 @@
 l2_argmin_kernel(const float* __restrict__ z, int T, int E, const float* __restrict__ cb, int K,
                  int64_t* __restrict__ idx, float* __restrict__ quant, const int* __restrict__ list,
                  const int* __restrict__ count, int min_count) {
+  pdl_wait();
   __shared__ __align__(16) float xs[AM_KC][AM_LD];
   __shared__ __align__(16) float es[AM_KC][AM_LD];
   __shared__ CandD merge[AM_TT][16];
@@ -163,6 +165,7 @@
 l2_argmin_short_list_kernel(const float* __restrict__ z, int E, const float* __restrict__ cb, int K,
                             int64_t* __restrict__ idx, float* __restrict__ quant, const int* __restrict__ list,
                             const int* __restrict__ count, int max_count) {
+  pdl_wait();
   const int n_tok = *count;
   if (n_tok > max_count) return;
   const int lane = threadIdx.x & 31;
@@ -197,10 +200,8 @@
 int l2_argmin_list_launch(const float* z, int T, int E, const float* codebook, int K, int64_t* idx, float* quant,
                           const int* list, const int* count, int grid, cudaStream_t st) {
   if (E % AM_KC != 0 || E % 4 != 0) return PGT_ERR_UNSUPPORTED;
-  l2_argmin_short_list_kernel<<<num_sms(), 256, 0, st>>>(z, E, codebook, K, idx, quant, list, count, AM_SHORT_LIST);
-  PGT_LAUNCH_OK();
-  l2_argmin_kernel<<<grid, 256, 0, st>>>(z, T, E, codebook, K, idx, quant, list, count, AM_SHORT_LIST);
-  PGT_LAUNCH_OK();
+  PGT_LAUNCH(l2_argmin_short_list_kernel, dim3(num_sms()), dim3(256), 0, st, z, E, codebook, K, idx, quant, list, count, AM_SHORT_LIST);
+  PGT_LAUNCH(l2_argmin_kernel, dim3(grid), dim3(256), 0, st, z, T, E, codebook, K, idx, quant, list, count, AM_SHORT_LIST);
   return PGT_OK;
 }
 
@@ -217,9 +218,8 @@
   const int warps = 8;
   ProfScope ps(PGT_PROF_ARGMAX, (double)T * K * 4 + (double)T * 8 + (quant ? (double)T * E * (quant_dtype == PGT_BF16 ? 2 : 4) : 0.0),
                static_cast<cudaStream_t>(stream));
-  argmax_gather_kernel<<<ceil_div(T, warps), warps * 32, 0, static_cast<cudaStream_t>(stream)>>>(
+  PGT_LAUNCH(argmax_gather_kernel, dim3(ceil_div(T, warps)), dim3(warps * 32), 0, static_cast<cudaStream_t>(stream),
       logits, T, K, codebook, E, idx_in, idx, quant, ldq, quant_dtype);
-  PGT_LAUNCH_OK();
   return PGT_OK;
 }
 
@@ -228,7 +228,6 @@
   PGT_CHECK_ARG(z && codebook && idx && T > 0 && K > 0 && E > 0 && E % AM_KC == 0);
   PGT_CHECK_ARG((reinterpret_cast<uintptr_t>(z) & 15) == 0 && (reinterpret_cast<uintptr_t>(codebook) & 15) == 0);
   ProfScope ps(PGT_PROF_ARGMIN, 2.0 * T * (double)K * E, static_cast<cudaStream_t>(stream));
-  l2_argmin_kernel<<<ceil_div(T, AM_TT), 256, 0, static_cast<cudaStream_t>(stream)>>>(z, T, E, codebook, K, idx, quant, nullptr, nullptr, 0);
-  PGT_LAUNCH_OK();
+  PGT_LAUNCH(l2_argmin_kernel, dim3(ceil_div(T, AM_TT)), dim3(256), 0, static_cast<cudaStream_t>(stream), z, T, E, codebook, K, idx, quant, nullptr, nullptr, 0);
   return PGT_OK;
 }
diff --git a/pgtformer_b200/csrc/common.cuh b/pgtformer_b200/csrc/common.cuh
--- a/pgtformer_b200/csrc/common.cuh
+++ b/pgtformer_b200/csrc/common.cuh
@@ -2,6 +2,8 @@
 #include <cuda_bf16.h>
 #include <cuda_runtime.h>
 #include <stdint.h>
+
+#include <utility>
 
 #include "../../include/pgt_b200.h"
 
@@ -43,7 +45,43 @@
     ::pgt::count_launch();                        \
   } while (0)
 
+template <typename... KArgs, typename... Args>
+static inline cudaError_t launch_pdl(void (*kernel)(KArgs...), dim3 grid, dim3 block, size_t smem, cudaStream_t st,
+                                     int cluster_x, Args&&... args) {
+  cudaLaunchAttribute attr[2];
+  attr[0].id = cudaLaunchAttributeProgrammaticStreamSerialization;
+  attr[0].val.programmaticStreamSerializationAllowed = 1;
+  cudaLaunchConfig_t cfg = {};
+  cfg.gridDim = grid;
+  cfg.blockDim = block;
+  cfg.dynamicSmemBytes = smem;
+  cfg.stream = st;
+  cfg.attrs = attr;
+  cfg.numAttrs = 1;
+  if (cluster_x > 1) {
+    attr[1].id = cudaLaunchAttributeClusterDimension;
+    attr[1].val.clusterDim.x = cluster_x;
+    attr[1].val.clusterDim.y = 1;
+    attr[1].val.clusterDim.z = 1;
+    cfg.numAttrs = 2;
+  }
+  return cudaLaunchKernelEx(&cfg, kernel, std::forward<Args>(args)...);
+}
+
+#define PGT_LAUNCH(kernel, grid, block, smem, st, ...)                                           \
+  do {                                                                                          \
+    cudaError_t _le = ::pgt::launch_pdl(kernel, grid, block, smem, st, 1, __VA_ARGS__);         \
+    if (_le != cudaSuccess) {                                                                   \
+      ::pgt::set_cuda_error(_le, "kernel launch");                                              \
+      return PGT_ERR_CUDA;                                                                      \
+    }                                                                                           \
+    PGT_LAUNCH_OK();                                                                            \
+  } while (0)
+
 static inline int ceil_div(int a, int b) { return (a + b - 1) / b; }
+
+__device__ __forceinline__ void pdl_wait() { asm volatile("griddepcontrol.wait;" ::: "memory"); }
+__device__ __forceinline__ void pdl_launch_dependents() { asm volatile("griddepcontrol.launch_dependents;" ::: "memory"); }
 
 __device__ __forceinline__ float rcp_approx(float x) {
   float r;
diff --git a/pgtformer_b200/csrc/conv_out.cu b/pgtformer_b200/csrc/conv_out.cu
--- a/pgtformer_b200/csrc/conv_out.cu
+++ b/pgtformer_b200/csrc/conv_out.cu
@@ -91,6 +91,7 @@
   __syncthreads();
   tc_fence_after();
   const uint32_t tmem_base = *tmem_ptr;
+  pdl_wait();
   const int per_frame = p.tiles_x * p.tiles_y;
 
   if (warp == 0) {
@@ -226,7 +227,6 @@
   char desc[64];
   snprintf(desc, sizeof(desc), "conv_out_gn F%d H%d W%d N%d", F, H, W, Cout);
   ProfScope ps(PGT_PROF_GEMM, 2.0 * F * (double)H * W * Cout * 9 * Cin, st, desc);
-  conv_out_gn_kernel<<<grid, CO_THREADS, CO_SMEM, st>>>(p);
-  PGT_LAUNCH_OK();
+  PGT_LAUNCH(conv_out_gn_kernel, dim3(grid), dim3(CO_THREADS), CO_SMEM, st, p);
   return PGT_OK;
 }
diff --git a/pgtformer_b200/csrc/elementwise.cu b/pgtformer_b200/csrc/elementwise.cu
--- a/pgtformer_b200/csrc/elementwise.cu
+++ b/pgtformer_b200/csrc/elementwise.cu
@@ -7,6 +7,7 @@
 
 __global__ void copy2d_kernel(const __nv_bfloat16* __restrict__ x, int ldx, size_t T, int C,
                               __nv_bfloat16* __restrict__ y, int ldy) {
+  pdl_wait();
   const int vc = C >> 3;
   const size_t total = T * vc;
   const size_t stride = (size_t)gridDim.x * blockDim.x;
@@ -30,6 +31,7 @@
 
 __global__ void nchw_to_nhwc_kernel(const float* __restrict__ x, int C, int HW, const float* __restrict__ mean,
                                     const float* __restrict__ stdv, __nv_bfloat16* __restrict__ y, int ldy) {
+  pdl_wait();
   __shared__ float tile[32][33];
   const int f = blockIdx.z;
   const int p0 = blockIdx.x * 32, c0 = blockIdx.y * 32;
@@ -53,6 +55,7 @@
 
 __global__ void nhwc_to_f32_kernel(const __nv_bfloat16* __restrict__ x, int ldx, int HW, int C, float* __restrict__ y,
                                    int to_nchw) {
+  pdl_wait();
   __shared__ float tile[32][33];
   const int f = blockIdx.z;
   const int p0 = blockIdx.x * 32, c0 = blockIdx.y * 32;
@@ -88,9 +91,8 @@
   PGT_CHECK_ARG(x && y && T > 0 && C % 8 == 0 && ldx % 8 == 0 && ldy % 8 == 0);
   ProfScope ps(PGT_PROF_MOVE, 2.0 * (double)T * C * 2, static_cast<cudaStream_t>(stream), "pgt_copy2d");
   const size_t total = (size_t)T * (C / 8);
-  copy2d_kernel<<<ew_grid(total, 256), 256, 0, static_cast<cudaStream_t>(stream)>>>(
+  PGT_LAUNCH(copy2d_kernel, dim3(ew_grid(total, 256)), dim3(256), 0, static_cast<cudaStream_t>(stream),
       reinterpret_cast<const __nv_bfloat16*>(x), ldx, (size_t)T, C, reinterpret_cast<__nv_bfloat16*>(y), ldy);
-  PGT_LAUNCH_OK();
   return PGT_OK;
 }
 
@@ -99,9 +101,8 @@
   PGT_CHECK_ARG(x && y && F > 0 && C > 0 && HW > 0 && ldy >= C && (mean == nullptr) == (stdv == nullptr));
   ProfScope ps(PGT_PROF_MOVE, 6.0 * F * (double)C * HW, static_cast<cudaStream_t>(stream), "pgt_nchw_f32_to_nhwc_bf16");
   dim3 grid(ceil_div(HW, 32), ceil_div(C, 32), F);
-  nchw_to_nhwc_kernel<<<grid, dim3(32, 8), 0, static_cast<cudaStream_t>(stream)>>>(
+  PGT_LAUNCH(nchw_to_nhwc_kernel, dim3(grid), dim3(32, 8), 0, static_cast<cudaStream_t>(stream),
       x, C, HW, mean, stdv, reinterpret_cast<__nv_bfloat16*>(y), ldy);
-  PGT_LAUNCH_OK();
   return PGT_OK;
 }
 
@@ -109,15 +110,15 @@
   PGT_CHECK_ARG(x && y && F > 0 && C > 0 && HW > 0 && ldx >= C);
   ProfScope ps(PGT_PROF_MOVE, 6.0 * F * (double)C * HW, static_cast<cudaStream_t>(stream), "pgt_nhwc_bf16_to_f32");
   dim3 grid(ceil_div(HW, 32), ceil_div(C, 32), F);
-  nhwc_to_f32_kernel<<<grid, dim3(32, 8), 0, static_cast<cudaStream_t>(stream)>>>(
+  PGT_LAUNCH(nhwc_to_f32_kernel, dim3(grid), dim3(32, 8), 0, static_cast<cudaStream_t>(stream),
       reinterpret_cast<const __nv_bfloat16*>(x), ldx, HW, C, y, to_nchw);
-  PGT_LAUNCH_OK();
   return PGT_OK;
 }
 
 namespace pgt {
 __global__ void regroup_frames_kernel(const __nv_bfloat16* __restrict__ x, int ldx, int b, int P, int C,
                                       __nv_bfloat16* __restrict__ y, int ldy, int dir) {
+  pdl_wait();
   const int vc = C >> 3;
   const size_t total = (size_t)b * 3 * P * vc;
   for (size_t i = (size_t)blockIdx.x * blockDim.x + threadIdx.x; i < total; i += (size_t)gridDim.x * blockDim.x) {
@@ -141,9 +142,8 @@
   PGT_CHECK_ARG(x && y && clips > 0 && P > 0 && C % 8 == 0 && ldx % 8 == 0 && ldy % 8 == 0 && (dir == 0 || dir == 1));
   ProfScope ps(PGT_PROF_MOVE, 4.0 * clips * 3.0 * P * C, static_cast<cudaStream_t>(stream), "pgt_regroup_frames");
   const size_t total = (size_t)clips * 3 * P * (C / 8);
-  regroup_frames_kernel<<<ew_grid(total, 256), 256, 0, static_cast<cudaStream_t>(stream)>>>(
+  PGT_LAUNCH(regroup_frames_kernel, dim3(ew_grid(total, 256)), dim3(256), 0, static_cast<cudaStream_t>(stream),
       reinterpret_cast<const __nv_bfloat16*>(x), ldx, clips, P, C, reinterpret_cast<__nv_bfloat16*>(y), ldy, dir);
-  PGT_LAUNCH_OK();
   return PGT_OK;
 }
 
@@ -152,6 +152,7 @@
 __constant__ float c_u8_to_unit[256];
 
 __global__ void u8hwc_to_f32nchw_kernel(const uint8_t* __restrict__ x, size_t HW, size_t total, float* __restrict__ y) {
+  pdl_wait();
   for (size_t i = (size_t)blockIdx.x * blockDim.x + threadIdx.x; i < total; i += (size_t)gridDim.x * blockDim.x) {
     const size_t f = i / HW, p = i - f * HW;
     const uint8_t* s = x + (f * HW + p) * 3;
@@ -164,6 +165,7 @@
 
 __global__ void f32nchw_to_u8hwc_kernel(const float* __restrict__ x, size_t HW, int first, int step, size_t total,
                                         uint8_t* __restrict__ y) {
+  pdl_wait();
   for (size_t i = (size_t)blockIdx.x * blockDim.x + threadIdx.x; i < total; i += (size_t)gridDim.x * blockDim.x) {
     const size_t j = i / HW, p = i - j * HW;
     const float* s = x + ((size_t)first + j * step) * 3 * HW + p;
@@ -178,6 +180,7 @@
 
 __global__ void gather_frames_kernel(const uint4* __restrict__ x, size_t vec_per_frame, const int* __restrict__ idx,
                                      uint4* __restrict__ y) {
+  pdl_wait();
   const uint4* s = x + (size_t)idx[blockIdx.y] * vec_per_frame;
   uint4* d = y + (size_t)blockIdx.y * vec_per_frame;
   for (size_t i = (size_t)blockIdx.x * blockDim.x + threadIdx.x; i < vec_per_frame; i += (size_t)gridDim.x * blockDim.x)
@@ -195,9 +198,8 @@
   }));
   const size_t HW = (size_t)H * W, total = (size_t)F * HW;
   ProfScope ps(PGT_PROF_MOVE, 15.0 * (double)total, static_cast<cudaStream_t>(stream), "pgt_u8hwc_to_f32nchw");
-  pgt::u8hwc_to_f32nchw_kernel<<<ew_grid(total, 256), 256, 0, static_cast<cudaStream_t>(stream)>>>(
+  PGT_LAUNCH(pgt::u8hwc_to_f32nchw_kernel, dim3(ew_grid(total, 256)), dim3(256), 0, static_cast<cudaStream_t>(stream),
       static_cast<const uint8_t*>(x_u8), HW, total, y);
-  PGT_LAUNCH_OK();
   return PGT_OK;
 }
 
@@ -205,9 +207,8 @@
   PGT_CHECK_ARG(x && y_u8 && n > 0 && H > 0 && W > 0 && first >= 0 && step >= 1);
   const size_t HW = (size_t)H * W, total = (size_t)n * HW;
   ProfScope ps(PGT_PROF_MOVE, 15.0 * (double)total, static_cast<cudaStream_t>(stream), "pgt_f32nchw_to_u8hwc");
-  pgt::f32nchw_to_u8hwc_kernel<<<ew_grid(total, 256), 256, 0, static_cast<cudaStream_t>(stream)>>>(
+  PGT_LAUNCH(pgt::f32nchw_to_u8hwc_kernel, dim3(ew_grid(total, 256)), dim3(256), 0, static_cast<cudaStream_t>(stream),
       x, HW, first, step, total, static_cast<uint8_t*>(y_u8));
-  PGT_LAUNCH_OK();
   return PGT_OK;
 }
 
@@ -217,8 +218,7 @@
   const size_t vec = (size_t)frame_bytes / 16;
   ProfScope ps(PGT_PROF_MOVE, 2.0 * (double)n * frame_bytes, static_cast<cudaStream_t>(stream), "pgt_gather_frames");
   unsigned bx = (unsigned)std::min<size_t>((vec + 255) / 256, 1024);
-  pgt::gather_frames_kernel<<<dim3(bx, n), 256, 0, static_cast<cudaStream_t>(stream)>>>(
+  PGT_LAUNCH(pgt::gather_frames_kernel, dim3(bx, n), dim3(256), 0, static_cast<cudaStream_t>(stream),
       static_cast<const uint4*>(x), vec, idx_dev, static_cast<uint4*>(y));
-  PGT_LAUNCH_OK();
-  return PGT_OK;
-}
+  return PGT_OK;
+}
diff --git a/pgtformer_b200/csrc/gemm_tc.cu b/pgtformer_b200/csrc/gemm_tc.cu
--- a/pgtformer_b200/csrc/gemm_tc.cu
+++ b/pgtformer_b200/csrc/gemm_tc.cu
@@ -553,6 +553,27 @@
   const uint32_t tmem_base = *tmem_ptr;
   const uint32_t rank = PAIR ? cluster_ctarank() : 0u;
 
+  int npre = 0;
+  if (warp == 0 && (int)blockIdx.x < num_tiles) {
+    int n_blk, m_blk;
+    tile_mn(p, blockIdx.x, m_blk, n_blk);
+    npre = p.num_kb < STAGES ? p.num_kb : STAGES;
+    if (elect_one()) {
+      for (int kb = 0; kb < npre; ++kb) {
+        void* dst_b = smem_b + kb * Cfg::B_STAGE_BYTES;
+        if constexpr (PAIR) {
+          if (rank == 0) mbar_arrive_expect_tx(&full_bar[kb], 2 * Cfg::STAGE_BYTES);
+          tma_load_2d_2sm(dst_b, &tmB, mapa_u32(smem_u32(&full_bar[kb]), 0), kb * BK, n_blk * BN + (int)rank * (BN / 2));
+        } else {
+          mbar_arrive_expect_tx(&full_bar[kb], Cfg::STAGE_BYTES);
+          tma_load_2d(dst_b, &tmB, &full_bar[kb], kb * BK, n_blk * BN);
+        }
+      }
+    }
+    __syncwarp();
+  }
+  pdl_wait();
+
   if (warp == 0) {
     {
       int stage = 0;
@@ -584,19 +605,20 @@
                 ax = x0 + qx; ay = y0 + qy; a5 = py;
               }
             }
+            const bool pre = tile == (int)blockIdx.x && kb < npre;
             if constexpr (PAIR) {
               const uint32_t fb = mapa_u32(smem_u32(&full_bar[stage]), 0);
-              if (rank == 0) mbar_arrive_expect_tx(&full_bar[stage], 2 * Cfg::STAGE_BYTES);
+              if (rank == 0 && !pre) mbar_arrive_expect_tx(&full_bar[stage], 2 * Cfg::STAGE_BYTES);
               if (p.mode == MODE_LINEAR) tma_load_2d_2sm(dst_a, &tmA, fb, kb * BK, m_blk * BM);
               else if (p.mode == MODE_CONV_S1) tma_load_4d_2sm(dst_a, &tmA, fb, cb * BK, ax, ay, n0);
               else tma_load_5d_2sm(dst_a, &tmA, fb, cb, ax, a5, ay, n0);
-              tma_load_2d_2sm(dst_b, &tmB, fb, kb * BK, n_blk * BN + (int)rank * (BN / 2));
+              if (!pre) tma_load_2d_2sm(dst_b, &tmB, fb, kb * BK, n_blk * BN + (int)rank * (BN / 2));
             } else {
-              mbar_arrive_expect_tx(&full_bar[stage], Cfg::STAGE_BYTES);
+              if (!pre) mbar_arrive_expect_tx(&full_bar[stage], Cfg::STAGE_BYTES);
               if (p.mode == MODE_LINEAR) tma_load_2d(dst_a, &tmA, &full_bar[stage], kb * BK, m_blk * BM);
               else if (p.mode == MODE_CONV_S1) tma_load_4d(dst_a, &tmA, &full_bar[stage], cb * BK, ax, ay, n0);
               else tma_load_5d(dst_a, &tmA, &full_bar[stage], cb, ax, a5, ay, n0);
-              tma_load_2d(dst_b, &tmB, &full_bar[stage], kb * BK, n_blk * BN);
+              if (!pre) tma_load_2d(dst_b, &tmB, &full_bar[stage], kb * BK, n_blk * BN);
             }
           }
           __syncwarp();
@@ -745,6 +767,20 @@
   tc_fence_after();
   const uint32_t tmem_base = *tmem_ptr;
 
+  const int npre = (int)blockIdx.x < num_tiles ? min(BS, p.ntaps * p.cin_blocks) : 0;
+  if (warp == 0) {
+    if (elect_one()) {
+      const int n_blk = blockIdx.x % p.n_tiles;
+      for (int i = 0; i < npre; ++i) {
+        const int cb = i / p.ntaps, t = i - cb * p.ntaps;
+        mbar_arrive_expect_tx(&b_full[i], Cfg::B_BYTES);
+        tma_load_2d(smem_b + i * Cfg::B_BYTES, &tmB, &b_full[i], t * cin_pad + cb * BK, n_blk * BN);
+      }
+    }
+    __syncwarp();
+  }
+  pdl_wait();
+
   if (warp == 0) {
     int as = 0, bs = 0;
     uint32_t aph = 0, bph = 0;
@@ -780,12 +816,14 @@
         if (++as == AS) { as = 0; aph ^= 1; }
         if (p.b_resident && tile != (int)blockIdx.x) continue;
         for (int t = 0; t < p.ntaps; ++t) {
-          mbar_wait(&b_empty[bs], bph ^ 1);
-          if (elect_one()) {
-            mbar_arrive_expect_tx(&b_full[bs], Cfg::B_BYTES);
-            tma_load_2d(smem_b + bs * Cfg::B_BYTES, &tmB, &b_full[bs], t * cin_pad + cb * BK, n_blk * BN);
+          if (tile != (int)blockIdx.x || cb * p.ntaps + t >= npre) {
+            mbar_wait(&b_empty[bs], bph ^ 1);
+            if (elect_one()) {
+              mbar_arrive_expect_tx(&b_full[bs], Cfg::B_BYTES);
+              tma_load_2d(smem_b + bs * Cfg::B_BYTES, &tmB, &b_full[bs], t * cin_pad + cb * BK, n_blk * BN);
+            }
+            __syncwarp();
           }
-          __syncwarp();
           if (++bs == BS) { bs = 0; bph ^= 1; }
         }
       }
@@ -1007,11 +1045,24 @@
   cluster_sync_all();
   tc_fence_after();
   const uint32_t tmem_base = *tmem_ptr;
+  const uint32_t a_full0 = mapa_u32(smem_u32(a_full), 0), b_full0 = mapa_u32(smem_u32(b_full), 0);
+
+  const int npre = (int)blockIdx.x < num_tiles ? min(BS, p.ntaps * p.cin_blocks) : 0;
+  if (warp == 0) {
+    if (elect_one()) {
+      for (int i = 0; i < npre; ++i) {
+        const int cb = i / p.ntaps, t = i - cb * p.ntaps;
+        if (rank == 0) mbar_arrive_expect_tx(&b_full[i], 2 * Cfg::B_BYTES);
+        tma_load_2d_2sm(smem_b + i * Cfg::B_BYTES, &tmB, b_full0 + i * 8, t * cin_pad + cb * BK, (int)rank * (BN / 2));
+      }
+    }
+    __syncwarp();
+  }
+  pdl_wait();
 
   if (warp == 0) {
     int as = 0, bs = 0;
     uint32_t aph = 0, bph = 0;
-    const uint32_t a_full0 = mapa_u32(smem_u32(a_full), 0), b_full0 = mapa_u32(smem_u32(b_full), 0);
     for (int tile = blockIdx.x; tile < num_tiles; tile += gridDim.x) {
       int n0, y0, x0;
       decode_conv_tile(p, tile, n0, y0, x0);
@@ -1041,12 +1092,14 @@
         if (++as == AS) { as = 0; aph ^= 1; }
         if (p.b_resident && tile != (int)blockIdx.x) continue;
         for (int t = 0; t < p.ntaps; ++t) {
-          mbar_wait(&b_empty[bs], bph ^ 1);
-          if (elect_one()) {
-            if (rank == 0) mbar_arrive_expect_tx(&b_full[bs], 2 * Cfg::B_BYTES);
-            tma_load_2d_2sm(smem_b + bs * Cfg::B_BYTES, &tmB, b_full0 + bs * 8, t * cin_pad + cb * BK, (int)rank * (BN / 2));
+          if (tile != (int)blockIdx.x || cb * p.ntaps + t >= npre) {
+            mbar_wait(&b_empty[bs], bph ^ 1);
+            if (elect_one()) {
+              if (rank == 0) mbar_arrive_expect_tx(&b_full[bs], 2 * Cfg::B_BYTES);
+              tma_load_2d_2sm(smem_b + bs * Cfg::B_BYTES, &tmB, b_full0 + bs * 8, t * cin_pad + cb * BK, (int)rank * (BN / 2));
+            }
+            __syncwarp();
           }
-          __syncwarp();
           if (++bs == BS) { bs = 0; bph ^= 1; }
         }
       }
@@ -1239,17 +1292,8 @@
       else snprintf(desc, sizeof(desc), "conv%d%s s%d F%d H%d W%d K%d N%d BN%d t%dx%dx%d e%d", p.ksize, PAIR ? " x2cta" : "", p.mode, p.F, p.H, p.W, p.K, p.N, BN, p.tn, p.th, p.tw, p.fast_epi);
     }
     ProfScope ps(PGT_PROF_GEMM, p.flops, stream, desc);
-    if (PAIR) {
-      cudaLaunchConfig_t cfg = {};
-      cfg.gridDim = dim3(grid); cfg.blockDim = dim3(GEMM_THREADS); cfg.dynamicSmemBytes = Cfg::SMEM_BYTES; cfg.stream = stream;
-      cudaLaunchAttribute attr[1];
-      attr[0].id = cudaLaunchAttributeClusterDimension;
-      attr[0].val.clusterDim.x = 2; attr[0].val.clusterDim.y = 1; attr[0].val.clusterDim.z = 1;
-      cfg.attrs = attr; cfg.numAttrs = 1;
-      PGT_CUDA_OK(cudaLaunchKernelEx(&cfg, gemm_tc_kernel<BN, PAIR>, tmA, tmB, tmO, tmR, tmX, p));
-    } else {
-      gemm_tc_kernel<BN, PAIR><<<grid, GEMM_THREADS, Cfg::SMEM_BYTES, stream>>>(tmA, tmB, tmO, tmR, tmX, p);
-    }
+    PGT_CUDA_OK(launch_pdl(gemm_tc_kernel<BN, PAIR>, dim3(grid), dim3(GEMM_THREADS), Cfg::SMEM_BYTES, stream, PAIR ? 2 : 1,
+                           tmA, tmB, tmO, tmR, tmX, p));
   }
   PGT_LAUNCH_OK();
   return PGT_OK;
@@ -1275,10 +1319,9 @@
       snprintf(desc, sizeof(desc), "halo3%s F%d H%d W%d K%d N%d BN%d e%d r%d", GN ? "+gn" : "", p.F, p.H, p.W, p.K, p.N, BN,
                p.fast_epi, p.b_resident);
     ProfScope ps(PGT_PROF_GEMM, p.flops, stream, desc);
-    conv_halo_kernel<BN, GN><<<grid, GN ? GEMM_THREADS + HALO_GN_THREADS : GEMM_THREADS, Cfg::SMEM_BYTES, stream>>>(
-        tmA, tmB, tmO, tmR, tmX, p);
-  }
-  PGT_LAUNCH_OK();
+    PGT_LAUNCH((conv_halo_kernel<BN, GN>), dim3(grid), dim3(GN ? GEMM_THREADS + HALO_GN_THREADS : GEMM_THREADS), Cfg::SMEM_BYTES,
+               stream, tmA, tmB, tmO, tmR, tmX, p);
+  }
   return PGT_OK;
 }
 
@@ -1302,9 +1345,8 @@
       snprintf(desc, sizeof(desc), "halo%d x2cta F%d H%d W%d K%d N%d BN%d e%d r%d", p.tap_kw, p.F, p.H, p.W, p.K, p.N, BN,
                p.fast_epi, p.b_resident);
     ProfScope ps(PGT_PROF_GEMM, p.flops, stream, desc);
-    conv_halo2_kernel<BN><<<grid, GEMM_THREADS, Cfg::SMEM_BYTES, stream>>>(tmA, tmB, tmO, tmR, tmX, p);
-  }
-  PGT_LAUNCH_OK();
+    PGT_LAUNCH(conv_halo2_kernel<BN>, dim3(grid), dim3(GEMM_THREADS), Cfg::SMEM_BYTES, stream, tmA, tmB, tmO, tmR, tmX, p);
+  }
   return PGT_OK;
 }
 
diff --git a/pgtformer_b200/csrc/l2_argmin_tc.cu b/pgtformer_b200/csrc/l2_argmin_tc.cu
--- a/pgtformer_b200/csrc/l2_argmin_tc.cu
+++ b/pgtformer_b200/csrc/l2_argmin_tc.cu
@@ -28,6 +28,7 @@
 
 __global__ void __launch_bounds__(256)
 codebook_pack_kernel(const float* __restrict__ cb, int K, int E, __nv_bfloat16* __restrict__ cb16, float* __restrict__ norm) {
+  pdl_wait();
   const int row = (blockIdx.x * blockDim.x + threadIdx.x) >> 5, lane = threadIdx.x & 31;
   if (row >= K) return;
   double s = 0.0;
@@ -57,6 +58,7 @@
 
 __global__ void __launch_bounds__(256)
 z_pack_kernel(const float* __restrict__ z, int T, int E, __nv_bfloat16* __restrict__ zb, float2* __restrict__ zn2) {
+  pdl_wait();
   constexpr int RB = 4;
   const int lane = threadIdx.x & 31;
   const int gw = (blockIdx.x * blockDim.x + threadIdx.x) >> 5, nw = (gridDim.x * blockDim.x) >> 5;
@@ -261,6 +263,7 @@
   cluster_sync_all();
   tc_fence_after();
   const uint32_t tmem_base = *tmem_ptr;
+  pdl_wait();
   const uint32_t rank = cluster_ctarank();
 
   if (warp == 0) {
@@ -428,8 +431,7 @@
   PGT_CHECK_ARG(codebook && cb_bf16 && cb_norm && K > 0 && E > 0);
   cudaStream_t st = static_cast<cudaStream_t>(stream);
   PGT_CUDA_OK(cudaMemsetAsync(cb_norm + K, 0, 2 * sizeof(float), st));
-  codebook_pack_kernel<<<ceil_div(K, 8), 256, 0, st>>>(codebook, K, E, reinterpret_cast<__nv_bfloat16*>(cb_bf16), cb_norm);
-  PGT_LAUNCH_OK();
+  PGT_LAUNCH(codebook_pack_kernel, dim3(ceil_div(K, 8)), dim3(256), 0, st, codebook, K, E, reinterpret_cast<__nv_bfloat16*>(cb_bf16), cb_norm);
   return PGT_OK;
 }
 
@@ -476,10 +478,9 @@
         if (best_waste < 0 || waste < best_waste) { best_waste = waste; pack_ctas = c; }
       }
     }
-    z_pack_kernel<<<pack_ctas, 256, 0, st>>>(z, T, E, zb, zn2);
-    l2_argmin_pair_kernel<<<2 * npairs, LT_THREADS, LT_SMEM, st>>>(tmA, tmB, z, zn2, T, E, codebook, cb_norm, K, idx, quant,
+    PGT_LAUNCH(z_pack_kernel, dim3(pack_ctas), dim3(256), 0, st, z, T, E, zb, zn2);
+    PGT_LAUNCH(l2_argmin_pair_kernel, dim3(2 * npairs), dim3(LT_THREADS), LT_SMEM, st, tmA, tmB, z, zn2, T, E, codebook, cb_norm, K, idx, quant,
                                                                    fb_count, fb_list);
-    PGT_LAUNCH_OK();
   }
   return l2_argmin_list_launch(z, T, E, codebook, K, idx, quant, fb_list, fb_count, num_sms(), st);
 }
diff --git a/pgtformer_b200/csrc/ln_linear.cu b/pgtformer_b200/csrc/ln_linear.cu
--- a/pgtformer_b200/csrc/ln_linear.cu
+++ b/pgtformer_b200/csrc/ln_linear.cu
@@ -63,6 +63,7 @@
   __syncthreads();
   tc_fence_after();
   const uint32_t tmem_base = *tmem_ptr;
+  if (warp != 0) pdl_wait();
   const int NB = p.nb;
 
   if (warp == 0) {
@@ -302,8 +303,7 @@
     char desc[64];
     if (prof_enabled()) snprintf(desc, sizeof(desc), "ln_linear M%d N%d K256", T, N);
     ProfScope ps(PGT_PROF_GEMM, 2.0 * (double)T * N * C, st, desc);
-    ln_linear_kernel<<<grid, LL_THREADS, LL_SMEM, st>>>(tx, to, tw, p);
-  }
-  PGT_LAUNCH_OK();
+    PGT_LAUNCH(ln_linear_kernel, dim3(grid), dim3(LL_THREADS), LL_SMEM, st, tx, to, tw, p);
+  }
   return PGT_OK;
 }
diff --git a/pgtformer_b200/csrc/mha_tc.cu b/pgtformer_b200/csrc/mha_tc.cu
--- a/pgtformer_b200/csrc/mha_tc.cu
+++ b/pgtformer_b200/csrc/mha_tc.cu
@@ -110,6 +110,7 @@
   __syncthreads();
   tc_fence_after();
   const uint32_t tmem_base = *tmem_ptr;
+  pdl_wait();
 
   if (warp == 0) {
     if (elect_one()) {
@@ -308,8 +309,7 @@
   static PerDeviceOnce once;
   PGT_CUDA_OK(once.run([] { return cudaFuncSetAttribute(mha_tc_kernel, cudaFuncAttributeMaxDynamicSharedMemorySize, FT_SMEM); }));
   dim3 grid(L / (2 * FT_BM), heads, clips);
-  mha_tc_kernel<<<grid, FT_THREADS, FT_SMEM, stream>>>(tq, tk, tv, L, reinterpret_cast<__nv_bfloat16*>(out), ldo);
-  PGT_LAUNCH_OK();
+  PGT_LAUNCH(mha_tc_kernel, dim3(grid), dim3(FT_THREADS), FT_SMEM, stream, tq, tk, tv, L, reinterpret_cast<__nv_bfloat16*>(out), ldo);
   return PGT_OK;
 }
 
diff --git a/pgtformer_b200/csrc/norm.cu b/pgtformer_b200/csrc/norm.cu
--- a/pgtformer_b200/csrc/norm.cu
+++ b/pgtformer_b200/csrc/norm.cu
@@ -21,6 +21,7 @@
 __global__ void __launch_bounds__(GN_THREADS)
 gn_stats_kernel(const __nv_bfloat16* __restrict__ x, int ldx, int HW, int C, int pix_per_chunk,
                 float* __restrict__ partial ) {
+  pdl_wait();
   extern __shared__ float sm[];
   const int vc = C >> 3;
   const int rows_par = GN_THREADS / vc;
@@ -81,6 +82,7 @@
 __global__ void __launch_bounds__(GN_FIN_PARTS * 32)
 gn_finalize_kernel(const float* __restrict__ partial, int nchunks, int HW, int C, const float* __restrict__ gamma,
                    const float* __restrict__ beta, float eps, float* __restrict__ ab ) {
+  pdl_wait();
   __shared__ float smean[GN_GROUPS], srstd[GN_GROUPS];
   __shared__ double ps[GN_FIN_PARTS][GN_GROUPS], pq[GN_FIN_PARTS][GN_GROUPS];
   const int f = blockIdx.x;
@@ -128,6 +130,7 @@
 __global__ void __launch_bounds__(GN_APPLY_THREADS, 3)
 gn_apply_kernel(const __nv_bfloat16* __restrict__ x, int ldx, int HW, int C, int pix_per_block,
                 const float* __restrict__ ab, int apply_silu, __nv_bfloat16* __restrict__ y, int ldy) {
+  pdl_wait();
   const int f = blockIdx.y;
   const int vc = C >> 3;
   const int rows_par = GN_APPLY_THREADS / vc;
@@ -186,6 +189,7 @@
 layernorm_kernel(const void* __restrict__ xin, int ldx, int x_dtype, int T, const float* __restrict__ gamma,
                  const float* __restrict__ beta, float eps, __nv_bfloat16* __restrict__ y, int ldy,
                  const __nv_bfloat16* __restrict__ pos, int ldpos, __nv_bfloat16* __restrict__ y2, int ldy2) {
+  pdl_wait();
   constexpr int C = 256 * NV;
   const int warp = (blockIdx.x * blockDim.x + threadIdx.x) >> 5;
   const int lane = threadIdx.x & 31;
@@ -269,6 +273,7 @@
 __global__ void __launch_bounds__(ADAIN_THREADS)
 adain_kernel(const void* __restrict__ qin, int ldq, int q_dtype, const __nv_bfloat16* __restrict__ l, int ldl, int HW,
              int C, float eps, __nv_bfloat16* __restrict__ y, int ldy) {
+  pdl_wait();
   __shared__ float red[4][ADAIN_THREADS / 8][64];
   __shared__ float sa[64], sb[64];
   const int f = blockIdx.y;
@@ -354,18 +359,15 @@
   const int ppc = ceil_div(HW, nchunks);
   float* ab = ws + (size_t)F * nchunks * GN_GROUPS * 2;
   const size_t stats_smem = ((size_t)(GN_THREADS / (C / 8)) + 1) * 2 * C * sizeof(float);
-  gn_stats_kernel<<<dim3(nchunks, F), GN_THREADS, stats_smem, st>>>(
+  PGT_LAUNCH(gn_stats_kernel, dim3(nchunks, F), dim3(GN_THREADS), stats_smem, st,
       reinterpret_cast<const __nv_bfloat16*>(x), ldx, HW, C, ppc, ws);
-  PGT_LAUNCH_OK();
-  gn_finalize_kernel<<<F, GN_FIN_PARTS * 32, 0, st>>>(ws, nchunks, HW, C, gamma, beta, eps, ab);
-  PGT_LAUNCH_OK();
+  PGT_LAUNCH(gn_finalize_kernel, dim3(F), dim3(GN_FIN_PARTS * 32), 0, st, ws, nchunks, HW, C, gamma, beta, eps, ab);
   int ppb = (131072 / (C * 2));
   if (ppb < 16) ppb = 16;
   const int nblk = ceil_div(HW, ppb);
-  gn_apply_kernel<<<dim3(nblk, F), GN_APPLY_THREADS, 0, st>>>(
+  PGT_LAUNCH(gn_apply_kernel, dim3(nblk, F), dim3(GN_APPLY_THREADS), 0, st,
       reinterpret_cast<const __nv_bfloat16*>(x), ldx, HW, C, ppb, ab, apply_silu,
       reinterpret_cast<__nv_bfloat16*>(y), ldy);
-  PGT_LAUNCH_OK();
   return PGT_OK;
 }
 
@@ -376,13 +378,11 @@
   PGT_CHECK_ARG(C % 32 == 0 && C % 8 == 0 && C / 8 <= GN_APPLY_THREADS && ldx % 8 == 0 && ldy % 8 == 0);
   cudaStream_t st = static_cast<cudaStream_t>(stream);
   ProfScope ps(PGT_PROF_NORM, 2.0 * F * (double)HW * C * 2, st, "gn_apply_stats");
-  gn_finalize_kernel<<<F, GN_FIN_PARTS * 32, 0, st>>>(stats, chunks_per_frame, HW, C, gamma, beta, eps, ws);
-  PGT_LAUNCH_OK();
+  PGT_LAUNCH(gn_finalize_kernel, dim3(F), dim3(GN_FIN_PARTS * 32), 0, st, stats, chunks_per_frame, HW, C, gamma, beta, eps, ws);
   int ppb = (131072 / (C * 2));
   if (ppb < 16) ppb = 16;
-  gn_apply_kernel<<<dim3(ceil_div(HW, ppb), F), GN_APPLY_THREADS, 0, st>>>(
+  PGT_LAUNCH(gn_apply_kernel, dim3(ceil_div(HW, ppb), F), dim3(GN_APPLY_THREADS), 0, st,
       reinterpret_cast<const __nv_bfloat16*>(x), ldx, HW, C, ppb, ws, apply_silu, reinterpret_cast<__nv_bfloat16*>(y), ldy);
-  PGT_LAUNCH_OK();
   return PGT_OK;
 }
 
@@ -392,8 +392,7 @@
   cudaStream_t st = static_cast<cudaStream_t>(stream);
   if (stats != nullptr) {
     PGT_CHECK_ARG(chunks_per_frame > 0);
-    gn_finalize_kernel<<<F, GN_FIN_PARTS * 32, 0, st>>>(stats, chunks_per_frame, HW, C, gamma, beta, eps, ab);
-    PGT_LAUNCH_OK();
+    PGT_LAUNCH(gn_finalize_kernel, dim3(F), dim3(GN_FIN_PARTS * 32), 0, st, stats, chunks_per_frame, HW, C, gamma, beta, eps, ab);
     return PGT_OK;
   }
   PGT_CHECK_ARG(x && ws && ldx % 8 == 0);
@@ -401,10 +400,8 @@
   const int nchunks = gn_chunks(HW);
   const int ppc = ceil_div(HW, nchunks);
   const size_t stats_smem = ((size_t)(GN_THREADS / (C / 8)) + 1) * 2 * C * sizeof(float);
-  gn_stats_kernel<<<dim3(nchunks, F), GN_THREADS, stats_smem, st>>>(reinterpret_cast<const __nv_bfloat16*>(x), ldx, HW, C, ppc, ws);
-  PGT_LAUNCH_OK();
-  gn_finalize_kernel<<<F, GN_FIN_PARTS * 32, 0, st>>>(ws, nchunks, HW, C, gamma, beta, eps, ab);
-  PGT_LAUNCH_OK();
+  PGT_LAUNCH(gn_stats_kernel, dim3(nchunks, F), dim3(GN_THREADS), stats_smem, st, reinterpret_cast<const __nv_bfloat16*>(x), ldx, HW, C, ppc, ws);
+  PGT_LAUNCH(gn_finalize_kernel, dim3(F), dim3(GN_FIN_PARTS * 32), 0, st, ws, nchunks, HW, C, gamma, beta, eps, ab);
   return PGT_OK;
 }
 
@@ -423,15 +420,14 @@
   auto y2b = reinterpret_cast<__nv_bfloat16*>(y2);
 #define PGT_LN_LAUNCH(NV_)                                                                                              \
   do {                                                                                                                \
-    if (y2b != nullptr) layernorm_kernel<NV_, true><<<grid, 256, 0, st>>>(x, ldx, x_dtype, T, gamma, beta, eps, yb, ldy, pb, ldpos, y2b, ldy2); \
-    else layernorm_kernel<NV_, false><<<grid, 256, 0, st>>>(x, ldx, x_dtype, T, gamma, beta, eps, yb, ldy, pb, ldpos, y2b, ldy2);           \
+    if (y2b != nullptr) PGT_LAUNCH((layernorm_kernel<NV_, true>), dim3(grid), dim3(256), 0, st, x, ldx, x_dtype, T, gamma, beta, eps, yb, ldy, pb, ldpos, y2b, ldy2); \
+    else PGT_LAUNCH((layernorm_kernel<NV_, false>), dim3(grid), dim3(256), 0, st, x, ldx, x_dtype, T, gamma, beta, eps, yb, ldy, pb, ldpos, y2b, ldy2);           \
   } while (0)
   if (C == 256) PGT_LN_LAUNCH(1);
   else if (C == 512) PGT_LN_LAUNCH(2);
   else if (C == 768) PGT_LN_LAUNCH(3);
   else PGT_LN_LAUNCH(4);
 #undef PGT_LN_LAUNCH
-  PGT_LAUNCH_OK();
   return PGT_OK;
 }
 
@@ -439,9 +435,8 @@
                          void* y, int ldy, void* stream) {
   PGT_CHECK_ARG(q && l && y && F > 0 && HW > 1 && C % 64 == 0 && ldq % 8 == 0 && ldl % 8 == 0 && ldy % 8 == 0);
   ProfScope ps(PGT_PROF_MOVE, 8.0 * F * (double)HW * C, static_cast<cudaStream_t>(stream), "adain");
-  adain_kernel<<<dim3(C / 64, F), ADAIN_THREADS, 0, static_cast<cudaStream_t>(stream)>>>(
+  PGT_LAUNCH(adain_kernel, dim3(C / 64, F), dim3(ADAIN_THREADS), 0, static_cast<cudaStream_t>(stream),
       q, ldq, q_dtype, reinterpret_cast<const __nv_bfloat16*>(l), ldl, HW, C, eps,
       reinterpret_cast<__nv_bfloat16*>(y), ldy);
-  PGT_LAUNCH_OK();
   return PGT_OK;
 }
diff --git a/pgtformer_b200/csrc/parsing.cu b/pgtformer_b200/csrc/parsing.cu
--- a/pgtformer_b200/csrc/parsing.cu
+++ b/pgtformer_b200/csrc/parsing.cu
@@ -18,6 +18,7 @@
 
 __global__ void maxpool3x3s2_kernel(const __nv_bfloat16* __restrict__ x, int ldx, int F, int H, int W, int C,
                                     __nv_bfloat16* __restrict__ y, int ldy) {
+  pdl_wait();
   const int Ho = H >> 1, Wo = W >> 1, vc = C >> 3;
   const size_t total = (size_t)F * Ho * Wo * vc;
   for (size_t i = (size_t)blockIdx.x * blockDim.x + threadIdx.x; i < total; i += (size_t)gridDim.x * blockDim.x) {
@@ -49,6 +50,7 @@
 
 __global__ void __launch_bounds__(256)
 global_avgpool_kernel(const __nv_bfloat16* __restrict__ x, int ldx, int HW, int C, __nv_bfloat16* __restrict__ y, int ldy) {
+  pdl_wait();
   __shared__ float red[32][64];
   const int f = blockIdx.y, cbase = blockIdx.x * 64;
   const int vcol = threadIdx.x & 7, prow = threadIdx.x >> 3;
@@ -78,6 +80,7 @@
                                       const __nv_bfloat16* __restrict__ scale, int lds, int plus_one,
                                       const __nv_bfloat16* __restrict__ addv, int ldv,
                                       const __nv_bfloat16* __restrict__ addm, int ldm, __nv_bfloat16* __restrict__ y, int ldy) {
+  pdl_wait();
   const int vc = C >> 3;
   const size_t total = (size_t)F * HW * vc;
   for (size_t i = (size_t)blockIdx.x * blockDim.x + threadIdx.x; i < total; i += (size_t)gridDim.x * blockDim.x) {
@@ -108,6 +111,7 @@
 __global__ void assemble_cond_kernel(const __nv_bfloat16* __restrict__ o0, int ld0, const __nv_bfloat16* __restrict__ o1,
                                      int ld1, const __nv_bfloat16* __restrict__ o2, int ld2, int F, int h8, int w8, int h16,
                                      int w16, int ncls, __nv_bfloat16* __restrict__ cond, int ldc) {
+  pdl_wait();
   const size_t total = (size_t)F * h16 * w16 * 64;
   const float sy = h16 > 1 ? (float)(h8 - 1) / (float)(h16 - 1) : 0.f;
   const float sx = w16 > 1 ? (float)(w8 - 1) / (float)(w16 - 1) : 0.f;
@@ -150,9 +154,8 @@
   const size_t total = (size_t)F * (H / 2) * (W / 2) * (C / 8);
   cudaStream_t st = static_cast<cudaStream_t>(stream);
   ProfScope ps(PGT_PROF_MOVE, 2.5 * F * (double)H * W * C, st, "maxpool");
-  maxpool3x3s2_kernel<<<grid_for(total, 256), 256, 0, st>>>(reinterpret_cast<const __nv_bfloat16*>(x), ldx, F, H, W, C,
+  PGT_LAUNCH(maxpool3x3s2_kernel, dim3(grid_for(total, 256)), dim3(256), 0, st, reinterpret_cast<const __nv_bfloat16*>(x), ldx, F, H, W, C,
                                                            reinterpret_cast<__nv_bfloat16*>(y), ldy);
-  PGT_LAUNCH_OK();
   return PGT_OK;
 }
 
@@ -160,9 +163,8 @@
   PGT_CHECK_ARG(x && y && F > 0 && HW > 0 && C % 8 == 0 && ldx % 8 == 0 && ldy >= C);
   cudaStream_t st = static_cast<cudaStream_t>(stream);
   ProfScope ps(PGT_PROF_MOVE, 2.0 * F * (double)HW * C, st, "avgpool");
-  global_avgpool_kernel<<<dim3(ceil_div(C, 64), F), 256, 0, st>>>(reinterpret_cast<const __nv_bfloat16*>(x), ldx, HW, C,
+  PGT_LAUNCH(global_avgpool_kernel, dim3(ceil_div(C, 64), F), dim3(256), 0, st, reinterpret_cast<const __nv_bfloat16*>(x), ldx, HW, C,
                                                                  reinterpret_cast<__nv_bfloat16*>(y), ldy);
-  PGT_LAUNCH_OK();
   return PGT_OK;
 }
 
@@ -173,11 +175,10 @@
   const size_t total = (size_t)F * HW * (C / 8);
   cudaStream_t st = static_cast<cudaStream_t>(stream);
   ProfScope ps(PGT_PROF_MOVE, (addm ? 6.0 : 4.0) * F * (double)HW * C, st, "channel_affine");
-  channel_affine_kernel<<<grid_for(total, 256), 256, 0, st>>>(
+  PGT_LAUNCH(channel_affine_kernel, dim3(grid_for(total, 256)), dim3(256), 0, st,
       reinterpret_cast<const __nv_bfloat16*>(x), ldx, F, HW, C, reinterpret_cast<const __nv_bfloat16*>(scale), lds, plus_one,
       reinterpret_cast<const __nv_bfloat16*>(addv), ldv, reinterpret_cast<const __nv_bfloat16*>(addm), ldm,
       reinterpret_cast<__nv_bfloat16*>(y), ldy);
-  PGT_LAUNCH_OK();
   return PGT_OK;
 }
 
@@ -188,9 +189,8 @@
   const size_t total = (size_t)F * h16 * w16 * 64;
   cudaStream_t st = static_cast<cudaStream_t>(stream);
   ProfScope ps(PGT_PROF_MOVE, 4.0 * (double)total, st, "assemble_cond");
-  assemble_cond_kernel<<<grid_for(total, 256), 256, 0, st>>>(
+  PGT_LAUNCH(assemble_cond_kernel, dim3(grid_for(total, 256)), dim3(256), 0, st,
       reinterpret_cast<const __nv_bfloat16*>(o0), ld0, reinterpret_cast<const __nv_bfloat16*>(o1), ld1,
       reinterpret_cast<const __nv_bfloat16*>(o2), ld2, F, h8, w8, h16, w16, ncls, reinterpret_cast<__nv_bfloat16*>(cond), ldc);
-  PGT_LAUNCH_OK();
   return PGT_OK;
 }
diff --git a/pgtformer_b200/csrc/rgb_conv.cu b/pgtformer_b200/csrc/rgb_conv.cu
--- a/pgtformer_b200/csrc/rgb_conv.cu
+++ b/pgtformer_b200/csrc/rgb_conv.cu
@@ -100,6 +100,7 @@
   __syncthreads();
   tc_fence_after();
   const uint32_t tmem_base = *tmem_ptr;
+  pdl_wait();
 
   if (warp < BW) {
     const int r = threadIdx.x & 127;
@@ -227,9 +228,8 @@
   const int grid = p.m_tiles < num_sms() * Cfg::PER_SM ? p.m_tiles : num_sms() * Cfg::PER_SM;
   {
     ProfScope ps(PGT_PROF_GEMM, 2.0 * (double)p.M * RC_N * Cfg::K, st, desc);
-    rgb_conv_kernel<KS, STRIDE, PAD><<<grid, Cfg::THREADS, Cfg::SMEM, st>>>(tw, to, p);
-  }
-  PGT_LAUNCH_OK();
+    PGT_LAUNCH((rgb_conv_kernel<KS, STRIDE, PAD>), dim3(grid), dim3(Cfg::THREADS), Cfg::SMEM, st, tw, to, p);
+  }
   return PGT_OK;
 }
 
diff --git a/pgtformer_b200/csrc/swin_mlp.cu b/pgtformer_b200/csrc/swin_mlp.cu
--- a/pgtformer_b200/csrc/swin_mlp.cu
+++ b/pgtformer_b200/csrc/swin_mlp.cu
@@ -189,6 +189,7 @@
   __syncthreads();
   tc_fence_after();
   const uint32_t tmem_base = *tmem_ptr;
+  if (warp != 0) pdl_wait();
 
   const int n_loc = (int)blockIdx.x < p.m_tiles ? (p.m_tiles - 1 - (int)blockIdx.x) / (int)gridDim.x + 1 : 0;
   const int n_grp[2] = {(n_loc + 1) >> 1, n_loc >> 1};
@@ -311,8 +312,7 @@
   const int grid = p.m_tiles < num_sms() ? p.m_tiles : num_sms();
   {
     ProfScope ps(PGT_PROF_GEMM, 4.0 * (double)T * C * C, st, "swin_mlp_fused C256");
-    swin_mlp_kernel<<<grid, SM_THREADS, SM_SMEM, st>>>(tx, to, t1, t2, p);
-  }
-  PGT_LAUNCH_OK();
+    PGT_LAUNCH(swin_mlp_kernel, dim3(grid), dim3(SM_THREADS), SM_SMEM, st, tx, to, t1, t2, p);
+  }
   return PGT_OK;
 }
diff --git a/pgtformer_b200/csrc/window3d.cu b/pgtformer_b200/csrc/window3d.cu
--- a/pgtformer_b200/csrc/window3d.cu
+++ b/pgtformer_b200/csrc/window3d.cu
@@ -32,6 +32,7 @@
 template <int HD>
 __global__ void __launch_bounds__(256)
 window3d_attn_kernel(const Win3dParams p) {
+  pdl_wait();
   constexpr int LDS = HD + 8;
   extern __shared__ __align__(16) unsigned char smem_raw[];
   __nv_bfloat16* qs = reinterpret_cast<__nv_bfloat16*>(smem_raw);
@@ -207,14 +208,13 @@
   dim3 grid(B * p.nd * p.nh * p.nw, heads);
   const size_t smem = (size_t)3 * W3_MAXNP * (hd + 8) * 2;
   ProfScope ps(PGT_PROF_WINDOW_ATTN, 4.0 * N * N * C * (double)grid.x, st, "window3d");
-  if (hd == 16) window3d_attn_kernel<16><<<grid, 256, smem, st>>>(p);
-  else if (hd == 32) window3d_attn_kernel<32><<<grid, 256, smem, st>>>(p);
+  if (hd == 16) PGT_LAUNCH((window3d_attn_kernel<16>), dim3(grid), dim3(256), smem, st, p);
+  else if (hd == 32) PGT_LAUNCH((window3d_attn_kernel<32>), dim3(grid), dim3(256), smem, st, p);
   else {
     static PerDeviceOnce once;
     PGT_CUDA_OK(once.run([] { return cudaFuncSetAttribute(window3d_attn_kernel<64>, cudaFuncAttributeMaxDynamicSharedMemorySize,
                                                           3 * W3_MAXNP * (64 + 8) * 2); }));
-    window3d_attn_kernel<64><<<grid, 256, smem, st>>>(p);
-  }
-  PGT_LAUNCH_OK();
+    PGT_LAUNCH((window3d_attn_kernel<64>), dim3(grid), dim3(256), smem, st, p);
+  }
   return PGT_OK;
 }
diff --git a/pgtformer_b200/csrc/window_attn_tc.cu b/pgtformer_b200/csrc/window_attn_tc.cu
--- a/pgtformer_b200/csrc/window_attn_tc.cu
+++ b/pgtformer_b200/csrc/window_attn_tc.cu
@@ -119,6 +119,7 @@
   __syncthreads();
   tc_fence_after();
   const uint32_t tmem_base = *tmem_ptr;
+  pdl_wait();
 
   const int my_pairs = (p.n_pairs - (int)blockIdx.x + (int)gridDim.x - 1) / (int)gridDim.x;
   const int NCH = p.n_chunks;
@@ -401,12 +402,11 @@
   if (d == 32) {
     static PerDeviceOnce once;
     PGT_CUDA_OK(once.run([] { return cudaFuncSetAttribute(window_attn_tc_kernel<32>, cudaFuncAttributeMaxDynamicSharedMemorySize, WT_SMEM); }));
-    window_attn_tc_kernel<32><<<grid, WT_THREADS, WT_SMEM, st>>>(mi[0], mi[1], mi[2], mi[3], p);
+    PGT_LAUNCH((window_attn_tc_kernel<32>), dim3(grid), dim3(WT_THREADS), WT_SMEM, st, mi[0], mi[1], mi[2], mi[3], p);
   } else {
     static PerDeviceOnce once;
     PGT_CUDA_OK(once.run([] { return cudaFuncSetAttribute(window_attn_tc_kernel<64>, cudaFuncAttributeMaxDynamicSharedMemorySize, WT_SMEM); }));
-    window_attn_tc_kernel<64><<<grid, WT_THREADS, WT_SMEM, st>>>(mi[0], mi[1], mi[2], mi[3], p);
-  }
-  PGT_LAUNCH_OK();
+    PGT_LAUNCH((window_attn_tc_kernel<64>), dim3(grid), dim3(WT_THREADS), WT_SMEM, st, mi[0], mi[1], mi[2], mi[3], p);
+  }
   return PGT_OK;
 }
```

New measurement: 183.4, median of 6. Within noise of the previous version (-0.3%).
